# foggy-frost-forest/UniMoE-Audio

Hardware: AMD Instinct MI355X
Metric: audio-tokens/sec/node (TTS decode, bs=8 per GPU) (higher is better)
Workload: dtype bf16; 1 GPU; BASELINE configs[1]: TTS decode batch 8 (16 CFG rows) per GPU, 300-token prompt, 36-layer DCMoE (8+1 routed, 2 shared), 12x1027 codec head, CFG 3.0 + top-k 45 + top-p 0.95 sampling, 16 kHz DAC 50 frames/s; global_batch=8, prompt_len=300, kv_len_end=396, parallelism=single, graph=True

## Files before the change

include/umoe.h:

```cpp
#ifndef UMOE_H
#define UMOE_H

#include <stddef.h>
#include <stdint.h>

#ifdef __cplusplus
extern "C" {
#endif

typedef void* umoe_stream_t;

const char* umoe_last_error(void);
int umoe_abi_version(void);
size_t umoe_struct_size(const char* name);

size_t umoe_packed_elems(int N, int K);
int umoe_pack_weight(const uint16_t* W, int N, int K, uint16_t* packed, umoe_stream_t stream);
int umoe_pack_gate_up(const uint16_t* Wg, const uint16_t* Wu, int I, int K, uint16_t* packed, umoe_stream_t stream);

typedef struct {
    const uint16_t* x;
    const uint16_t* gate_w;
    const uint16_t* norm_w;
    uint16_t* h_out;
// ... 366 lines not shown
int umoe_delay_step(int64_t* pred, int32_t* tokens, int32_t* state, const int32_t* delay, int B, int C, int Tmax,
                    int eos, int pad, int max_delay, umoe_stream_t stream);
int umoe_delay_step_rows(int64_t* pred, int32_t* tokens, int32_t* state, const int32_t* delay, int B, int C, int Tmax,
                         int eos, int pad, int max_delay, const umoe_row_params* row_params, umoe_stream_t stream);
int umoe_delay_step_clock(int64_t* pred, int32_t* tokens, int32_t* state, const int32_t* delay, int B, int C, int Tmax,
                          int eos, int pad, int max_delay, const umoe_row_params* row_params, const int32_t* row_clock,
                          umoe_stream_t stream);

int umoe_codec_ce_fwd(const float* logits, const int64_t* labels, int N, int C, int V, float* nll_ws, float* probs,
                      float* ch_loss, int32_t* ch_count, float* total, umoe_stream_t stream);
int umoe_codec_ce_bwd(const float* probs, const int64_t* labels, const int32_t* ch_count, int N, int C, int V, float grad,
                      float* dlogits, umoe_stream_t stream);

int umoe_rvq_from_codes(const int32_t* codes, const float* codebooks, const float* out_w, const float* out_b, int NQ,
                        int CB, int cd, int Dl, int T, float* z, umoe_stream_t stream);
int umoe_rvq_from_delayed(const int32_t* tokens, int B, int Tmax, int NQ, const int32_t* prefill_step, const int32_t* delay, int t_valid,
                          int pad, const int32_t* rows, int Bz, int f0, int n, const float* codebooks, const float* out_w, const float* out_b,
                          int CB, int cd, int Dl, float* z, int z_off, int Lz, umoe_stream_t stream);
int umoe_rvq_nearest(const float* z, const float* codebooks, const float* in_w, const float* in_b, const float* out_w,
                     const float* out_b, int NQ, int CB, int cd, int Dl, int T, int32_t* codes, float* resid_ws,
                     umoe_stream_t stream);

int umoe_dac_conv1d(const float* x, const float* w, const float* bias, const float* snake_alpha, const float* resid, int B, int Cin,
                    int L, int Cout, int K, int stride, int dilation, int pad, int act, float* y, int* Lout_out, umoe_stream_t stream);
int umoe_dac_conv_transpose1d(const float* x, const float* w, const float* bias, const float* snake_alpha, int B, int Cin, int L,
                              int Cout, int K, int stride, int pad, int out_pad, float* y, int* Lout_out, umoe_stream_t stream);
int umoe_dac_conv1d_win(const float* x, int x_off, int Lx, const float* w, const float* bias, const float* snake_alpha, const float* resid,
                        int r_off, int Lr, int B, int Cin, int L, int Cout, int K, int stride, int dilation, int pad, int act, int t_begin,
                        int n, float* y, int y_off, int Ly, umoe_stream_t stream);
int umoe_dac_conv_transpose1d_win(const float* x, int x_off, int Lx, const float* w, const float* bias, const float* snake_alpha, int B,
                                  int Cin, int L, int Cout, int K, int stride, int pad, int out_pad, int t_begin, int n, float* y, int y_off,
                                  int Ly, umoe_stream_t stream);
int umoe_dac_resample(const float* x, const float* kern, int B, int L, int o, int n, int width, int Lout, float* y, umoe_stream_t stream);

int umoe_vision_rope(uint16_t* qkv, const float* cos_t, const float* sin_t, int S, int H, int hd, umoe_stream_t stream);
int umoe_vision_attn(const uint16_t* qkv, const int32_t* seg_lo, const int32_t* seg_hi, int S, int H, int hd, float scale, uint16_t* out,
                     umoe_stream_t stream);
int umoe_swiglu_pair(const uint16_t* gu, int S, int I, int ldh, uint16_t* h, umoe_stream_t stream);
int umoe_gelu(uint16_t* x, long n, umoe_stream_t stream);

typedef struct {
    int hidden, layers, heads, kv_heads, head_dim;
    int n_dyn, n_real, n_fix, inter_dyn, inter_shared;
    int codec_channels, codec_vocab, eos, pad, bos;
    int mrope0, mrope1, mrope2;
    float rms_eps, top_p;
    int fixed_top_k;
    double jitter_eps;
    int rows;
    int Lmax;
    int Tmax;
    int attn_splits;
    int ep_rank, ep_size;
} umoe_engine_cfg;

typedef struct {
    const uint16_t* in_norm;
    const uint16_t* qkv_w;
    const float* qkv_b;
    const uint16_t* o_w;
    const uint16_t* post_norm;
    const uint16_t* gate_w;
    const uint16_t* const* exp_gu;
    const uint16_t* const* exp_dn;
    const uint16_t* const* sh_gu;
    const uint16_t* const* sh_dn;
    const uint16_t* rm_qkv;
    const uint16_t* rm_o;
    const uint16_t* const* rm_exp_gate;
    const uint16_t* const* rm_exp_up;
    const uint16_t* const* rm_exp_down;
    const uint16_t* const* rm_sh_gate;
    const uint16_t* const* rm_sh_up;
    const uint16_t* const* rm_sh_down;
} umoe_layer_weights;

typedef struct umoe_engine umoe_engine;
int umoe_engine_create(const umoe_engine_cfg* cfg, umoe_engine** out);
void umoe_engine_destroy(umoe_engine* e);
int umoe_engine_set_layer(umoe_engine* e, int layer, const umoe_layer_weights* w);
int umoe_engine_set_layer_fp8(umoe_engine* e, int layer, const uint8_t* const* gu8, const int8_t* const* gu_e, const uint8_t* const* dn8,
                              const int8_t* const* dn_e);
int umoe_engine_set_fp8_wide(umoe_engine* e, int on);
int umoe_fp8_convert_probe(const uint8_t* q, const int8_t* e, int N, int K, uint16_t* out, umoe_stream_t stream);
int umoe_engine_set_globals(umoe_engine* e, const uint16_t* final_norm, const uint16_t* codec_emb,
                            const uint16_t* codec_head_w, const uint16_t* cos_tab, const uint16_t* sin_tab, int max_pos,
                            const int32_t* delay_pattern_host);
size_t umoe_engine_workspace_bytes(const umoe_engine* e);
int umoe_engine_prefill(umoe_engine* e, const uint16_t* x, const uint8_t* valid_host, int T, umoe_stream_t stream);
int umoe_engine_prefill_pos(umoe_engine* e, const uint16_t* x, const uint8_t* valid_host, int T, const int32_t* pos3_host,
                            const int32_t* next_pos_host, umoe_stream_t stream);
int umoe_engine_prefill_external(umoe_engine* e, const uint8_t* valid_host, int T, const int32_t* pos3_host, const int32_t* next_pos_host,
                                 umoe_stream_t stream);
typedef struct {
    int32_t* tokens;
    int32_t* state;
    float cfg_scale, temperature, top_p, eos_mul;
    int top_k, do_sample, min_tokens;
    uint64_t seed;
    int32_t* row_clock;
    const umoe_row_params* row_params;
} umoe_decode_io;
int umoe_engine_decode_step(umoe_engine* e, const umoe_decode_io* io, umoe_stream_t stream);
int umoe_engine_capture(umoe_engine* e, const umoe_decode_io* io, umoe_stream_t stream);
int umoe_engine_replay(umoe_engine* e, umoe_stream_t stream);
int umoe_engine_profile_step(umoe_engine* e, const umoe_decode_io* io, umoe_stream_t stream, float* ms, int* launches,
                             int n);
int umoe_engine_reserve(umoe_engine* e, int n_tok);
int umoe_engine_admit(umoe_engine* e, const umoe_decode_io* io, int b, const uint16_t* x, const uint8_t* valid_host, int T,
                      int prefill_step, int prefix_len, umoe_stream_t stream);
int umoe_engine_admit_external(umoe_engine* e, const umoe_decode_io* io, int b, const uint8_t* valid_host, int T, int prefill_step,
                               int prefix_len, umoe_stream_t stream);
enum { UMOE_EP_PEER = 0, UMOE_EP_LOOPBACK = 1, UMOE_EP_RCCL = 2 };
int umoe_engine_ep_region(umoe_engine* e, void** base_out, size_t* bytes_out);
int umoe_engine_ep_connect(umoe_engine* e, void* const* peers, void* rccl_comm, int mode);
int umoe_engine_ep_error(umoe_engine* e, umoe_stream_t stream, int* code_out);
int umoe_engine_set_probe(umoe_engine* e, const uint16_t* teach_x, uint16_t* dump_x1, uint16_t* dump_x, uint16_t* dump_logits);
int umoe_engine_info(umoe_engine* e, const char* key);
const void* umoe_engine_buffer(umoe_engine* e, const char* name, size_t* bytes);

#ifdef __cplusplus
}
#endif
#endif
```

unimoe_audio_amd/_lib.py:

```python
from __future__ import annotations

import ctypes as C
import os
import subprocess

_HERE = os.path.dirname(os.path.abspath(__file__))
_CSRC = os.path.join(_HERE, "csrc")
_SO = os.environ.get("UMOE_HIP_LIB") or os.path.join(_CSRC, "libumoe_hip.so")
_lib = None


class UmoeError(RuntimeError):
    pass


def build(force: bool = False) -> str:
    srcs = [os.path.join(_CSRC, f) for f in os.listdir(_CSRC) if f.endswith((".hip", ".h"))]
    srcs.append(os.path.join(os.path.dirname(_HERE), "include", "umoe.h"))
    stale = (not os.path.exists(_SO)) or any(os.path.getmtime(s) > os.path.getmtime(_SO) for s in srcs)
    if force or stale:
        subprocess.check_call(["make", "-C", _CSRC, "-j4", "-s"])
    return _SO


# ... 44 lines not shown
                ("counts", vp), ("offsets", vp), ("slot_token", vp), ("max_rows", i32), ("slot_rows", i32), ("row_base", i32),
                ("x", vp), ("ldx", i32), ("h", vp), ("ldh", i32), ("gu", vp), ("ldgu", i32), ("dy", vp), ("lddy", i32),
                ("dx_slots", vp), ("lddx", i32), ("dw_gate", C.POINTER(vp)), ("dw_up", C.POINTER(vp)), ("dw_down", C.POINTER(vp)),
                ("ws", vp), ("ws_bytes", C.c_size_t), ("w_down_T", vp), ("w_gateup_T", vp)]


class AttnBwdArgs(C.Structure):
    _fields_ = [("q", vp), ("k_cache", vp), ("v_cache", vp), ("kv_start_host", vp), ("d_out", vp), ("rows", i32), ("T", i32), ("H", i32),
                ("KVH", i32), ("hd", i32), ("Lmax", i32), ("scale", f32), ("dq", vp), ("dk_cache", vp), ("dv_cache", vp), ("ws", vp),
                ("ws_bytes", C.c_size_t), ("out", vp), ("lse", vp)]


class CombineArgs(C.Structure):
    _fields_ = [("y_slots", vp), ("slot_of", vp), ("moe_w", vp), ("y_shared", vp), ("global_w", vp), ("resid", vp),
                ("out", vp), ("S", i32), ("D", i32), ("n_real", i32), ("n_dyn", i32), ("n_fix", i32), ("y_parts", vp), ("n_parts", i32), ("part_stride", C.c_long),
                ("shared_row0", i32), ("norm_w", vp),
                ("norm_out", vp), ("rms_eps", f32), ("expert_mask", vp), ("mask_ld", i32), ("dense_rows", i32), ("ep_xfer", vp)]


class RopeArgs(C.Structure):
    _fields_ = [("qkv", vp), ("cos_tab", vp), ("sin_tab", vp), ("pos3", vp), ("kv_pos", vp), ("n_tok", i32), ("T", i32),
                ("H", i32), ("KVH", i32), ("hd", i32), ("sec0", i32), ("sec1", i32), ("sec2", i32), ("Lmax", i32),
                ("q_out", vp), ("k_cache", vp), ("v_cache", vp)]


class AttnArgs(C.Structure):
    _fields_ = [("q", vp), ("k_cache", vp), ("v_cache", vp), ("kv_start", vp), ("q_pos0", vp), ("rows", i32),
                ("nq", i32), ("H", i32), ("KVH", i32), ("hd", i32), ("Lmax", i32), ("splits", i32), ("scale", f32),
                ("part_o", vp), ("part_ml", vp), ("out", vp), ("qkv_raw", vp), ("cos_tab", vp), ("sin_tab", vp), ("pos3", vp),
                ("sec0", i32), ("sec1", i32), ("sec2", i32), ("lse_out", vp)]


class RowParams(C.Structure):
    _fields_ = [("cfg_scale", f32), ("temperature", f32), ("top_p", f32), ("eos_mul", f32), ("top_k", C.c_int32), ("do_sample", C.c_int32),
                ("min_tokens", C.c_int32), ("max_tokens", C.c_int32), ("seed", u64)]


class SampleArgs(C.Structure):
    _fields_ = [("logits", vp), ("B", i32), ("C", i32), ("V", i32), ("cfg_scale", f32), ("temperature", f32),
                ("top_p", f32), ("eos_mul", f32), ("top_k", i32), ("eos", i32), ("enable_eos", i32),
                ("min_tokens", i32), ("step", vp), ("do_sample", i32), ("seed", u64), ("pred", vp), ("probs_out", vp),
                ("row_clock", vp), ("row_params", vp)]


class EngineCfg(C.Structure):
    _fields_ = [("hidden", i32), ("layers", i32), ("heads", i32), ("kv_heads", i32), ("head_dim", i32),
                ("n_dyn", i32), ("n_real", i32), ("n_fix", i32), ("inter_dyn", i32), ("inter_shared", i32),
                ("codec_channels", i32), ("codec_vocab", i32), ("eos", i32), ("pad", i32), ("bos", i32),
                ("mrope0", i32), ("mrope1", i32), ("mrope2", i32), ("rms_eps", f32), ("top_p", f32),
                ("fixed_top_k", i32), ("jitter_eps", f64), ("rows", i32), ("Lmax", i32), ("Tmax", i32),
                ("attn_splits", i32), ("ep_rank", i32), ("ep_size", i32)]


class LayerWeights(C.Structure):
    _fields_ = [("in_norm", vp), ("qkv_w", vp), ("qkv_b", vp), ("o_w", vp), ("post_norm", vp), ("gate_w", vp),
                ("exp_gu", C.POINTER(vp)), ("exp_dn", C.POINTER(vp)), ("sh_gu", C.POINTER(vp)), ("sh_dn", C.POINTER(vp)),
                ("rm_qkv", vp), ("rm_o", vp), ("rm_exp_gate", C.POINTER(vp)), ("rm_exp_up", C.POINTER(vp)),
                ("rm_exp_down", C.POINTER(vp)), ("rm_sh_gate", C.POINTER(vp)), ("rm_sh_up", C.POINTER(vp)),
                ("rm_sh_down", C.POINTER(vp))]


class DecodeIO(C.Structure):
    _fields_ = [("tokens", vp), ("state", vp), ("cfg_scale", f32), ("temperature", f32), ("top_p", f32),
                ("eos_mul", f32), ("top_k", i32), ("do_sample", i32), ("min_tokens", i32), ("seed", u64), ("row_clock", vp), ("row_params", vp)]


EXPORTS = [
    "umoe_last_error", "umoe_abi_version", "umoe_packed_elems", "umoe_pack_weight", "umoe_pack_gate_up",
    "umoe_router_fwd", "umoe_router_dispatch_fwd", "umoe_dispatch_build", "umoe_transpose_slots_compact", "umoe_aux_loss_fwd", "umoe_aux_loss_fwd_ws", "umoe_aux_loss_workspace_floats", "umoe_permute_fwd", "umoe_grouped_gemm", "umoe_grouped_swiglu_fwd", "umoe_shared_swiglu_fwd", "umoe_attn_prefill_fwd",
    "umoe_unpermute_combine_fwd", "umoe_rmsnorm_residual_fwd", "umoe_qkv_mrope_kvappend", "umoe_attn_decode",
    "umoe_codec_embed_sum", "umoe_codec_embed_sum_bwd", "umoe_mul_noise", "umoe_codec_head_cfg_sample", "umoe_delay_step", "umoe_rvq_from_codes",
    "umoe_rvq_nearest", "umoe_codec_ce_fwd", "umoe_codec_ce_bwd", "umoe_engine_create", "umoe_engine_destroy", "umoe_engine_set_layer",
    "umoe_engine_set_globals", "umoe_engine_workspace_bytes", "umoe_engine_prefill", "umoe_engine_decode_step",
    "umoe_engine_capture", "umoe_engine_replay", "umoe_engine_buffer", "umoe_engine_profile_step", "umoe_prefetch", "umoe_tiled_gemm", "umoe_tiled_gemm_tn", "umoe_tiled_gemm_tn_workspace_bytes", "umoe_tiled_gemm_tn_split", "umoe_dispatch_build_aligned", "umoe_transpose_slots", "umoe_swiglu_bwd",
    "umoe_unpermute_combine_bwd", "umoe_permute_bwd", "umoe_router_bwd", "umoe_rmsnorm_residual_bwd", "umoe_aux_loss_bwd", "umoe_attn_softmax_fwd", "umoe_attn_softmax_bwd", "umoe_qkv_mrope_bwd",
    "umoe_swiglu_bwd_workspace_bytes", "umoe_grouped_swiglu_bwd", "umoe_shared_swiglu_bwd",
    "umoe_attn_prefill_bwd_workspace_bytes", "umoe_attn_prefill_bwd",
    "umoe_ep_unique_id", "umoe_ep_comm_create", "umoe_ep_comm_destroy", "umoe_ep_all_to_all",
    "umoe_ep_ipc_export", "umoe_ep_ipc_open", "umoe_ep_ipc_close", "umoe_engine_ep_region", "umoe_engine_ep_connect",
    "umoe_engine_ep_error", "umoe_token_drop", "umoe_router_bwd_drop", "umoe_router_bwd_ex", "umoe_dac_conv1d", "umoe_dac_conv_transpose1d", "umoe_dac_resample", "umoe_vision_rope", "umoe_vision_attn", "umoe_swiglu_pair", "umoe_gelu", "umoe_engine_prefill_pos", "umoe_engine_set_probe", "umoe_engine_info", "umoe_engine_prefill_external", "umoe_engine_set_layer_fp8", "umoe_fp8_convert_probe",
    "umoe_dac_conv1d_win", "umoe_dac_conv_transpose1d_win", "umoe_rvq_from_delayed", "umoe_delay_step_rows",
    "umoe_delay_step_clock", "umoe_engine_reserve", "umoe_engine_admit", "umoe_engine_admit_external", "umoe_gemm_wide", "umoe_pack_rows",
    "umoe_gemm_wide_fp8", "umoe_engine_set_fp8_wide", "umoe_tiled_gemm_wp8",
]

EP_PEER, EP_LOOPBACK, EP_RCCL = 0, 1, 2
MAX_EP = 8


def _mirrors():
    return {"umoe_router_args": RouterArgs, "umoe_group_t": Group, "umoe_gemm_args": GemmArgs, "umoe_tgroup_t": TGroup,
            "umoe_tgemm_args": TGemmArgs, "umoe_tn_group_t": TnGroup, "umoe_tgemm_tn_args": TGemmTnArgs, "umoe_swiglu_bwd_args": SwigluBwdArgs, "umoe_attn_bwd_args": AttnBwdArgs,
            "umoe_combine_args": CombineArgs, "umoe_rope_args": RopeArgs, "umoe_attn_args": AttnArgs, "umoe_sample_args": SampleArgs,
            "umoe_engine_cfg": EngineCfg, "umoe_layer_weights": LayerWeights, "umoe_decode_io": DecodeIO}


STRUCT_MIRRORS = _mirrors()
TABLE_MIRRORS = {"umoe_row_params": RowParams}


def lib():
    global _lib
    if _lib is None:
        if not os.path.exists(_SO):
            raise UmoeError(f"{_SO} is missing: run `python -c 'import __graft_entry__ as g; g.build()'` "
                            "(hipcc --offload-arch=gfx950). There is no CPU fallback for the product path.")
        L = C.CDLL(_SO)
        L.umoe_last_error.restype = C.c_char_p
        L.umoe_packed_elems.restype = C.c_size_t
        L.umoe_packed_elems.argtypes = [i32, i32]
        L.umoe_engine_workspace_bytes.restype = C.c_size_t
        L.umoe_engine_workspace_bytes.argtypes = [vp]
        L.umoe_engine_buffer.restype = vp
        L.umoe_engine_buffer.argtypes = [vp, C.c_char_p, C.POINTER(C.c_size_t)]
        L.umoe_engine_destroy.restype = None
        L.umoe_engine_destroy.argtypes = [vp]
        L.umoe_pack_weight.argtypes = [vp, i32, i32, vp, vp]
        L.umoe_pack_gate_up.argtypes = [vp, vp, i32, i32, vp, vp]
        L.umoe_router_fwd.argtypes = [C.POINTER(RouterArgs), vp]
        L.umoe_dispatch_build.argtypes = [vp, i32, i32, i32, vp, vp, vp, vp, vp]
        L.umoe_aux_loss_fwd.argtypes = [vp, i32, vp, vp, i32, i32, i32, vp, vp]
        L.umoe_aux_loss_fwd_ws.argtypes = [vp, i32, vp, vp, i32, i32, i32, vp, vp, vp]
        L.umoe_aux_loss_workspace_floats.argtypes = []
        L.umoe_aux_loss_workspace_floats.restype = C.c_size_t
        L.umoe_prefetch.argtypes = [vp, C.c_size_t, i32, vp]
        L.umoe_transpose_slots.argtypes = [vp, i32, i32, vp, vp, vp, i32, i32, vp, i32, vp]
        L.umoe_swiglu_bwd.argtypes = [vp, i32, vp, i32, i32, vp, i32, vp, i32, vp]
        L.umoe_unpermute_combine_bwd.argtypes = [vp, vp, vp, vp, vp, vp, vp]
        L.umoe_permute_bwd.argtypes = [vp, vp, i32, vp, i32, i32, i32, vp, vp, vp]
        L.umoe_router_bwd.argtypes = [vp, i32, vp, vp, vp, vp, vp, vp, i32, i32, i32, i32, f64, vp, vp]
        L.umoe_router_bwd_drop.argtypes = [vp, i32, vp, vp, vp, vp, vp, vp, i32, i32, i32, i32, f64, vp, vp]
        L.umoe_router_bwd_ex.argtypes = [vp, i32, vp, vp, vp, vp, vp, vp, i32, i32, i32, i32, f64, i32, vp, vp, vp]
        L.umoe_dac_conv1d.argtypes = [vp, vp, vp, vp, vp, i32, i32, i32, i32, i32, i32, i32, i32, i32, vp, C.POINTER(i32), vp]
        L.umoe_dac_conv_transpose1d.argtypes = [vp, vp, vp, vp, i32, i32, i32, i32, i32, i32, i32, i32, vp, C.POINTER(i32), vp]
        L.umoe_dac_resample.argtypes = [vp, vp, i32, i32, i32, i32, i32, i32, vp, vp]
        L.umoe_dac_conv1d_win.argtypes = [vp, i32, i32, vp, vp, vp, vp, i32, i32] + [i32] * 9 + [i32, i32, vp, i32, i32, vp]
        L.umoe_dac_conv_transpose1d_win.argtypes = [vp, i32, i32, vp, vp, vp] + [i32] * 8 + [i32, i32, vp, i32, i32, vp]
        L.umoe_rvq_from_delayed.argtypes = [vp, i32, i32, i32, vp, vp, i32, i32, vp, i32, i32, i32, vp, vp, vp, i32, i32, i32, vp, i32, i32, vp]
        L.umoe_vision_rope.argtypes = [vp, vp, vp, i32, i32, i32, vp]
        L.umoe_vision_attn.argtypes = [vp, vp, vp, i32, i32, i32, f32, vp, vp]
        L.umoe_swiglu_pair.argtypes = [vp, i32, i32, i32, vp, vp]
        L.umoe_gelu.argtypes = [vp, C.c_long, vp]
        L.umoe_engine_prefill_pos.argtypes = [vp, vp, vp, i32, vp, vp, vp]
        L.umoe_token_drop.argtypes = [vp, i32, vp, vp, i32, i32, i32, i32, i32, i32, vp, vp, vp, vp, vp]
        L.umoe_rmsnorm_residual_bwd.argtypes = [vp, vp, vp, vp, f32, i32, i32, vp, vp, vp, C.c_size_t, vp]
        L.umoe_dispatch_build_aligned.argtypes = [vp, i32, i32, i32, i32, vp, vp, vp, vp, vp]
        L.umoe_aux_loss_bwd.argtypes = [vp, i32, vp, vp, i32, i32, i32, vp, vp, vp, vp]
        L.umoe_attn_softmax_fwd.argtypes = [vp, i32, i32, i32, i32, i32, f32, vp, i32, vp]
        L.umoe_attn_softmax_bwd.argtypes = [vp, vp, i32, i32, i32, i32, f32, vp, vp]
        L.umoe_qkv_mrope_bwd.argtypes = [C.POINTER(RopeArgs), vp, vp, vp, vp, vp]
        L.umoe_tiled_gemm_tn.argtypes = [C.POINTER(TGemmTnArgs), vp]
        L.umoe_tiled_gemm_tn_workspace_bytes.argtypes = [C.POINTER(TGemmTnArgs)]
        L.umoe_tiled_gemm_tn_workspace_bytes.restype = C.c_size_t
        L.umoe_tiled_gemm_tn_split.argtypes = [C.POINTER(TGemmTnArgs)]
        L.umoe_swiglu_bwd_workspace_bytes.argtypes = [C.POINTER(SwigluBwdArgs)]
        L.umoe_swiglu_bwd_workspace_bytes.restype = C.c_size_t
        L.umoe_grouped_swiglu_bwd.argtypes = [C.POINTER(SwigluBwdArgs), vp]
        L.umoe_shared_swiglu_bwd.argtypes = [C.POINTER(SwigluBwdArgs), vp]
        L.umoe_attn_prefill_bwd_workspace_bytes.argtypes = [C.POINTER(AttnBwdArgs)]
        L.umoe_attn_prefill_bwd_workspace_bytes.restype = C.c_size_t
        L.umoe_attn_prefill_bwd.argtypes = [C.POINTER(AttnBwdArgs), vp]
        L.umoe_ep_unique_id.argtypes = [vp]
        L.umoe_ep_comm_create.argtypes = [vp, i32, i32, C.POINTER(vp)]
        L.umoe_ep_comm_destroy.argtypes = [vp]
        L.umoe_ep_all_to_all.argtypes = [vp, vp, vp, C.c_size_t, i32, vp]
        L.umoe_ep_ipc_export.argtypes = [vp, vp]
        L.umoe_ep_ipc_open.argtypes = [vp, C.POINTER(vp)]
        L.umoe_ep_ipc_close.argtypes = [vp]
        L.umoe_engine_ep_region.argtypes = [vp, C.POINTER(vp), C.POINTER(C.c_size_t)]
        L.umoe_engine_ep_connect.argtypes = [vp, C.POINTER(vp), vp, i32]
        L.umoe_engine_ep_error.argtypes = [vp, vp, C.POINTER(i32)]
        L.umoe_engine_set_probe.argtypes = [vp, vp, vp, vp, vp]
        L.umoe_engine_info.argtypes = [vp, C.c_char_p]
        L.umoe_engine_prefill_external.argtypes = [vp, vp, i32, vp, vp, vp]
        L.umoe_router_dispatch_fwd.argtypes = [C.POINTER(RouterArgs), vp, vp, vp, vp, vp]
        L.umoe_permute_fwd.argtypes = [vp, i32, vp, vp, i32, vp, vp]
        L.umoe_grouped_gemm.argtypes = [C.POINTER(GemmArgs), vp]
        L.umoe_unpermute_combine_fwd.argtypes = [C.POINTER(CombineArgs), vp]
        L.umoe_rmsnorm_residual_fwd.argtypes = [vp, vp, vp, f32, i32, i32, vp, vp, vp]
        L.umoe_qkv_mrope_kvappend.argtypes = [C.POINTER(RopeArgs), vp]
        L.umoe_attn_decode.argtypes = [C.POINTER(AttnArgs), vp]
        L.umoe_attn_prefill_fwd.argtypes = [C.POINTER(AttnArgs), vp]
        L.umoe_codec_embed_sum.argtypes = [vp, vp, i32, i32, i32, i32, vp, vp]
        L.umoe_codec_embed_sum_bwd.argtypes = [vp, vp, i32, i32, i32, i32, vp, vp]
        L.umoe_mul_noise.argtypes = [vp, vp, C.c_long, vp, vp]
        L.umoe_codec_head_cfg_sample.argtypes = [C.POINTER(SampleArgs), vp]
        L.umoe_delay_step.argtypes = [vp, vp, vp, vp, i32, i32, i32, i32, i32, i32, vp]
        if not hasattr(L, "umoe_delay_step_rows"):
            raise UmoeError(f"{_SO} predates this package (no umoe_delay_step_rows): rebuild it (`make -C unimoe_audio_amd/csrc`)")
        L.umoe_delay_step_rows.argtypes = [vp, vp, vp, vp, i32, i32, i32, i32, i32, i32, vp, vp]
        if not hasattr(L, "umoe_engine_admit"):
            raise UmoeError(f"{_SO} predates this package (no umoe_engine_admit): rebuild it (`make -C unimoe_audio_amd/csrc`)")
        L.umoe_delay_step_clock.argtypes = [vp, vp, vp, vp, i32, i32, i32, i32, i32, i32, vp, vp, vp]
        L.umoe_engine_reserve.argtypes = [vp, i32]
        L.umoe_engine_admit.argtypes = [vp, C.POINTER(DecodeIO), i32, vp, vp, i32, i32, i32, vp]
        L.umoe_engine_admit_external.argtypes = [vp, C.POINTER(DecodeIO), i32, vp, i32, i32, i32, vp]
        if not hasattr(L, "umoe_gemm_wide"):
            raise UmoeError(f"{_SO} predates this package (no umoe_gemm_wide): rebuild it (`make -C unimoe_audio_amd/csrc`)")
        L.umoe_gemm_wide.argtypes = [C.POINTER(vp), C.POINTER(i32), C.POINTER(i32), i32, i32, C.POINTER(vp), C.POINTER(vp), i32, i32,
                                     C.POINTER(vp), C.POINTER(vp), i32, i32, i32, vp]
        L.umoe_pack_rows.argtypes = [vp, i32, i32, i32, vp, f32, vp, vp]
        if not hasattr(L, "umoe_gemm_wide_fp8"):
            raise UmoeError(f"{_SO} predates this package (no umoe_gemm_wide_fp8): rebuild it (`make -C unimoe_audio_amd/csrc`)")
        L.umoe_gemm_wide_fp8.argtypes = [C.POINTER(vp), C.POINTER(vp), C.POINTER(i32), C.POINTER(i32), i32, i32, C.POINTER(vp), C.POINTER(vp), i32, i32,
                                         i32, i32, i32, vp]
        L.umoe_engine_set_fp8_wide.argtypes = [vp, i32]
        if not hasattr(L, "umoe_tiled_gemm_wp8"):
            raise UmoeError(f"{_SO} predates this package (no umoe_tiled_gemm_wp8): rebuild it (`make -C unimoe_audio_amd/csrc`)")
        L.umoe_tiled_gemm_wp8.argtypes = [C.POINTER(TGemmArgs), C.POINTER(vp), C.POINTER(vp), vp]
        L.umoe_rvq_from_codes.argtypes = [vp, vp, vp, vp, i32, i32, i32, i32, i32, vp, vp]
        L.umoe_rvq_nearest.argtypes = [vp, vp, vp, vp, vp, vp, i32, i32, i32, i32, i32, vp, vp, vp]
        L.umoe_codec_ce_fwd.argtypes = [vp, vp, i32, i32, i32, vp, vp, vp, vp, vp, vp]
        L.umoe_codec_ce_bwd.argtypes = [vp, vp, vp, i32, i32, i32, f32, vp, vp]
        L.umoe_engine_create.argtypes = [C.POINTER(EngineCfg), C.POINTER(vp)]
        L.umoe_engine_set_layer.argtypes = [vp, i32, C.POINTER(LayerWeights)]
        L.umoe_engine_set_globals.argtypes = [vp, vp, vp, vp, vp, vp, i32, vp]
        L.umoe_engine_prefill.argtypes = [vp, vp, vp, i32, vp]
        L.umoe_engine_decode_step.argtypes = [vp, C.POINTER(DecodeIO), vp]
        L.umoe_engine_capture.argtypes = [vp, C.POINTER(DecodeIO), vp]
        L.umoe_engine_replay.argtypes = [vp, vp]
        L.umoe_engine_profile_step.argtypes = [vp, C.POINTER(DecodeIO), vp, C.POINTER(f32), C.POINTER(i32), i32]
        if not hasattr(L, "umoe_struct_size"):
            raise UmoeError(f"{_SO} predates this package (no umoe_struct_size): rebuild it (`make -C unimoe_audio_amd/csrc`)")
        L.umoe_struct_size.restype = C.c_size_t
        L.umoe_struct_size.argtypes = [C.c_char_p]
        for cname, cls in list(STRUCT_MIRRORS.items()) + list(TABLE_MIRRORS.items()):
            built = int(L.umoe_struct_size(cname.encode()))
            if built != C.sizeof(cls):
                raise UmoeError(f"{_SO}: sizeof({cname}) is {built} in the library and {C.sizeof(cls)} in unimoe_audio_amd/_lib.py: "
                                "the library and the package are of different versions -- rebuild (`make -C unimoe_audio_amd/csrc`)")
        _lib = L
    return _lib


def check(rc: int, what: str = ""):
    if rc != 0:
        msg = lib().umoe_last_error()
        raise UmoeError(f"{what} failed (rc={rc}): {msg.decode() if msg else ''}")
```

unimoe_audio_amd/csrc/umoe_common.h:

```cpp
#pragma once
#include <hip/hip_runtime.h>
#include <stdarg.h>
#include <stdint.h>
#include <stdio.h>

#include "umoe.h"

typedef __attribute__((ext_vector_type(8))) __bf16 bf16x8_t;
typedef __attribute__((ext_vector_type(4))) float f32x4_t;

#define UMOE_MAXE 16

void umoe_set_error(const char* fmt, ...);
#define UMOE_HIP(expr)                                                                      \
    do {                                                                                    \
        hipError_t _e = (expr);                                                             \
        if (_e != hipSuccess) {                                                             \
            umoe_set_error("%s failed: %s (%s:%d)", #expr, hipGetErrorString(_e), __FILE__, __LINE__); \
            return -2;                                                                      \
        }                                                                                   \
    } while (0)
#define UMOE_REQUIRE(cond, ...)          \
    do {                                 \
        if (!(cond)) {                   \
// ... 101 lines not shown
    p = fma(p, r, 1.0 / 3628800.0);
    p = fma(p, r, 1.0 / 362880.0);
    p = fma(p, r, 1.0 / 40320.0);
    p = fma(p, r, 1.0 / 5040.0);
    p = fma(p, r, 1.0 / 720.0);
    p = fma(p, r, 1.0 / 120.0);
    p = fma(p, r, 1.0 / 24.0);
    p = fma(p, r, 1.0 / 6.0);
    p = fma(p, r, 0.5);
    p = fma(p, r, 1.0);
    p = fma(p, r, 1.0);
    const long long ki = (long long)k;
    const double scale = __longlong_as_double((ki + 1023) << 52);
    return (float)(p * scale);
}

__device__ __forceinline__ float wave_sum(float v) {
#pragma unroll
    for (int o = 32; o >= 1; o >>= 1) v += __shfl_xor(v, o, 64);
    return v;
}
__device__ __forceinline__ float wave_max(float v) {
#pragma unroll
    for (int o = 32; o >= 1; o >>= 1) v = fmaxf(v, __shfl_xor(v, o, 64));
    return v;
}

#if defined(__HIPCC__)
__device__ __forceinline__ float block_sum_256(float v, float* sh) {
    v = wave_sum(v);
    if ((threadIdx.x & 63) == 0) sh[threadIdx.x >> 6] = v;
    __syncthreads();
    const float r = sh[0] + sh[1] + sh[2] + sh[3];
    __syncthreads();
    return r;
}
#endif
static inline int ceil_div(int a, int b) { return (a + b - 1) / b; }

struct BwdSide {
    hipStream_t side = nullptr;
    hipEvent_t fork = nullptr, mid = nullptr, join = nullptr;
    bool ok = false;
};
BwdSide& bwd_side();

#define UMOE_EP_PARTS 16
#define UMOE_EP_FLAG_BYTES (2 * UMOE_MAX_EP * UMOE_EP_PARTS * 64)
struct umoe_ep_xfer {
    char* peer_base[UMOE_MAX_EP];
    const char* src;
    long src_stride;
    char* dst;
    size_t chunk;
    size_t data_off;
    int kind;
    int rank, size, loopback;
    int rows, row_bytes, n_sub;
    const uint32_t* step;
    int layer, layers;
    uint32_t* err;
    const uint32_t* round;
    int n_cwg;
};
int umoe_ep_push(const umoe_ep_xfer& x, hipStream_t s);
int umoe_ep_pull(const umoe_ep_xfer& x, hipStream_t s);
int umoe_ep_pull_pack(const umoe_ep_xfer& x, const uint16_t* own_rows, hipStream_t s);
int umoe_router_norm_push(const umoe_router_args* a, const umoe_ep_xfer& x, hipStream_t s);
int umoe_ep_rccl_allgather(void* comm, const void* send, void* recv, size_t bytes, hipStream_t s);

#define UMOE_FLAG_REPL 8
struct umoe_rider_pub {
    uint32_t* flags;
    const uint32_t* step;
    int layer, layers;
    uint32_t* err;
};

int umoe_moe_flat(const umoe_gemm_args* gu, const umoe_gemm_args* dn, uint32_t* flags, int flag_words, int n_wg, hipStream_t s);
bool umoe_moe_flat_feasible(int n_wg, int S, int D, int I_dyn, int I_sh, int n_real, int n_fix);
int umoe_moe_flat_fp8(const umoe_gemm_args* gu, const umoe_gemm_args* dn, const int8_t* const* e_gu, const int8_t* const* e_dn, uint32_t* flags,
                      int flag_words, int n_wg, hipStream_t s);
bool umoe_moe_flat_fp8_feasible(int n_wg, int S, int D, int I_dyn, int I_sh, int n_real, int n_fix);

struct umoe_rider2;
int umoe_gemm_riders(const umoe_gemm_args* a, int kind, const umoe_rider2* r2, const umoe_rider_pub* pub, hipStream_t s);

#define UMOE_MT_MAXG 4
#define UMOE_MT_MAXT UMOE_MAX_EP
struct umoe_mt_args {
    const uint16_t* w[UMOE_MT_MAXG];
    int num_groups, n_blocks, k;
    int tiles, n_rows;
    const uint16_t* b;
    int b_group_tiles;
    uint16_t* h_out;
    uint16_t* y_out[UMOE_MT_MAXG][UMOE_MT_MAXT];
    int ldo;
    int epilogue;
    const umoe_router_args* fused_router;
};
int umoe_gemm_mt(const umoe_mt_args* a, hipStream_t s);

#define UMOE_EPF_MAXT 24
struct umoe_epf_desc {
    const umoe_router_args* router;
    const umoe_rider_pub* pub;
    int R, rank, loopback, E_loc, S, D, I_dyn, I_sh, n_fix, n_wg;
    char* const* peer_base;
    size_t disp_off, ret_off;
    const uint16_t* const* w_lgu;
    const uint16_t* const* w_ldn;
    const uint16_t* const* w_sgu;
    const uint16_t* const* w_sdn;
    uint16_t* xgp;
    uint16_t* hpk;
    uint16_t* h_sh; int ldh, h_row0;
    uint16_t* y_sh; int ldy, y_row0;
    uint32_t* flags; int flag_words;
    const uint32_t* round;
    uint32_t* tasks_dev;
    int n_cwg;
    int proda_base[4], proda_n[4], prodb_base[UMOE_MT_MAXG], prodb_n[UMOE_MT_MAXG];
};
int umoe_moe_ep_prepare(umoe_epf_desc* d, hipStream_t s);
int umoe_moe_ep(const umoe_epf_desc* d, hipStream_t s);

#if defined(__HIPCC__)
typedef __attribute__((address_space(1))) uint32_t umoe_gu32;
#define UMOE_SYS_AUX 17
__device__ __forceinline__ umoe_gu32* umoe_ep_flag(char* base, int kind, int tile, int part) {
    return reinterpret_cast<umoe_gu32*>(reinterpret_cast<uintptr_t>(base + ((size_t)(kind * UMOE_MAX_EP + tile) * UMOE_EP_PARTS + part) * 64));
}
__device__ __forceinline__ uint32_t umoe_ep_epoch(const umoe_ep_xfer& x) { return *x.step * (uint32_t)x.layers + (uint32_t)x.layer + 1u; }
__device__ __forceinline__ void umoe_ep_wait(umoe_gu32* flag, uint32_t epoch, uint32_t* err_word) {
    umoe_gu32* err = reinterpret_cast<umoe_gu32*>(reinterpret_cast<uintptr_t>(err_word));
    const unsigned long long t0 = wall_clock64();
    for (unsigned spins = 0;; ++spins) {
        const uint32_t v = __hip_atomic_load(flag, __ATOMIC_RELAXED, __HIP_MEMORY_SCOPE_SYSTEM);
        if ((int32_t)(v - epoch) >= 0) break;
        __builtin_amdgcn_s_sleep(2);
        if ((spins & 255u) == 255u) {
            if (__hip_atomic_load(err, __ATOMIC_RELAXED, __HIP_MEMORY_SCOPE_AGENT) != 0u) break;
            if (wall_clock64() - t0 > 1000000000ull) {
                __hip_atomic_store(err, 1u, __ATOMIC_RELAXED, __HIP_MEMORY_SCOPE_AGENT);
                break;
            }
        }
    }
}
#endif
```

unimoe_audio_amd/csrc/umoe_engine.hip:

```cpp
#include <string.h>

#include <string>
#include <vector>

#include "umoe_common.h"
#include "umoe_riders_dev.h"

namespace {

struct LayerDev {
    umoe_layer_weights w;
    std::vector<const uint16_t*> exp_gu, exp_dn, sh_gu, sh_dn;
    std::vector<const uint16_t*> rm_eg, rm_eu, rm_ed, rm_sg, rm_su, rm_sd;
    bool has_rm = false;
    bool has_rm_attn = false;
    bool has_rm_exp = false;
    bool exp_bf16 = true;
    bool set = false;
    std::vector<const uint16_t*> f8_gu, f8_dn;
    std::vector<const int8_t*> f8e_gu, f8e_dn;
    bool has_f8 = false;
};

struct Carver {
    char* base = nullptr;
    size_t off = 0;
    template <typename T>
    T* take(size_t n) {
        off = (off + 255) & ~(size_t)255;
        T* p = base ? reinterpret_cast<T*>(base + off) : nullptr;
        off += n * sizeof(T);
        return p;
    }
};

}

struct umoe_engine {
    umoe_engine_cfg c;
    std::vector<LayerDev> layers;
    const uint16_t *final_norm = nullptr, *codec_emb = nullptr, *codec_head_w = nullptr, *cos_tab = nullptr,
                   *sin_tab = nullptr;
    int max_pos = 0;
    int max_delay = 0;
    char* ws = nullptr;
    size_t ws_bytes = 0;
    int cap_tok = 0;
    uint16_t *k_cache = nullptr, *v_cache = nullptr;
    int32_t* d_delay = nullptr;
    umoe_group_t* d_groups = nullptr;
    std::vector<umoe_group_t> h_groups;
    std::vector<umoe_group_t> h_gu_pub;
    int groups_for_tok = -1;
    uint16_t *x = nullptr, *hin = nullptr, *x1 = nullptr, *h2 = nullptr, *qkv = nullptr, *q_r = nullptr, *attn_out = nullptr,
             *hbuf = nullptr, *ybuf = nullptr;
    float *part_o = nullptr, *part_ml = nullptr, *logits = nullptr, *ypart = nullptr;
    int32_t *pos3 = nullptr, *kv_pos = nullptr, *q_pos0 = nullptr, *kv_start = nullptr, *tok_in = nullptr,
            *valid_count = nullptr, *eng_state = nullptr;
    void* r_logits = nullptr;
    int64_t *r_topk = nullptr, *pred = nullptr;
    int32_t *r_sel = nullptr, *r_mask = nullptr, *counts = nullptr, *offsets = nullptr, *slot_token = nullptr,
            *slot_of = nullptr;
    float *r_routing = nullptr, *r_global = nullptr, *r_moe = nullptr;
    int32_t* all_mask = nullptr;
    int64_t* all_topk = nullptr;
    int T_prompt = 0;
    int adm_row0 = -1;
    int32_t* adm_q0 = nullptr;
    int reserved_tok = 0;
    const uint16_t* probe_teach = nullptr;
    uint16_t *probe_x1 = nullptr, *probe_x = nullptr, *probe_logits = nullptr;
    bool probe_on() const { return probe_teach || probe_x1 || probe_x || probe_logits; }
    hipGraph_t graph = nullptr;
    hipGraphExec_t exec = nullptr;
    bool fuse_router = true;
    bool fuse_cq = true;
    int cb_ep_layer = -1;
    bool cb_pending = false;
    umoe_combine_args cb_stash{};
    int dense_min_rows = 2;
    int expert_launch = 0;
    bool fp8 = false;
    int prefill_fp8 = 0;
    int expert_fp8 = 0;
    bool fp8_wide = false;
    int n_cu = 0;
    bool tiled_prefill = true;
    bool prof = false;
    std::vector<hipEvent_t> ev;
    std::vector<int> ev_kind;
    size_t ev_used = 0;
    int E_loc = 0;
    char* ep_region = nullptr;
    size_t ep_region_bytes = 0;
    int ep_mem_kind = 0;
    char* ep_peers[UMOE_MAX_EP] = {};
    void* ep_comm = nullptr;
    int ep_mode = -1;
    uint32_t* ep_words = nullptr;
    uint16_t* xg = nullptr;
    uint16_t *xgp = nullptr, *hpk = nullptr;
    uint16_t *wide_in = nullptr, *wide_h = nullptr;
    int row_tiles = 1;
    bool in_decode_step = false;
    bool ep_flat = true;
    bool epf_ready = false;
    umoe_epf_desc epf{};
    uint32_t* epf_tasks = nullptr;
    bool ep_decode(int n_tok) const { return c.ep_size > 1 && n_tok == c.rows; }
    int groups_per_layer() const { return 2 + 2 * (c.n_real + c.n_fix); }
};

static size_t carve(umoe_engine* e, int n_tok, char* base) {
    const umoe_engine_cfg& c = e->c;
    const int D = c.hidden, QKV = (c.heads + 2 * c.kv_heads) * c.head_dim, HD = c.heads * c.head_dim;
    const int E = c.n_dyn + c.n_fix, G = c.n_real + c.n_fix;
    const int Imax = c.inter_dyn > c.inter_shared ? c.inter_dyn : c.inter_shared;
    const size_t slots = (size_t)n_tok * G;
    const int splits = c.attn_splits > 1 ? c.attn_splits : 1;
    Carver k;
    k.base = base;
    e->x = k.take<uint16_t>((size_t)n_tok * D);
    e->hin = k.take<uint16_t>((size_t)n_tok * D);
    e->x1 = k.take<uint16_t>((size_t)n_tok * D);
    e->h2 = k.take<uint16_t>((size_t)n_tok * D);
    e->qkv = k.take<uint16_t>((size_t)n_tok * QKV);
    e->q_r = k.take<uint16_t>((size_t)n_tok * HD);
    e->attn_out = k.take<uint16_t>((size_t)n_tok * HD);
    e->hbuf = k.take<uint16_t>(slots * Imax);
    e->ybuf = k.take<uint16_t>(slots * D + (c.ep_size > 1 ? (size_t)c.n_real * c.rows * D : 0));
    e->xg = k.take<uint16_t>(c.ep_size > 1 ? (size_t)c.ep_size * c.rows * D : 0);
    e->xgp = k.take<uint16_t>(c.ep_size > 1 ? (size_t)c.ep_size * 16 * D : 0);
    e->hpk = k.take<uint16_t>(c.ep_size > 1 ? (size_t)c.n_real * 16 * c.inter_dyn : 0);
    const int wt = (c.ep_size == 1 && c.rows > 16 && c.rows <= 64) ? ceil_div(c.rows, 16) : 0;
    e->wide_in = k.take<uint16_t>((size_t)wt * 16 * (D > HD ? D : HD));
    e->wide_h = k.take<uint16_t>((size_t)wt * 16 * Imax * G);
    e->part_o = k.take<float>((size_t)n_tok * c.heads * splits * c.head_dim);
    e->part_ml = k.take<float>((size_t)n_tok * c.heads * splits * 2);
    e->logits = k.take<float>((size_t)c.rows * c.codec_channels * c.codec_vocab);
    e->pos3 = k.take<int32_t>((size_t)3 * n_tok);
    e->kv_pos = k.take<int32_t>(n_tok);
    e->q_pos0 = k.take<int32_t>(c.rows);
    e->kv_start = k.take<int32_t>(c.rows);
    e->valid_count = k.take<int32_t>(c.rows);
    e->eng_state = k.take<int32_t>(8);
    e->tok_in = k.take<int32_t>((size_t)c.rows * c.codec_channels);
    e->r_logits = k.take<float>((size_t)n_tok * E);
    e->r_topk = k.take<int64_t>(n_tok);
    e->pred = k.take<int64_t>((size_t)c.rows * c.codec_channels);
    e->r_sel = k.take<int32_t>((size_t)n_tok * c.n_dyn);
    e->r_mask = k.take<int32_t>((size_t)n_tok * E);
    e->counts = k.take<int32_t>(UMOE_MAXE);
    e->offsets = k.take<int32_t>(UMOE_MAXE + 1);
    e->slot_token = k.take<int32_t>((size_t)n_tok * c.n_real + 1);
    e->slot_of = k.take<int32_t>((size_t)n_tok * c.n_real);
    e->r_routing = k.take<float>((size_t)n_tok * c.n_dyn);
    e->r_global = k.take<float>((size_t)n_tok * E);
    e->r_moe = k.take<float>((size_t)n_tok * c.n_real);
    e->all_mask = k.take<int32_t>((size_t)c.layers * c.rows * E);
    e->all_topk = k.take<int64_t>((size_t)c.layers * c.rows);
    return (k.off + 255) & ~(size_t)255;
}

static int ensure_workspace(umoe_engine* e, int n_tok) {
    if (n_tok <= e->cap_tok) return 0;
    if (e->ws) UMOE_HIP(hipFree(e->ws));
// ... 175 lines not shown
    if (const char* v = getenv("UMOE_FUSE_ROUTER")) e->fuse_router = atoi(v) != 0;
    if (const char* v = getenv("UMOE_DENSE_MIN_ROWS")) e->dense_min_rows = atoi(v);
    if (const char* v = getenv("UMOE_FUSE_CQ")) e->fuse_cq = atoi(v) != 0;
    *out = e;
    return 0;
}

extern "C" void umoe_engine_destroy(umoe_engine* e) {
    if (!e) return;
    if (e->exec) (void)hipGraphExecDestroy(e->exec);
    if (e->graph) (void)hipGraphDestroy(e->graph);
    for (hipEvent_t x : e->ev) (void)hipEventDestroy(x);
    if (e->ws) (void)hipFree(e->ws);
    if (e->adm_q0) (void)hipFree(e->adm_q0);
    if (e->ep_region) (void)hipFree(e->ep_region);
    if (e->ep_words) (void)hipFree(e->ep_words);
    if (e->epf_tasks) (void)hipFree(e->epf_tasks);
    if (e->k_cache) (void)hipFree(e->k_cache);
    if (e->v_cache) (void)hipFree(e->v_cache);
    if (e->d_delay) (void)hipFree(e->d_delay);
    if (e->d_groups) (void)hipFree(e->d_groups);
    delete e;
}

extern "C" int umoe_engine_set_layer(umoe_engine* e, int layer, const umoe_layer_weights* w) {
    UMOE_REQUIRE(e && w && layer >= 0 && layer < e->c.layers, "umoe_engine_set_layer: bad layer %d", layer);
    LayerDev& L = e->layers[layer];
    L.w = *w;
    const bool any_exp = w->exp_gu || w->exp_dn || w->sh_gu || w->sh_dn || w->rm_exp_gate || w->rm_exp_up || w->rm_exp_down || w->rm_sh_gate ||
                         w->rm_sh_up || w->rm_sh_down;
    L.exp_bf16 = any_exp;
    if (any_exp) {
        UMOE_REQUIRE(w->exp_gu && w->exp_dn && (e->c.n_fix == 0 || (w->sh_gu && w->sh_dn)),
                     "umoe_engine_set_layer: layer %d: exp_gu / exp_dn / sh_gu / sh_dn go together (all NULL with every rm_exp_* / rm_sh_*: an fp8-only layer)", layer);
        L.exp_gu.assign(w->exp_gu, w->exp_gu + e->E_loc);
        L.exp_dn.assign(w->exp_dn, w->exp_dn + e->E_loc);
        L.sh_gu.assign(w->sh_gu, w->sh_gu + e->c.n_fix);
        L.sh_dn.assign(w->sh_dn, w->sh_dn + e->c.n_fix);
    } else {
        UMOE_REQUIRE(e->c.ep_size == 1, "umoe_engine_set_layer: layer %d: an fp8-only layer (no bf16 expert weights) is not supported expert parallel", layer);
        L.exp_gu.assign(e->E_loc, nullptr); L.exp_dn.assign(e->E_loc, nullptr);
        L.sh_gu.assign(e->c.n_fix, nullptr); L.sh_dn.assign(e->c.n_fix, nullptr);
    }
    L.has_rm_attn = w->rm_qkv && w->rm_o;
    L.has_rm_exp = w->rm_exp_gate && w->rm_exp_up && w->rm_exp_down && (e->c.n_fix == 0 || (w->rm_sh_gate && w->rm_sh_up && w->rm_sh_down));
    L.has_rm = L.has_rm_attn && L.has_rm_exp;
    L.rm_eg.clear(); L.rm_eu.clear(); L.rm_ed.clear(); L.rm_sg.clear(); L.rm_su.clear(); L.rm_sd.clear();
    if (L.has_rm) {
        L.rm_eg.assign(w->rm_exp_gate, w->rm_exp_gate + e->c.n_real);
        L.rm_eu.assign(w->rm_exp_up, w->rm_exp_up + e->c.n_real);
        L.rm_ed.assign(w->rm_exp_down, w->rm_exp_down + e->c.n_real);
        if (e->c.n_fix) {
            L.rm_sg.assign(w->rm_sh_gate, w->rm_sh_gate + e->c.n_fix);
            L.rm_su.assign(w->rm_sh_up, w->rm_sh_up + e->c.n_fix);
            L.rm_sd.assign(w->rm_sh_down, w->rm_sh_down + e->c.n_fix);
        }
    }
    L.set = true;
    e->groups_for_tok = -1;
    return 0;
}

extern "C" int umoe_engine_set_layer_fp8(umoe_engine* e, int layer, const uint8_t* const* gu8, const int8_t* const* gu_e, const uint8_t* const* dn8,
                                         const int8_t* const* dn_e) {
    UMOE_REQUIRE(e && gu8 && gu_e && dn8 && dn_e && layer >= 0 && layer < e->c.layers, "umoe_engine_set_layer_fp8: bad argument (layer %d)", layer);
    UMOE_REQUIRE(e->c.ep_size == 1, "umoe_engine_set_layer_fp8: fp8 expert weights run on the flat expert launch only, not expert parallel (ep_size %d)",
                 e->c.ep_size);
    LayerDev& L = e->layers[layer];
    UMOE_REQUIRE(L.set, "umoe_engine_set_layer_fp8: umoe_engine_set_layer(%d) first", layer);
    const int G = e->c.n_real + e->c.n_fix;
    for (int i = 0; i < G; ++i)
        UMOE_REQUIRE(gu8[i] && gu_e[i] && dn8[i] && dn_e[i], "umoe_engine_set_layer_fp8: layer %d group %d: null pointer", layer, i);
    L.f8_gu.assign(G, nullptr); L.f8_dn.assign(G, nullptr);
    for (int i = 0; i < G; ++i) {
        L.f8_gu[i] = reinterpret_cast<const uint16_t*>(gu8[i]);
        L.f8_dn[i] = reinterpret_cast<const uint16_t*>(dn8[i]);
    }
    L.f8e_gu.assign(gu_e, gu_e + G); L.f8e_dn.assign(dn_e, dn_e + G);
    L.has_f8 = true;
    e->fp8 = true;
    return 0;
}

extern "C" int umoe_engine_set_fp8_wide(umoe_engine* e, int on) {
    UMOE_REQUIRE(e, "umoe_engine_set_fp8_wide: null engine");
    e->fp8_wide = on != 0;
    return 0;
}

extern "C" int umoe_engine_set_globals(umoe_engine* e, const uint16_t* final_norm, const uint16_t* codec_emb,
                                       const uint16_t* codec_head_w, const uint16_t* cos_tab, const uint16_t* sin_tab,
                                       int max_pos, const int32_t* delay_pattern_host) {
    UMOE_REQUIRE(e && final_norm && codec_emb && codec_head_w && cos_tab && sin_tab && delay_pattern_host,
                 "umoe_engine_set_globals: null argument");
    e->final_norm = final_norm; e->codec_emb = codec_emb; e->codec_head_w = codec_head_w;
    e->cos_tab = cos_tab; e->sin_tab = sin_tab; e->max_pos = max_pos;
    UMOE_HIP(hipMemcpy(e->d_delay, delay_pattern_host, sizeof(int32_t) * e->c.codec_channels, hipMemcpyHostToDevice));
    e->max_delay = 0;
    for (int i = 0; i < e->c.codec_channels; ++i) e->max_delay = delay_pattern_host[i] > e->max_delay ? delay_pattern_host[i] : e->max_delay;
    e->groups_for_tok = -1;
    return 0;
}

extern "C" size_t umoe_engine_workspace_bytes(const umoe_engine* e) { return e ? e->ws_bytes : 0; }

extern "C" int umoe_engine_ep_region(umoe_engine* e, void** base_out, size_t* bytes_out) {
    UMOE_REQUIRE(e && base_out && bytes_out, "umoe_engine_ep_region: null argument");
    UMOE_REQUIRE(e->c.ep_size > 1 && e->ep_region, "umoe_engine_ep_region: engine was created with ep_size 1");
    *base_out = e->ep_region;
    *bytes_out = e->ep_region_bytes;
    return 0;
}

extern "C" int umoe_engine_ep_connect(umoe_engine* e, void* const* peers, void* rccl_comm, int mode) {
    UMOE_REQUIRE(e && e->c.ep_size > 1, "umoe_engine_ep_connect: engine was created with ep_size 1");
    UMOE_REQUIRE(mode == UMOE_EP_PEER || mode == UMOE_EP_LOOPBACK || mode == UMOE_EP_RCCL, "umoe_engine_ep_connect: bad mode %d", mode);
    if (mode == UMOE_EP_RCCL) {
        UMOE_REQUIRE(rccl_comm, "umoe_engine_ep_connect: the RCCL mode needs a communicator");
        e->ep_comm = rccl_comm;
        for (int p = 0; p < e->c.ep_size; ++p) e->ep_peers[p] = e->ep_region;
    } else if (mode == UMOE_EP_LOOPBACK) {
        for (int p = 0; p < e->c.ep_size; ++p) e->ep_peers[p] = e->ep_region;
    } else {
        UMOE_REQUIRE(peers, "umoe_engine_ep_connect: the peer mode needs every rank's region");
        for (int p = 0; p < e->c.ep_size; ++p) {
            UMOE_REQUIRE(peers[p], "umoe_engine_ep_connect: region of rank %d is null", p);
            e->ep_peers[p] = (char*)peers[p];
        }
        UMOE_REQUIRE(e->ep_peers[e->c.ep_rank] == e->ep_region, "umoe_engine_ep_connect: peers[ep_rank] must be this engine's own region");
    }
    e->ep_mode = mode;
    e->groups_for_tok = -1;
    e->epf_ready = false;
    const umoe_engine_cfg& c = e->c;
    if (mode != UMOE_EP_RCCL && e->ep_flat && e->fuse_router && e->n_cu > 0 && c.hidden == 2048 && c.n_dyn == 9 && c.n_fix == 2 && c.rows <= 16 &&
        e->E_loc >= 1 && e->E_loc <= UMOE_MT_MAXG) {
        umoe_epf_desc& d = e->epf;
        memset(&d, 0, sizeof(d));
        d.n_wg = e->n_cu < 256 ? e->n_cu : 256;
        d.R = c.ep_size; d.E_loc = e->E_loc; d.S = c.rows; d.D = c.hidden; d.I_dyn = c.inter_dyn; d.I_sh = c.inter_shared; d.n_fix = c.n_fix;
        if (!e->epf_tasks) UMOE_HIP(hipMalloc(&e->epf_tasks, (size_t)256 * UMOE_EPF_MAXT * sizeof(uint32_t)));
        d.tasks_dev = e->epf_tasks;
        const int rc = umoe_moe_ep_prepare(&d, nullptr);
        if (rc < 0) return rc;
        e->epf_ready = rc == 0;
    }
    return 0;
}

extern "C" int umoe_engine_ep_error(umoe_engine* e, umoe_stream_t stream, int* code_out) {
    UMOE_REQUIRE(e && code_out, "umoe_engine_ep_error: null argument");
    uint32_t w[2] = {0, 0};
    UMOE_HIP(hipStreamSynchronize((hipStream_t)stream));
    UMOE_HIP(hipMemcpy(w, e->ep_words, sizeof(w), hipMemcpyDeviceToHost));
    *code_out = (int)w[1];
    return 0;
}

enum { K_QKV = 0, K_ROPE, K_ATTN, K_OPROJ, K_ROUTER, K_DISPATCH, K_GATEUP, K_DOWN, K_COMBINE, K_EMBED, K_HEAD, K_SAMPLE,
       K_DELAY, K_NUM };

static void prof_mark(umoe_engine* e, int kind, hipStream_t s) {
    if (!e->prof) return;
    if (e->ev_used == e->ev.size()) {
        hipEvent_t x;
        if (hipEventCreate(&x) != hipSuccess) return;
// ... 176 lines not shown
    int rc;
    umoe_router_args ra{};
    ra.x = e->x1; ra.gate_w = L.w.gate_w; ra.norm_w = L.w.post_norm; ra.h_out = e->h2; ra.S = n_tok; ra.D = D;
    ra.n_dyn = c.n_dyn; ra.n_real = c.n_real; ra.n_fix = c.n_fix; ra.logits_bf16 = 1; ra.top_p = c.top_p;
    ra.fixed_top_k = c.fixed_top_k; ra.jitter_eps = c.jitter_eps; ra.rms_eps = c.rms_eps;
    ra.logits_out = e->r_logits; ra.sel = e->r_sel; ra.routing_w = e->r_routing; ra.global_w = e->r_global; ra.moe_w = e->r_moe;
    ra.expert_mask = e->all_mask + (size_t)l * c.rows * E;
    ra.top_k = e->all_topk + (size_t)l * c.rows;
    const size_t tile = (size_t)n_tok * D * 2, chunk_y = (size_t)El * tile;
    umoe_ep_xfer x{};
    for (int p = 0; p < ep; ++p) x.peer_base[p] = e->ep_peers[p];
    x.rank = rank; x.size = ep; x.loopback = e->ep_mode == UMOE_EP_LOOPBACK; x.step = e->ep_words; x.err = e->ep_words + 1;
    x.layer = l; x.layers = c.layers; x.rows = n_tok; x.row_bytes = D * 2;
    x.kind = 0; x.n_sub = 1; x.chunk = tile; x.data_off = UMOE_EP_FLAG_BYTES;
    umoe_router_args rn = ra;
    rn.norm_only = 1;
    if ((rc = umoe_router_norm_push(&rn, x, s))) return rc;
    ra.h_out = nullptr;
    PROF(K_ROUTER);
    umoe_gemm_args sg{};
    sg.groups = g + 2 + c.n_real; sg.groups_host = gh + 2 + c.n_real; sg.num_groups = c.n_fix; sg.max_rows = n_tok;
    sg.max_n_blocks = 2 * c.inter_shared / 16; sg.max_k = D; sg.a = e->h2; sg.lda = D; sg.out = e->hbuf; sg.ldo = Imax; sg.n_valid = Imax;
    sg.prologue = UMOE_PRO_PLAIN; sg.epilogue = UMOE_EPI_SWIGLU; sg.nt = 2; sg.waves = 8;
    if ((rc = umoe_grouped_gemm(&sg, s))) return rc;
    PROF(K_GATEUP);
    x.dst = (char*)e->xgp; x.chunk = tile;
    {
        umoe_ep_xfer xp = x;
        if ((rc = umoe_ep_pull_pack(xp, e->h2, s))) return rc;
    }
    PROF(K_DISPATCH);
    umoe_mt_args gu{};
    for (int q = 0; q < El; ++q) gu.w[q] = L.exp_gu[q];
    gu.num_groups = El; gu.n_blocks = 2 * c.inter_dyn / 16; gu.k = D; gu.tiles = ep; gu.n_rows = n_tok;
    gu.b = e->xgp; gu.b_group_tiles = 0; gu.h_out = e->hpk; gu.epilogue = UMOE_EPI_SWIGLU;
    gu.fused_router = e->fuse_router ? &ra : nullptr;
    if ((rc = umoe_gemm_mt(&gu, s))) return rc;
    if (!e->fuse_router) {
        if ((rc = umoe_router_fwd(&ra, s))) return rc;
    }
    PROF(K_GATEUP);
    uint16_t* yloc = e->ybuf + (size_t)G * n_tok * D;
    uint16_t* slab_ret = reinterpret_cast<uint16_t*>(e->ep_region + UMOE_EP_FLAG_BYTES + (size_t)ep * tile);
    umoe_mt_args dn{};
    for (int q = 0; q < El; ++q) dn.w[q] = L.exp_dn[q];
    dn.num_groups = El; dn.n_blocks = D / 16; dn.k = c.inter_dyn; dn.tiles = ep; dn.n_rows = n_tok;
    dn.b = e->hpk; dn.b_group_tiles = ep; dn.ldo = D; dn.epilogue = UMOE_EPI_BF16;
    for (int q = 0; q < El; ++q)
        for (int t = 0; t < ep; ++t)
            dn.y_out[q][t] = (t == rank) ? slab_ret + (size_t)(rank * El + q) * n_tok * D : yloc + (size_t)(t * El + q) * n_tok * D;
    if ((rc = umoe_gemm_mt(&dn, s))) return rc;
    PROF(K_DOWN);
    x.kind = 1; x.n_sub = El; x.chunk = chunk_y; x.data_off = UMOE_EP_FLAG_BYTES + (size_t)ep * tile;
    x.src = (const char*)yloc; x.src_stride = (long)chunk_y;
    if ((rc = umoe_ep_push(x, s))) return rc;
    PROF(K_DISPATCH);
    umoe_gemm_args sd{};
    sd.groups = g + 2 + G + c.n_real; sd.groups_host = gh + 2 + G + c.n_real; sd.num_groups = c.n_fix; sd.max_rows = n_tok;
    sd.max_n_blocks = D / 16; sd.max_k = c.inter_shared; sd.a = e->hbuf; sd.lda = Imax; sd.out = e->ybuf; sd.ldo = D; sd.n_valid = D;
    sd.prologue = UMOE_PRO_PLAIN; sd.epilogue = UMOE_EPI_BF16; sd.nt = 2; sd.waves = 8;
    if ((rc = umoe_grouped_gemm(&sd, s))) return rc;
    PROF(K_DOWN);
    umoe_combine_args cb{};
    cb.y_slots = slab_ret; cb.shared_row0 = -1; cb.slot_of = nullptr; cb.moe_w = e->r_moe;
    cb.expert_mask = ra.expert_mask; cb.mask_ld = E; cb.dense_rows = n_tok;
    cb.y_shared = e->ybuf + (size_t)n_tok * c.n_real * D; cb.global_w = e->r_global;
    cb.resid = e->x1; cb.out = e->x; cb.S = n_tok; cb.D = D; cb.n_real = c.n_real; cb.n_dyn = c.n_dyn; cb.n_fix = c.n_fix;
    cb.norm_w = (l + 1 < c.layers) ? e->layers[l + 1].w.in_norm : e->final_norm; cb.norm_out = e->hin; cb.rms_eps = c.rms_eps;
    cb.ep_xfer = &x;
    rc = umoe_unpermute_combine_fwd(&cb, s);
    PROF(K_COMBINE);
    return rc;
}

enum MoeForm {
    MOE_TILED,
    MOE_RAGGED,
    MOE_FLAT,
    MOE_RIDERS,
    MOE_ROUTER,
    MOE_WIDE,
};

static bool flat_moe_on() {
    const char* v = getenv("UMOE_FLAT_MOE");
    return !v || atoi(v) != 0;
}
static int flat_wgs(const umoe_engine* e) { return e->n_cu < 256 ? e->n_cu : 256; }

static MoeForm moe_form(const umoe_engine* e, const LayerDev& L, int n_tok) {
    const umoe_engine_cfg& c = e->c;
    if (wide_mode(e, n_tok)) return MOE_WIDE;
    if (!dense_mode(e, n_tok)) {
        if (!L.exp_bf16) return MOE_TILED;
        return (L.has_rm && n_tok >= 64 && e->tiled_prefill && c.n_real + c.n_fix <= 12) ? MOE_TILED : MOE_RAGGED;
    }
    if (!(e->fuse_router && c.n_dyn == 9 && c.n_fix == 2 && (c.hidden == 2048 || c.hidden == 4096))) return MOE_ROUTER;
    const int n_wg = flat_wgs(e);
    if (flat_moe_on() && n_wg > 0 && umoe_moe_flat_feasible(n_wg, n_tok, c.hidden, c.inter_dyn, c.inter_shared, c.n_real, c.n_fix)) return MOE_FLAT;
    return MOE_RIDERS;
}

static int experts_two_launches(umoe_engine* e, const umoe_gemm_args* gu, const umoe_gemm_args* dn, hipStream_t s) {
    int rc;
    if ((rc = umoe_grouped_gemm(gu, s))) return rc;
    PROF(K_GATEUP);
    if ((rc = umoe_grouped_gemm(dn, s))) return rc;
    PROF(K_DOWN);
    return 0;
}

static int experts_tiled(umoe_engine* e, const LayerDev& L, const umoe_group_t* gu_groups, int n_tok, hipStream_t s) {
    const umoe_engine_cfg& c = e->c;
    const int D = c.hidden, G = c.n_real + c.n_fix, Imax = c.inter_dyn > c.inter_shared ? c.inter_dyn : c.inter_shared;
    int rc;
    const bool f8 = !L.exp_bf16;
    const uint8_t* w8[12];
    const int8_t* ex[12];
    umoe_tgroup_t tg[12];
    memset(tg, 0, sizeof(tg));
    for (int x = 0; x < G; ++x) {
        const umoe_group_t& src = gu_groups[x];
        const bool sh = x >= c.n_real;
        if (f8) {
            w8[x] = reinterpret_cast<const uint8_t*>(L.f8_gu[x]); ex[x] = L.f8e_gu[x];
        } else {
            tg[x].w = sh ? L.rm_sg[x - c.n_real] : L.rm_eg[x];
            tg[x].w2 = sh ? L.rm_su[x - c.n_real] : L.rm_eu[x];
        }
        tg[x].rows = src.rows; tg[x].row_off = src.row_off; tg[x].count = src.count; tg[x].static_count = src.static_count;
        tg[x].a_row_base = src.a_row_base; tg[x].out_row_base = src.out_row_base;
        tg[x].n = sh ? c.inter_shared : c.inter_dyn; tg[x].k = D; tg[x].ldw = D;
    }
    umoe_tgemm_args ta{};
    ta.groups = tg; ta.num_groups = G; ta.max_rows = n_tok; ta.a = e->h2; ta.lda = D; ta.out = e->hbuf; ta.ldo = Imax;
    ta.epilogue = UMOE_EPI_SWIGLU;
    if ((rc = f8 ? umoe_tiled_gemm_wp8(&ta, w8, ex, s) : umoe_tiled_gemm(&ta, s))) return rc;
    PROF(K_GATEUP);
    memset(tg, 0, sizeof(tg));
    for (int x = 0; x < G; ++x) {
        const umoe_group_t& src = gu_groups[G + x];
        const bool sh = x >= c.n_real;
        if (f8) {
            w8[x] = reinterpret_cast<const uint8_t*>(L.f8_dn[x]); ex[x] = L.f8e_dn[x];
        } else {
            tg[x].w = sh ? L.rm_sd[x - c.n_real] : L.rm_ed[x];
        }
        tg[x].row_off = src.row_off; tg[x].count = src.count; tg[x].static_count = src.static_count;
        tg[x].a_row_base = src.a_row_base; tg[x].out_row_base = src.out_row_base;
        tg[x].n = D; tg[x].k = sh ? c.inter_shared : c.inter_dyn; tg[x].ldw = tg[x].k;
    }
    umoe_tgemm_args td{};
    td.groups = tg; td.num_groups = G; td.max_rows = n_tok; td.a = e->hbuf; td.lda = Imax; td.out = e->ybuf; td.ldo = D;
    td.epilogue = UMOE_EPI_BF16;
    if ((rc = f8 ? umoe_tiled_gemm_wp8(&td, w8, ex, s) : umoe_tiled_gemm(&td, s))) return rc;
    PROF(K_DOWN);
    if (f8) e->prefill_fp8 = 1;
    return 0;
}

static int wide_dense(umoe_engine* e, const uint16_t* a, int K, const uint16_t* w, int n_blocks, const float* bias, const uint16_t* resid, void* out,
                      int ldo, int n_valid, int epilogue, int u, int n_tok, hipStream_t s) {
    int rc;
    if ((rc = umoe_pack_rows(a, K, n_tok, K, nullptr, 0.f, e->wide_in, s))) return rc;
    PROF(K_DISPATCH);
    const uint16_t* b = e->wide_in;
// ... 90 lines not shown
                e->cb_ep_layer = -1;
            }
            rc = umoe_gemm_riders(&a, epc ? 4 : 2, &r2, &cpub, s);
            if (rc == 1) {
                if (epc) e->cb_stash.ep_xfer = &x;
                if ((rc = umoe_unpermute_combine_fwd(&e->cb_stash, s)) == 0) rc = 1;
            }
        }
        if (rc == 1) rc = umoe_grouped_gemm(&a, s);
    }
    if (rc) return rc;
    PROF(K_QKV);
    umoe_rope_args r{};
    r.qkv = e->qkv; r.cos_tab = e->cos_tab; r.sin_tab = e->sin_tab; r.pos3 = e->pos3; r.kv_pos = e->kv_pos;
    r.n_tok = n_tok; r.T = T; r.H = c.heads; r.KVH = c.kv_heads; r.hd = c.head_dim;
    r.sec0 = c.mrope0; r.sec1 = c.mrope1; r.sec2 = c.mrope2; r.Lmax = c.Lmax;
    r.q_out = e->q_r; r.k_cache = e->k_cache + kv_l; r.v_cache = e->v_cache + kv_l;
    const bool fuse_rope = (T == 1) && (c.mrope0 % 8 == 0) && ((c.mrope0 + c.mrope1) % 8 == 0);
    if (!fuse_rope) {
        if ((rc = umoe_qkv_mrope_kvappend(&r, s))) return rc;
        PROF(K_ROPE);
    }
    umoe_attn_args t{};
    t.q = e->q_r; t.k_cache = r.k_cache; t.v_cache = r.v_cache; t.kv_start = e->kv_start; t.q_pos0 = e->q_pos0;
    t.rows = c.rows; t.nq = T;
    if (adm) { t.kv_start = e->kv_start + e->adm_row0; t.q_pos0 = e->adm_q0; t.rows = 2; } t.H = c.heads; t.KVH = c.kv_heads; t.hd = c.head_dim; t.Lmax = c.Lmax; t.splits = splits;
    t.scale = 1.0f / sqrtf((float)c.head_dim); t.part_o = e->part_o; t.part_ml = e->part_ml; t.out = e->attn_out;
    if (fuse_rope) {
        t.qkv_raw = e->qkv; t.cos_tab = e->cos_tab; t.sin_tab = e->sin_tab; t.pos3 = e->pos3;
        t.sec0 = c.mrope0; t.sec1 = c.mrope1; t.sec2 = c.mrope2;
    }
    if ((rc = (T > 1 ? umoe_attn_prefill_fwd(&t, s) : umoe_attn_decode(&t, s)))) return rc;
    PROF(K_ATTN);
    umoe_gemm_args o{};
    o.groups = g + 1; o.groups_host = gh + 1; o.num_groups = 1; o.max_rows = n_tok; o.max_n_blocks = D / 16; o.max_k = HD;
    o.a = e->attn_out; o.lda = HD; o.resid = e->x; o.out = e->x1; o.ldo = D; o.n_valid = D;
    o.prologue = UMOE_PRO_PLAIN; o.epilogue = UMOE_EPI_BF16_RESID;
    if (wide) {
        rc = wide_dense(e, e->attn_out, HD, L.w.o_w, D / 16, nullptr, e->x, e->x1, D, D, UMOE_EPI_BF16_RESID, 16, n_tok, s);
    } else if (tiled) {
        umoe_tgroup_t tg{};
        tg.w = L.w.rm_o; tg.static_count = n_tok; tg.n = D; tg.k = HD; tg.ldw = HD;
        umoe_tgemm_args ta{};
        ta.groups = &tg; ta.num_groups = 1; ta.max_rows = n_tok; ta.a = e->attn_out; ta.lda = HD; ta.resid = e->x; ta.out = e->x1;
        ta.ldo = D; ta.epilogue = UMOE_EPI_BF16_RESID;
        rc = umoe_tiled_gemm(&ta, s);
    } else {
        rc = umoe_grouped_gemm(&o, s);
    }
    if (rc) return rc;
    PROF(K_OPROJ);
    if (e->probe_x1 && n_tok == c.rows && !adm)
        UMOE_HIP(hipMemcpyAsync(e->probe_x1 + (size_t)l * c.rows * D, e->x1, (size_t)c.rows * D * 2, hipMemcpyDeviceToDevice, s));
    if (e->ep_decode(n_tok)) return run_moe_ep(e, l, n_tok, s);
    const MoeForm form = moe_form(e, L, n_tok);
    const bool dense = form == MOE_FLAT || form == MOE_RIDERS || form == MOE_ROUTER || form == MOE_WIDE;
    if (form != MOE_WIDE && n_tok == c.rows && n_tok > 16 && !adm) {
        e->expert_launch = 0;
        e->row_tiles = 1;
    }
    UMOE_REQUIRE(!(e->fp8 && dense && form != MOE_FLAT && form != MOE_WIDE), "umoe_engine: fp8 expert weights need the flat expert launch (layer %d)", l);
    UMOE_REQUIRE(L.exp_bf16 || (L.has_f8 && (form == MOE_TILED || form == MOE_FLAT || form == MOE_WIDE)),
                 "umoe_engine: layer %d holds no bf16 expert weights (fp8-only) and this pass would stream them", l);
    umoe_router_args ra{};
    ra.x = e->x1; ra.gate_w = L.w.gate_w; ra.norm_w = L.w.post_norm; ra.h_out = e->h2; ra.S = n_tok; ra.D = D;
    ra.n_dyn = c.n_dyn; ra.n_real = c.n_real; ra.n_fix = c.n_fix; ra.logits_bf16 = 1; ra.top_p = c.top_p;
    ra.fixed_top_k = c.fixed_top_k; ra.jitter_eps = c.jitter_eps; ra.rms_eps = c.rms_eps;
    ra.logits_out = e->r_logits; ra.top_k = e->r_topk; ra.sel = e->r_sel; ra.expert_mask = e->r_mask;
    ra.routing_w = e->r_routing; ra.global_w = e->r_global; ra.moe_w = e->r_moe;
    if (n_tok == c.rows && !adm) {
        ra.expert_mask = e->all_mask + (size_t)l * c.rows * E;
        ra.top_k = e->all_topk + (size_t)l * c.rows;
    }
    umoe_gemm_args gu{};
    gu.groups = g + 2; gu.groups_host = gh + 2; gu.num_groups = G; gu.max_rows = n_tok;
    gu.max_n_blocks = 2 * Imax / 16; gu.max_k = D;
    gu.a = e->h2; gu.lda = D; gu.out = e->hbuf; gu.ldo = Imax; gu.n_valid = Imax;
    gu.prologue = UMOE_PRO_PLAIN; gu.epilogue = UMOE_EPI_SWIGLU; gu.nt = dense ? 14 : 0;
    umoe_gemm_args dn{};
    dn.groups = g + 2 + G; dn.groups_host = gh + 2 + G; dn.num_groups = G; dn.max_rows = n_tok; dn.max_n_blocks = D / 16;
    dn.max_k = Imax;
    dn.a = e->hbuf; dn.lda = Imax; dn.out = e->ybuf; dn.ldo = D; dn.n_valid = D;
    dn.prologue = UMOE_PRO_PLAIN; dn.epilogue = UMOE_EPI_BF16; dn.nt = dense ? 6 : 0;
    switch (form) {
        case MOE_TILED:
            if ((rc = umoe_router_dispatch_fwd(&ra, e->counts, e->offsets, e->slot_token, e->slot_of, s))) return rc;
            PROF(K_ROUTER);
            if ((rc = experts_tiled(e, L, gh + 2, n_tok, s))) return rc;
            break;
        case MOE_RAGGED:
            if ((rc = umoe_router_dispatch_fwd(&ra, e->counts, e->offsets, e->slot_token, e->slot_of, s))) return rc;
            PROF(K_ROUTER);
            if ((rc = experts_two_launches(e, &gu, &dn, s))) return rc;
            break;
        case MOE_FLAT: {
            umoe_rider_pub rpub{};
            rpub.flags = e->ep_words + 1024; rpub.step = e->ep_words; rpub.layer = l; rpub.layers = c.layers; rpub.err = e->ep_words + 1;
            gu.fused_router = &ra;
            gu.rider_pub = &rpub;
            gu.groups_host = e->h_gu_pub.data() + (size_t)l * G;
            const int n_wg = flat_wgs(e);
            if (e->fp8) {
                UMOE_REQUIRE(L.has_f8 && G <= UMOE_MAXE, "umoe_engine: fp8 expert weights: layer %d has none (umoe_engine_set_layer_fp8)", l);
                umoe_group_t g8u[UMOE_MAXE], g8d[UMOE_MAXE];
                const int8_t* e8u[UMOE_MAXE];
                const int8_t* e8d[UMOE_MAXE];
                for (int i = 0; i < G; ++i) {
                    const int x = i < c.n_fix ? c.n_real + i : i - c.n_fix;
                    g8u[i] = gu.groups_host[i]; g8u[i].w = L.f8_gu[x]; e8u[i] = L.f8e_gu[x];
                    g8d[i] = dn.groups_host[i]; g8d[i].w = L.f8_dn[i]; e8d[i] = L.f8e_dn[i];
                }
                umoe_gemm_args gu8 = gu, dn8 = dn;
                gu8.groups_host = g8u; dn8.groups_host = g8d;
                rc = umoe_moe_flat_fp8(&gu8, &dn8, e8u, e8d, e->ep_words + 64, 512 - 64, n_wg, s);
            } else {
                rc = umoe_moe_flat(&gu, &dn, e->ep_words + 64, 512 - 64, n_wg, s);
            }
            UMOE_REQUIRE(rc != 1, "umoe_engine: the %sflat expert launch has no schedule for this shape on %d workgroups (layer %d)", e->fp8 ? "fp8 " : "", n_wg, l);
            if (rc) return rc;
            e->expert_launch = 2;
            e->expert_fp8 = e->fp8 ? 1 : 0;
            PROF(K_GATEUP);
            break;
        }
        case MOE_RIDERS: {
            umoe_router_args rn = ra;
            rn.norm_only = 1;
            if ((rc = umoe_router_fwd(&rn, s))) return rc;
            PROF(K_ROUTER);
            ra.h_out = nullptr;
            gu.fused_router = &ra;
            if ((rc = experts_two_launches(e, &gu, &dn, s))) return rc;
            e->expert_launch = 0;
            e->expert_fp8 = 0;
            break;
        }
        case MOE_ROUTER:
            if ((rc = umoe_router_fwd(&ra, s))) return rc;
            PROF(K_ROUTER);
            if ((rc = experts_two_launches(e, &gu, &dn, s))) return rc;
            e->expert_launch = 0;
            e->expert_fp8 = 0;
            break;
        case MOE_WIDE:
            ra.h_out = nullptr;
            if ((rc = umoe_router_fwd(&ra, s))) return rc;
            PROF(K_ROUTER);
            if ((rc = experts_wide(e, L, n_tok, s))) return rc;
            e->expert_launch = 4;
            e->expert_fp8 = e->fp8 ? 1 : 0;
            e->row_tiles = ceil_div(n_tok, 16);
            break;
    }
    umoe_combine_args cb{};
    cb.y_slots = e->ybuf; cb.shared_row0 = -1; cb.slot_of = dense ? nullptr : e->slot_of; cb.moe_w = e->r_moe;
    cb.expert_mask = ra.expert_mask; cb.mask_ld = E; cb.dense_rows = n_tok;
    cb.y_shared = c.n_fix ? e->ybuf + (size_t)n_tok * c.n_real * D : nullptr; cb.global_w = e->r_global;
    cb.resid = e->x1; cb.out = e->x; cb.S = n_tok; cb.D = D; cb.n_real = c.n_real; cb.n_dyn = c.n_dyn; cb.n_fix = c.n_fix;
    cb.norm_w = (l + 1 < c.layers) ? e->layers[l + 1].w.in_norm : e->final_norm; cb.norm_out = e->hin; cb.rms_eps = c.rms_eps;
    const bool cq_fits = e->n_cu <= 0 || n_tok + QKV / 16 <= 2 * e->n_cu;
    if (dense && T == 1 && e->fuse_cq && cq_fits && l + 1 < c.layers && D == 2048 && n_tok <= 16 && c.n_fix >= 1 && !e->probe_on()) {
        e->cb_stash = cb;
        e->cb_pending = true;
        return 0;
    }
    rc = umoe_unpermute_combine_fwd(&cb, s);
    PROF(K_COMBINE);
    return rc;
}

__global__ void epoch_bump_kernel(uint32_t* ep_step) {
    if (threadIdx.x == 0) ep_step[0] += 1u;
}

extern "C" int umoe_engine_prefill(umoe_engine* e, const uint16_t* x, const uint8_t* valid_host, int T,
                                   umoe_stream_t stream) {
    return umoe_engine_prefill_pos(e, x, valid_host, T, nullptr, nullptr, stream);
}

static int prefill_state(umoe_engine* e, const uint8_t* valid_host, int T, const int32_t* pos3_host, const int32_t* next_pos_host, hipStream_t s) {
    const umoe_engine_cfg& c = e->c;
    const int n_tok = c.rows * T;
    std::vector<int32_t> pos((size_t)3 * n_tok), kvp(n_tok), start(c.rows), q0(c.rows, 0), vc(c.rows);
    for (int r = 0; r < c.rows; ++r) {
        int cnt = 0, first = T;
        for (int t = 0; t < T; ++t) {
            const int v = valid_host[(size_t)r * T + t] != 0;
            cnt += v;
            if (v && first == T) first = t;
            const int p = v ? cnt - 1 : 1;
            for (int k = 0; k < 3; ++k) {
                const int pk = pos3_host ? pos3_host[((size_t)k * c.rows + r) * T + t] : p;
                UMOE_REQUIRE(pk >= 0 && pk < e->max_pos, "umoe_engine_prefill: position %d outside the rope table (%d)", pk, e->max_pos);
                pos[(size_t)k * n_tok + r * T + t] = pk;
            }
            kvp[r * T + t] = t;
        }
        for (int t = first; t < T; ++t)
            UMOE_REQUIRE(valid_host[(size_t)r * T + t], "umoe_engine_prefill: row %d is not left-padded", r);
        start[r] = first;
        vc[r] = next_pos_host ? next_pos_host[r] : cnt;
        UMOE_REQUIRE(vc[r] >= 0 && vc[r] + c.Lmax - T < e->max_pos, "umoe_engine_prefill: rope table too short");
    }
    UMOE_HIP(hipMemcpyAsync(e->pos3, pos.data(), pos.size() * 4, hipMemcpyHostToDevice, s));
// ... 309 lines not shown
    if (int rc = fp8_only_check(e, 0)) return rc;
    if (!e->fp8) return 0;
    const umoe_engine_cfg& c = e->c;
    UMOE_REQUIRE(c.ep_size == 1, "umoe_engine: fp8 expert weights are not supported expert parallel (ep_size %d)", c.ep_size);
    if (e->fp8_wide && fp8_wide_on() && wide_shapes(e, c.rows)) {
        for (int l = 0; l < c.layers; ++l)
            UMOE_REQUIRE(e->layers[l].has_f8, "umoe_engine: fp8 expert weights: layer %d has none (umoe_engine_set_layer_fp8)", l);
        return 0;
    }
    UMOE_REQUIRE(flat_moe_on(), "umoe_engine: fp8 expert weights need the flat expert launch (UMOE_FLAT_MOE=0 UMOE_FUSE_CQ=0 is the bf16 launch-per-kernel form)");
    UMOE_REQUIRE(e->fuse_router, "umoe_engine: fp8 expert weights need the flat expert launch with its router riders (UMOE_FUSE_ROUTER=0 selects a bf16 path)");
    UMOE_REQUIRE(dense_mode(e, c.rows) && c.n_dyn == 9 && c.n_fix == 2 && (c.hidden == 2048 || c.hidden == 4096),
                 "umoe_engine: fp8 expert weights need the dense decode layout of the flat expert launch (rows %d)", c.rows);
    const int n_wg = flat_wgs(e);
    UMOE_REQUIRE(n_wg > 0 && umoe_moe_flat_feasible(n_wg, c.rows, c.hidden, c.inter_dyn, c.inter_shared, c.n_real, c.n_fix) &&
                     umoe_moe_flat_fp8_feasible(n_wg, c.rows, c.hidden, c.inter_dyn, c.inter_shared, c.n_real, c.n_fix),
                 "umoe_engine: fp8 expert weights: the flat expert launch has no schedule on %d compute units", e->n_cu);
    for (int l = 0; l < c.layers; ++l)
        UMOE_REQUIRE(e->layers[l].has_f8, "umoe_engine: fp8 expert weights: layer %d has none (umoe_engine_set_layer_fp8)", l);
    return 0;
}

extern "C" int umoe_engine_decode_step(umoe_engine* e, const umoe_decode_io* io, umoe_stream_t stream) {
    UMOE_REQUIRE(e && io && io->tokens && io->state, "umoe_engine_decode_step: null argument");
    UMOE_REQUIRE(e->T_prompt > 0 || (io->row_clock && e->reserved_tok > 0), "umoe_engine_decode_step: prefill first");
    UMOE_REQUIRE(!io->row_clock || e->c.ep_size == 1, "umoe_engine_decode_step: per-row clocks are not supported expert parallel");
    if (int rc = fp8_step_check(e)) return rc;
    return enqueue_step(e, io, (hipStream_t)stream);
}

extern "C" int umoe_engine_profile_step(umoe_engine* e, const umoe_decode_io* io, umoe_stream_t stream, float* ms,
                                        int* launches, int n) {
    UMOE_REQUIRE(e && io && ms && launches && n >= K_NUM, "umoe_engine_profile_step: need %d output slots", K_NUM);
    hipStream_t s = (hipStream_t)stream;
    if (int rc = fp8_step_check(e)) return rc;
    e->prof = true;
    e->ev_used = 0;
    const int rc = enqueue_step(e, io, s);
    e->prof = false;
    if (rc) return rc;
    UMOE_HIP(hipStreamSynchronize(s));
    for (size_t i = 1; i < e->ev_used; ++i) {
        const int k = e->ev_kind[i];
        if (k < 0) continue;
        float t = 0.f;
        UMOE_HIP(hipEventElapsedTime(&t, e->ev[i - 1], e->ev[i]));
        ms[k] += t;
        launches[k] += 1;
    }
    return 0;
}

extern "C" int umoe_engine_capture(umoe_engine* e, const umoe_decode_io* io, umoe_stream_t stream) {
    UMOE_REQUIRE(e && io && io->tokens && io->state, "umoe_engine_capture: null argument");
    UMOE_REQUIRE(e->T_prompt > 0 || (io->row_clock && e->reserved_tok > 0), "umoe_engine_capture: prefill first");
    UMOE_REQUIRE(!io->row_clock || e->c.ep_size == 1, "umoe_engine_capture: per-row clocks are not supported expert parallel");
    UMOE_REQUIRE(!e->probe_on(), "umoe_engine_capture: the per-layer probe works on eager steps only (umoe_engine_set_probe)");
    if (int rc = fp8_step_check(e)) return rc;
    hipStream_t s = (hipStream_t)stream;
    if (e->exec) { (void)hipGraphExecDestroy(e->exec); e->exec = nullptr; }
    if (e->graph) { (void)hipGraphDestroy(e->graph); e->graph = nullptr; }
    UMOE_HIP(hipStreamBeginCapture(s, hipStreamCaptureModeThreadLocal));
    const int rc = enqueue_step(e, io, s);
    hipGraph_t g = nullptr;
    const hipError_t ec = hipStreamEndCapture(s, &g);
    if (rc) return rc;
    UMOE_REQUIRE(ec == hipSuccess && g, "umoe_engine_capture: hipStreamEndCapture failed: %s", hipGetErrorString(ec));
    e->graph = g;
    UMOE_HIP(hipGraphInstantiate(&e->exec, e->graph, nullptr, nullptr, 0));
    return 0;
}

extern "C" int umoe_engine_replay(umoe_engine* e, umoe_stream_t stream) {
    UMOE_REQUIRE(e && e->exec, "umoe_engine_replay: no captured step");
    UMOE_HIP(hipGraphLaunch(e->exec, (hipStream_t)stream));
    return 0;
}

extern "C" int umoe_engine_info(umoe_engine* e, const char* key) {
    if (!e || !key) return -1;
    if (!strcmp(key, "expert_launch")) return e->expert_launch;
    if (!strcmp(key, "row_tiles")) return e->expert_launch == 4 ? e->row_tiles : 1;
    if (!strcmp(key, "expert_fp8")) return e->expert_fp8;
    if (!strcmp(key, "prefill_fp8")) return e->prefill_fp8;
    if (!strcmp(key, "expert_bf16_resident")) return fp8_only(e) ? 0 : 1;
    if (!strcmp(key, "n_cu")) return e->n_cu;
    return -1;
}

extern "C" int umoe_engine_set_probe(umoe_engine* e, const uint16_t* teach_x, uint16_t* dump_x1, uint16_t* dump_x, uint16_t* dump_logits) {
    UMOE_REQUIRE(e, "umoe_engine_set_probe: null engine");
    UMOE_REQUIRE(e->c.ep_size == 1 || !(teach_x || dump_x1 || dump_x || dump_logits), "umoe_engine_set_probe: not with expert parallel engines");
    e->probe_teach = teach_x; e->probe_x1 = dump_x1; e->probe_x = dump_x; e->probe_logits = dump_logits;
    return 0;
}

extern "C" const void* umoe_engine_buffer(umoe_engine* e, const char* name, size_t* bytes) {
    if (!e || !name) return nullptr;
    const umoe_engine_cfg& c = e->c;
    const int E = c.n_dyn + c.n_fix;
    struct Item { const char* n; const void* p; size_t b; };
    const Item items[] = {
        {"x", e->x, (size_t)c.rows * c.hidden * 2},
        {"logits", e->logits, (size_t)c.rows * c.codec_channels * c.codec_vocab * 4},
        {"pred", e->pred, (size_t)c.rows / 2 * c.codec_channels * 8},
        {"all_mask", e->all_mask, (size_t)c.layers * c.rows * E * 4},
        {"all_topk", e->all_topk, (size_t)c.layers * c.rows * 8},
        {"router_logits", e->r_logits, (size_t)c.rows * E * 2},
        {"k_cache", e->k_cache, (size_t)c.layers * c.rows * c.kv_heads * c.Lmax * c.head_dim * 2},
        {"v_cache", e->v_cache, (size_t)c.layers * c.rows * c.kv_heads * c.Lmax * c.head_dim * 2},
        {"counts", e->counts, (size_t)c.n_real * 4},
        {"xg", e->xg, (size_t)(c.ep_size > 1 ? c.ep_size : 0) * c.rows * c.hidden * 2},
        {"ep_words", e->ep_words, 8},
        {"q_pos0", e->q_pos0, (size_t)c.rows * 4},
        {"kv_start", e->kv_start, (size_t)c.rows * 4},
        {"valid_count", e->valid_count, (size_t)c.rows * 4},
    };
    for (const Item& it : items)
        if (!strcmp(it.n, name)) {
            if (bytes) *bytes = it.b;
            return it.p;
        }
    return nullptr;
}
```

unimoe_audio_amd/csrc/umoe_flat_dev.h:

```cpp
#pragma once
#include "umoe_common.h"
#include "umoe_router_dev.h"

#include <type_traits>

#define FLAT_MAXG UMOE_GROUPS_INLINE
#define FLAT_MAXWG 256
#define FLAT_NP_MIN 4
#define FLAT_NP_MAX 7
#define FLAT_ND_MAX2 6
#define FLAT_ND_MAX1 10
#define FLAT_SLICES 2

struct flat_args {
    const uint16_t* a;
    const uint16_t* norm_w;
    float rms_eps;
    int lda, S, G;
    int pair0[FLAT_MAXG + 1];
    const uint16_t* w_gu[FLAT_MAXG];
    uint16_t* h;
    uint16_t* y;
    uint32_t* flags;
    unsigned long long* dbg;
    int ldh, ldy, kb_gu;
    const uint16_t* w_dn[FLAT_MAXG];
    int h_row[FLAT_MAXG];
    int dn_kb[FLAT_MAXG];
    int dn_a_row[FLAT_MAXG];
    int dn_y_row[FLAT_MAXG];
    int dn_nb[FLAT_MAXG];
    int prod_base[FLAT_MAXG];
    int prod_n[FLAT_MAXG];
    uint32_t gu[FLAT_MAXWG];
    uint32_t dn[FLAT_MAXWG];
};

__device__ __forceinline__ int flat_lds_chunk_off(int QS, int h, int i, int m) {
    return h * QS + (i >> 4) * 256 + (((i & 15) + m) & 15) * 16;
}

__device__ __forceinline__ void flat_wait(uint32_t* flag, uint32_t epoch, uint32_t* err_word, uint32_t code) {
    umoe_gu32* f = reinterpret_cast<umoe_gu32*>(reinterpret_cast<uintptr_t>(flag));
    umoe_gu32* err = reinterpret_cast<umoe_gu32*>(reinterpret_cast<uintptr_t>(err_word));
    const unsigned long long t0 = wall_clock64();
    for (unsigned spins = 0;; ++spins) {
        if ((int32_t)(__hip_atomic_load(f, __ATOMIC_RELAXED, __HIP_MEMORY_SCOPE_AGENT) - epoch) >= 0) break;
        __builtin_amdgcn_s_sleep(1);
        if ((spins & 1023u) == 1023u) {
            if (__hip_atomic_load(err, __ATOMIC_RELAXED, __HIP_MEMORY_SCOPE_AGENT) != 0u) break;
            if (wall_clock64() - t0 > 200000000ull) {
                uint32_t zero = 0u;
                __hip_atomic_compare_exchange_strong(err, &zero, code, __ATOMIC_RELAXED, __ATOMIC_RELAXED, __HIP_MEMORY_SCOPE_AGENT);
                break;
            }
        }
    }
}

#ifdef UMOE_TIMELINE
struct flat_stamps { unsigned long long t[16]; };
#define FSTAMP(k) do { if (A.dbg) st.t[k] = wall_clock64(); } while (0)
#else
struct flat_stamps {};
#define FSTAMP(k) do { } while (0)
#endif

typedef uint32_t flat_u32x4 __attribute__((ext_vector_type(4)));
typedef uint32_t flat_u32x2 __attribute__((ext_vector_type(2)));

struct flat_f8 {
    const int8_t* e_gu[FLAT_MAXG];
    const int8_t* e_dn[FLAT_MAXG];
};
typedef __bf16 flat_bf16x2 __attribute__((ext_vector_type(2)));
__device__ __forceinline__ float flat_f8_scale(int e) { return __uint_as_float((uint32_t)(e + 127) << 23); }
__device__ __forceinline__ bf16x8_t flat_f8_frag(uint32_t lo, uint32_t hi, float sc) {
    const flat_bf16x2 a = __builtin_amdgcn_cvt_scalef32_pk_bf16_fp8(lo, sc, false), b = __builtin_amdgcn_cvt_scalef32_pk_bf16_fp8(lo, sc, true);
    const flat_bf16x2 c = __builtin_amdgcn_cvt_scalef32_pk_bf16_fp8(hi, sc, false), d = __builtin_amdgcn_cvt_scalef32_pk_bf16_fp8(hi, sc, true);
    return bf16x8_t{a[0], a[1], b[0], b[1], c[0], c[1], d[0], d[1]};
}

__device__ __forceinline__ uint32_t flat_epoch(const umoe_rider_pub& pub) {
    asm volatile("" ::: "memory");
    return __builtin_nontemporal_load(pub.step) * (uint32_t)pub.layers + (uint32_t)pub.layer + 1u;
}

template <int NP, bool PUBLISH = true, bool F8 = false>
__device__ __forceinline__ void flat_gateup(const flat_args& A, const umoe_rider_pub& pub, const int fp0, const unsigned b, char* smem, flat_stamps& st,
                                            const int tid_in, const flat_f8* F = nullptr) {
    constexpr int NT = 2 * NP, WV = 8, KB = 64;
    const int tid = tid_in, lane = tid & 63;
    const int wave = __builtin_amdgcn_readfirstlane(tid >> 6);
    constexpr int QS = (KB * 16 + 255) & ~255, RS = QS * 4;
    const int i0 = __builtin_amdgcn_readfirstlane((KB * wave) / WV), i1 = __builtin_amdgcn_readfirstlane((KB * (wave + 1)) / WV);
    constexpr int CS = F8 ? 2 : 1;
    const int c0 = i0 / CS, c1 = i1 / CS;
    int g0 = 0;
#pragma unroll
    for (int i = 1; i < FLAT_MAXG; ++i) g0 += (fp0 >= A.pair0[i] && i < A.G) ? 1 : 0;
    const int p0 = A.pair0[g0], cut = A.pair0[g0 + 1];
    const uint16_t *wg0 = A.w_gu[g0], *wg1 = A.w_gu[g0 + 1 < FLAT_MAXG ? g0 + 1 : g0];
    const int g1 = min(g0 + 1, A.G - 1);
    f32x4_t acc[NT];
    const flat_u32x4* wp[NT];
    [[maybe_unused]] const int8_t* ep[F8 ? NT : 1];
    [[maybe_unused]] int ev[F8 ? NT : 1];
#pragma unroll
    for (int t = 0; t < NT; ++t) {
        acc[t] = f32x4_t{0.f, 0.f, 0.f, 0.f};
        const int pp = fp0 + (t >> 1);
        const bool second = pp >= cut;
        const int lp = pp - (second ? cut : p0);
        if constexpr (F8) {
            const int blk = 2 * lp + (t & 1);
            wp[t] = reinterpret_cast<const flat_u32x4*>(second ? wg1 : wg0) + ((size_t)blk * (KB / 2)) * 64 + lane;
            ep[t] = (second ? F->e_gu[g0 + 1 < FLAT_MAXG ? g0 + 1 : g0] : F->e_gu[g0]) + blk * 16 + (lane & 15);
        } else {
            wp[t] = reinterpret_cast<const flat_u32x4*>(second ? wg1 : wg0) + ((size_t)(2 * lp + (t & 1)) * KB) * 64 + lane;
        }
    }
    auto load_scales = [&]() {
        if constexpr (F8) {
#pragma unroll
            for (int t = 0; t < NT; ++t) ev[t] = *ep[t];
        }
    };
    flat_u32x4 w0[NT], w1[NT];
    auto load_chunk = [&](flat_u32x4 (&dst)[NT], int ii) {
        const int ic = min(ii, c1 - 1);
#pragma unroll
        for (int t = 0; t < NT; ++t) dst[t] = __builtin_nontemporal_load(wp[t] + (size_t)ic * 64);
    };
    const int count = A.S;
    {
        constexpr int TPR = WV * 4;
        const int m = tid / TPR, sub = tid % TPR;
        const bool valid = m < count;
        const uint16_t* src = A.a + (size_t)(valid ? m : 0) * A.lda;
        char* dst = smem + m * RS;
        char* nw_lds = smem + 16 * RS;
        auto norm_stage = [&](uint4 (&buf)[8], const uint4 nw1) {
            st16(nw_lds + (tid & (4 * KB - 1)) * 16, nw1);
            float q4[4];
#pragma unroll
            for (int hq = 0; hq < 4; ++hq) {
                float c2[2];
#pragma unroll
                for (int k2 = 0; k2 < 2; ++k2) {
                    float f[8];
                    unpack8(buf[hq * 2 + k2], f);
                    float cs = 0.f;
#pragma unroll
                    for (int j = 0; j < 8; ++j) cs += f[j] * f[j];
                    c2[k2] = cs;
                }
                float v = c2[0] + c2[1];
#pragma unroll
                for (int o = 16; o >= 1; o >>= 1) v += __shfl_xor(v, o, 64);
                q4[hq] = v;
            }
            const float ss = ((q4[0] + q4[1]) + q4[2]) + q4[3];
            const float rs = rsqrtf(ss / (float)(KB * 32) + A.rms_eps);
            __syncthreads();
            FSTAMP(2);
#pragma unroll
            for (int n = 0; n < 8; ++n) asm volatile("" : "+v"(buf[n].x), "+v"(buf[n].y), "+v"(buf[n].z), "+v"(buf[n].w));
#pragma unroll
            for (int n = 0; n < 8; ++n) {
                const int h = n >> 1, i = sub + TPR * (n & 1);
                float f[8], w[8];
                unpack8(buf[n], f);
                unpack8(*reinterpret_cast<const uint4*>(nw_lds + (h * KB + i) * 16), w);
#pragma unroll
                for (int j = 0; j < 8; ++j) f[j] = w[j] * rbf(f[j] * rs);
                if (valid) st16(dst + flat_lds_chunk_off(QS, h, i, m), pack8(f));
            }
        };
        uint4 buf[8];
#pragma unroll
        for (int n = 0; n < 8; ++n) buf[n] = ld16(src + ((n >> 1) * KB + sub + TPR * (n & 1)) * 8);
        const uint4 nw1 = ld16(A.norm_w + (tid & (4 * KB - 1)) * 8);
        __builtin_amdgcn_sched_barrier(0);
        load_chunk(w0, c0);
        load_scales();
        __builtin_amdgcn_sched_barrier(0);
        FSTAMP(1);
        norm_stage(buf, nw1);
    }
    __syncthreads();
    FSTAMP(3);
    const int h = lane >> 4, mm = lane & 15;
    const char* bbase = smem + mm * RS;
    auto compute_chunk = [&](const flat_u32x4 (&src)[NT], int ii) {
        if (ii < c1) {
            if constexpr (F8) {
#pragma unroll
                for (int k = 0; k < 2; ++k) {
                    const uint4 bv = *reinterpret_cast<const uint4*>(bbase + flat_lds_chunk_off(QS, h, 2 * ii + k, mm));
                    const bf16x8_t bfrag = __builtin_bit_cast(bf16x8_t, bv);
#pragma unroll
                    for (int t = 0; t < NT; ++t)
                        acc[t] = __builtin_amdgcn_mfma_f32_16x16x32_bf16(flat_f8_frag(src[t][2 * k], src[t][2 * k + 1], flat_f8_scale(ev[t])), bfrag, acc[t], 0, 0, 0);
                }
            } else {
                const uint4 bv = *reinterpret_cast<const uint4*>(bbase + flat_lds_chunk_off(QS, h, ii, mm));
                const bf16x8_t bfrag = __builtin_bit_cast(bf16x8_t, bv);
#pragma unroll
                for (int t = 0; t < NT; ++t) acc[t] = __builtin_amdgcn_mfma_f32_16x16x32_bf16(__builtin_bit_cast(bf16x8_t, src[t]), bfrag, acc[t], 0, 0, 0);
            }
        }
    };
    for (int i = c0; i < c1; i += 2) {
        if (i + 1 < c1) load_chunk(w1, i + 1);
        compute_chunk(w0, i);
        if (i + 2 < c1) load_chunk(w0, i + 2);
        if (i + 1 < c1) compute_chunk(w1, i + 1);
    }
    FSTAMP(4);
    __syncthreads();
    FSTAMP(5);
    f32x4_t* red = reinterpret_cast<f32x4_t*>(smem);
#pragma unroll
    for (int t = 0; t < NT; ++t) red[(wave * NT + t) * 64 + lane] = acc[t];
    __syncthreads();
    auto reduced = [&](int t) -> f32x4_t {
        f32x4_t s = red[t * 64 + lane];
#pragma unroll
        for (int w = 1; w < WV; ++w) {
            const f32x4_t v = red[(w * NT + t) * 64 + lane];
            s[0] += v[0]; s[1] += v[1]; s[2] += v[2]; s[3] += v[3];
        }
        return s;
    };
    const auto orsrc = __builtin_amdgcn_make_buffer_rsrc(A.h, 0, 0x7fffffff, 0x00020000);
    for (int q = wave; q < NP; q += WV) {
        const int pp = fp0 + q;
        const int grp = pp >= cut ? g1 : g0;
        const int col = (pp - A.pair0[grp]) * 16 + 4 * h;
        const long orow = (long)A.h_row[grp] + mm;
        const f32x4_t ga = reduced(2 * q), ua = reduced(2 * q + 1);
        uint16_t yv[4];
#pragma unroll
        for (int j = 0; j < 4; ++j) {
            const float gt = rbf(ga[j]);
            const float up = rbf(ua[j]);
            const float si = rbf(gt / (1.0f + expf(-gt)));
            yv[j] = f2bf(si * up);
        }
        const flat_u32x2 v2 = {(uint32_t)yv[0] | ((uint32_t)yv[1] << 16), (uint32_t)yv[2] | ((uint32_t)yv[3] << 16)};
        if (mm < count) __builtin_amdgcn_raw_buffer_store_b64(v2, orsrc, (int)((orow * A.ldh + col) * 2), 0, 16);
    }
    if constexpr (PUBLISH) {
        asm volatile("s_waitcnt vmcnt(0)" ::: "memory");
        __syncthreads();
        if (tid == 0)
            __hip_atomic_store(reinterpret_cast<umoe_gu32*>(reinterpret_cast<uintptr_t>(A.flags + b)), flat_epoch(pub), __ATOMIC_RELAXED, __HIP_MEMORY_SCOPE_AGENT);
    }
    FSTAMP(6);
}

template <int ND, int U, bool F8 = false>
__device__ __forceinline__ void flat_down(const flat_args& A, const umoe_rider_pub& pub, const int grp, const int nb0, char* smem, flat_stamps& st,
                                          const int sb, const int tid_in, const flat_f8* F = nullptr) {
    constexpr int NT = ND, WV = 8;
    const int tid = tid_in, lane = tid & 63;
    const int wave = __builtin_amdgcn_readfirstlane(tid >> 6);
    const int KB = A.dn_kb[grp];
    const int QS = (KB * 16 + 255) & ~255, RS = QS * 4;
    int i0, i1;
    if (KB % 2 == 0) {
        const int units = KB / 2;
        i0 = 2 * ((units * wave) / WV);
        i1 = 2 * ((units * (wave + 1)) / WV);
    } else {
        i0 = (KB * wave) / WV;
        i1 = (KB * (wave + 1)) / WV;
    }
    i0 = __builtin_amdgcn_readfirstlane(i0);
    i1 = __builtin_amdgcn_readfirstlane(i1);
    f32x4_t acc[NT];
    using FW = std::conditional_t<U == 2, flat_u32x4, flat_u32x2>;
    constexpr int UL = F8 ? 1 : U;
    using WT = std::conditional_t<F8, FW, flat_u32x4>;
    const WT* wp[NT];
    [[maybe_unused]] int ev[F8 ? NT : 1];
#pragma unroll
    for (int t = 0; t < NT; ++t) {
        acc[t] = f32x4_t{0.f, 0.f, 0.f, 0.f};
        if constexpr (F8) {
            const int KB2 = (KB + 1) >> 1;
            wp[t] = reinterpret_cast<const WT*>(reinterpret_cast<const flat_u32x4*>(A.w_dn[grp]) + ((size_t)(nb0 + t) * KB2) * 64 + lane);
        } else {
            wp[t] = reinterpret_cast<const flat_u32x4*>(A.w_dn[grp]) + ((size_t)(nb0 + t) * KB) * 64 + lane;
        }
    }
    WT w0[NT][UL], w1[NT][UL];
    auto load_chunk = [&](WT (&dst)[NT][UL], int ibase) {
        if constexpr (F8) {
            const int ii = min(ibase, i1 - U);
#pragma unroll
            for (int t = 0; t < NT; ++t)
                dst[t][0] = __builtin_nontemporal_load(U == 2 ? wp[t] + (size_t)(ii >> 1) * 64 : wp[t] + (size_t)(ii >> 1) * 128 + (ii & 1));
        } else {
#pragma unroll
            for (int u = 0; u < U; ++u) {
                const int ii = min(ibase + u, i1 - 1);
#pragma unroll
                for (int t = 0; t < NT; ++t) dst[t][u] = __builtin_nontemporal_load(wp[t] + (size_t)ii * 64);
            }
        }
    };
    if (i0 < i1) load_chunk(w0, i0);
    if constexpr (F8) {
        const int8_t* e = F->e_dn[grp] + nb0 * 16 + (lane & 15);
#pragma unroll
        for (int t = 0; t < NT; ++t) ev[t] = e[t * 16];
    }
    const int count = A.S;
    if (tid < A.prod_n[grp]) flat_wait(A.flags + A.prod_base[grp] + tid, flat_epoch(pub), pub.err, 3u);
    __syncthreads();
    FSTAMP(sb);
    {
        constexpr int TPR = WV * 4;
        const int m = tid / TPR, sub = tid % TPR;
        const bool valid = m < count;
        const long arow = (long)A.dn_a_row[grp] + (valid ? m : 0);
        char* dst = smem + m * RS;
        const auto rsrc = __builtin_amdgcn_make_buffer_rsrc(A.h, 0, 0x7fffffff, 0x00020000);
        for (int ib0 = 0; ib0 < KB; ib0 += 4 * TPR) {
            uint4 buf[16];
#pragma unroll
            for (int n = 0; n < 16; ++n) {
                const int h = n >> 2, i = min(ib0 + sub + TPR * (n & 3), KB - 1);
                const flat_u32x4 t4 = __builtin_amdgcn_raw_buffer_load_b128(rsrc, (int)((arow * A.ldh + (h * KB + i) * 8) * 2), 0, 16);
                buf[n] = make_uint4(t4[0], t4[1], t4[2], t4[3]);
            }
            if (ib0 == 0) {
                __builtin_amdgcn_sched_barrier(0);
                if (i0 + U < i1) load_chunk(w1, i0 + U);
                __builtin_amdgcn_sched_barrier(0);
            }
#pragma unroll
            for (int n = 0; n < 16; ++n) {
                const int h = n >> 2, i = ib0 + sub + TPR * (n & 3);
                if (valid && i < KB) st16(dst + flat_lds_chunk_off(QS, h, i, m), buf[n]);
            }
        }
    }
    __syncthreads();
    FSTAMP(sb + 1);
    const int h = lane >> 4, mm = lane & 15;
    const char* bbase = smem + mm * RS;
    auto compute_chunk = [&](const WT (&src)[NT][UL], int ibase) {
#pragma unroll
        for (int u = 0; u < U; ++u) {
            const int ii = ibase + u;
            if (ii < i1) {
                const uint4 bv = *reinterpret_cast<const uint4*>(bbase + flat_lds_chunk_off(QS, h, ii, mm));
                const bf16x8_t bfrag = __builtin_bit_cast(bf16x8_t, bv);
#pragma unroll
                for (int t = 0; t < NT; ++t) {
                    if constexpr (F8)
                        acc[t] = __builtin_amdgcn_mfma_f32_16x16x32_bf16(flat_f8_frag(src[t][0][2 * u], src[t][0][2 * u + 1], flat_f8_scale(ev[t])), bfrag, acc[t], 0, 0, 0);
                    else
                        acc[t] = __builtin_amdgcn_mfma_f32_16x16x32_bf16(__builtin_bit_cast(bf16x8_t, src[t][u]), bfrag, acc[t], 0, 0, 0);
                }
            }
        }
    };
    for (int i = i0; i < i1; i += 2 * U) {
        if (i + U < i1 && i != i0) load_chunk(w1, i + U);
        compute_chunk(w0, i);
        if (i + 2 * U < i1) load_chunk(w0, i + 2 * U);
        if (i + U < i1) compute_chunk(w1, i + U);
    }
    FSTAMP(sb + 2);
    __syncthreads();
    FSTAMP(sb + 3);
    f32x4_t* red = reinterpret_cast<f32x4_t*>(smem);
#pragma unroll
    for (int t = 0; t < NT; ++t) red[(wave * NT + t) * 64 + lane] = acc[t];
    __syncthreads();
    if (mm >= count) return;
    for (int t = wave; t < NT; t += WV) {
        f32x4_t s = red[t * 64 + lane];
#pragma unroll
        for (int w = 1; w < WV; ++w) {
            const f32x4_t v = red[(w * NT + t) * 64 + lane];
            s[0] += v[0]; s[1] += v[1]; s[2] += v[2]; s[3] += v[3];
        }
        const int n = (nb0 + t) * 16 + 4 * h;
        uint16_t yv[4];
#pragma unroll
        for (int j = 0; j < 4; ++j) yv[j] = f2bf(rbf(s[j] + 0.f));
        uint16_t* o = A.y + ((long)A.dn_y_row[grp] + mm) * A.ldy + n;
        *reinterpret_cast<uint2*>(o) = make_uint2((uint32_t)yv[0] | ((uint32_t)yv[1] << 16), (uint32_t)yv[2] | ((uint32_t)yv[3] << 16));
    }
}
```

unimoe_audio_amd/csrc/umoe_moe_flat.hip:

```cpp
#include <stdlib.h>
#include <string.h>

#include <algorithm>
#include <vector>

#include "umoe_common.h"
#include "umoe_router_dev.h"

#include "umoe_flat_dev.h"

#define FLAT_RIDER_LDS 512

template <bool F8>
__device__ __forceinline__ void moe_flat_body(const flat_args& A, const umoe_router_args& ra, const umoe_rider_pub& pub, const int lds_gemm, const flat_f8* F) {
    extern __shared__ __attribute__((aligned(16))) char smem[];
    const unsigned b = blockIdx.x;
    const unsigned eg = A.gu[b], ed = A.dn[b];
    flat_stamps st;
#ifdef UMOE_TIMELINE
    if (A.dbg) {
#pragma unroll
        for (int k = 0; k < 16; ++k) st.t[k] = 0;
        st.t[0] = wall_clock64();
    }
#endif
    const int token = (int)(eg >> 16) - 1;
    if (token >= 0) {
        float* rl = reinterpret_cast<float*>(smem + lds_gemm);
        if (threadIdx.x < 256) {
#ifdef UMOE_TIMELINE
            TL_ENTER(5);
#endif
            if (ra.logits_bf16) router4_body<9, 2, 1, false>(ra, token, threadIdx.x, rl TL_PASS);
            else router4_body<9, 2, 0, false>(ra, token, threadIdx.x, rl TL_PASS);
        } else {
            __syncthreads();
            __syncthreads();
        }
    }
    const int fp0 = (int)(eg & 2047u), np = (int)((eg >> 11) & 7u);
    switch (np) {
        case 4: flat_gateup<4, true, F8>(A, pub, fp0, b, smem, st, (int)threadIdx.x, F); break;
        case 5: flat_gateup<5, true, F8>(A, pub, fp0, b, smem, st, (int)threadIdx.x, F); break;
        case 6: flat_gateup<6, true, F8>(A, pub, fp0, b, smem, st, (int)threadIdx.x, F); break;
        case 7: flat_gateup<7, true, F8>(A, pub, fp0, b, smem, st, (int)threadIdx.x, F); break;
        default: break;
    }
    for (int sl = 0; sl < FLAT_SLICES; ++sl) {
        const unsigned e16 = (ed >> (16 * sl)) & 0xffffu;
        const int nd = (int)(e16 >> 12), grp = (int)(e16 & 15u), nb0 = (int)((e16 >> 4) & 255u);
        if (nd == 0) break;
        __syncthreads();
        if (A.dn_kb[grp] & 1) {
            switch (nd) {
                case 1: flat_down<1, 1, F8>(A, pub, grp, nb0, smem, st, 7 + 4 * sl, (int)threadIdx.x, F); break;
                case 2: flat_down<2, 1, F8>(A, pub, grp, nb0, smem, st, 7 + 4 * sl, (int)threadIdx.x, F); break;
                case 3: flat_down<3, 1, F8>(A, pub, grp, nb0, smem, st, 7 + 4 * sl, (int)threadIdx.x, F); break;
                case 4: flat_down<4, 1, F8>(A, pub, grp, nb0, smem, st, 7 + 4 * sl, (int)threadIdx.x, F); break;
                case 5: flat_down<5, 1, F8>(A, pub, grp, nb0, smem, st, 7 + 4 * sl, (int)threadIdx.x, F); break;
                case 6: flat_down<6, 1, F8>(A, pub, grp, nb0, smem, st, 7 + 4 * sl, (int)threadIdx.x, F); break;
                case 7: flat_down<7, 1, F8>(A, pub, grp, nb0, smem, st, 7 + 4 * sl, (int)threadIdx.x, F); break;
                case 8: flat_down<8, 1, F8>(A, pub, grp, nb0, smem, st, 7 + 4 * sl, (int)threadIdx.x, F); break;
                case 9: flat_down<9, 1, F8>(A, pub, grp, nb0, smem, st, 7 + 4 * sl, (int)threadIdx.x, F); break;
                default: flat_down<10, 1, F8>(A, pub, grp, nb0, smem, st, 7 + 4 * sl, (int)threadIdx.x, F); break;
            }
        } else {
            switch (nd) {
                case 1: flat_down<1, 2, F8>(A, pub, grp, nb0, smem, st, 7 + 4 * sl, (int)threadIdx.x, F); break;
                case 2: flat_down<2, 2, F8>(A, pub, grp, nb0, smem, st, 7 + 4 * sl, (int)threadIdx.x, F); break;
                case 3: flat_down<3, 2, F8>(A, pub, grp, nb0, smem, st, 7 + 4 * sl, (int)threadIdx.x, F); break;
                case 4: flat_down<4, 2, F8>(A, pub, grp, nb0, smem, st, 7 + 4 * sl, (int)threadIdx.x, F); break;
                case 5: flat_down<5, 2, F8>(A, pub, grp, nb0, smem, st, 7 + 4 * sl, (int)threadIdx.x, F); break;
                default: flat_down<6, 2, F8>(A, pub, grp, nb0, smem, st, 7 + 4 * sl, (int)threadIdx.x, F); break;
            }
        }
    }
#ifdef UMOE_TIMELINE
    if (A.dbg && threadIdx.x == 0) {
        st.t[15] = wall_clock64();
#pragma unroll
        for (int k = 0; k < 16; ++k) A.dbg[(size_t)b * 16 + k] = st.t[k];
    }
#endif
}

__global__ __launch_bounds__(512, 1) void moe_flat_kernel(const flat_args A, const umoe_router_args ra, const umoe_rider_pub pub, const int lds_gemm) {
    moe_flat_body<false>(A, ra, pub, lds_gemm, nullptr);
}

__global__ __launch_bounds__(512, 1) void moe_flat_fp8_kernel(const flat_args A, const umoe_router_args ra, const umoe_rider_pub pub, const int lds_gemm,
                                                              const flat_f8 F) {
    moe_flat_body<true>(A, ra, pub, lds_gemm, &F);
}

struct FlatPlan {
    bool ok = false;
    int n_wg = 0;
    uint32_t gu[FLAT_MAXWG], dn[FLAT_MAXWG];
    int prod_base[FLAT_MAXG], prod_n[FLAT_MAXG];
    double makespan = 0, mean = 0;
};

struct FlatShape {
    int G, S, n_wg, kb_gu;
    int pairs[FLAT_MAXG], dn_nb[FLAT_MAXG], dn_kb[FLAT_MAXG], dn_src[FLAT_MAXG];
    int rider_less, heavy_at;
    double rider, stage, flagc, pair_scale;
    int fp8;
    bool operator==(const FlatShape& o) const { return memcmp(this, &o, sizeof(*this)) == 0; }
};

struct FlatSlices { int n[FLAT_MAXWG]; int grp[FLAT_MAXWG][FLAT_SLICES], nb0[FLAT_MAXWG][FLAT_SLICES], nd[FLAT_MAXWG][FLAT_SLICES]; };
static bool flat_assign(const FlatShape& sh, const double* avail, const double* seam, const int* ex, double T, FlatSlices& o) {
    const int n = sh.n_wg;
    double fre[FLAT_MAXWG];
    for (int j = 0; j < n; ++j) { fre[j] = avail[j]; o.n[j] = 0; }
    for (int q = 0; q < sh.G; ++q) {
        const int i = ex[q];
        const double se = seam[sh.dn_src[i]], cb = sh.fp8 ? 0.5 * sh.dn_kb[i] : (double)sh.dn_kb[i];
        const int ndmax = (sh.dn_kb[i] & 1) ? FLAT_ND_MAX1 : FLAT_ND_MAX2;
        int left = sh.dn_nb[i], next = 0;
        while (left > 0) {
            int bj = -1;
            double bs = 1e30;
            for (int j = 0; j < n; ++j) {
                if (o.n[j] >= FLAT_SLICES) continue;
                const double st = std::max(fre[j], se);
                if (st < bs && st + sh.stage + cb <= T) { bs = st; bj = j; }
            }
            if (bj < 0) return false;
            int nd = (int)((T - bs - sh.stage) / cb);
            nd = std::min(std::min(nd, ndmax), left);
            const int k = o.n[bj]++;
            o.grp[bj][k] = i; o.nb0[bj][k] = next; o.nd[bj][k] = nd;
            fre[bj] = bs + sh.stage + nd * cb;
            next += nd; left -= nd;
        }
    }
    return true;
}

static void flat_plan(const FlatShape& sh, FlatPlan& out) {
    out.ok = false;
    out.n_wg = sh.n_wg;
    const int n = sh.n_wg, G = sh.G, S = sh.S;
    if (n < 1 || n > FLAT_MAXWG || G > FLAT_MAXG || S > n) return;
    int P = 0, pair0[FLAT_MAXG + 1];
    for (int i = 0; i < G; ++i) { pair0[i] = P; P += sh.pairs[i]; }
    pair0[G] = P;
    if (P >= 2048) return;
    const double cp = sh.fp8 ? (double)sh.kb_gu : 2.0 * sh.kb_gu;
    double total = P * cp + S * sh.rider + n * sh.stage;
    int kb_big = 0;
    for (int i = 0; i < G; ++i) { total += (sh.fp8 ? 0.5 : 1.0) * sh.dn_nb[i] * sh.dn_kb[i]; kb_big = std::max(kb_big, sh.dn_kb[i]); }
    FlatPlan best;
    double best_T = 1e30;
    std::vector<int> np(n), fp0(n);
    std::vector<double> avail(n);
    FlatSlices sl;
    for (int rider_less = 1; rider_less >= 0; --rider_less) {
        if (sh.rider_less >= 0 && rider_less != sh.rider_less) continue;
        if (best.ok) break;
        const int adj = rider_less ? S : 0;
        const int base = (P + adj) / n;
        const int extra = P + adj - base * n;
        const int np_max = extra ? base + 1 : base, np_min = rider_less ? base - 1 : base;
        if (np_max > FLAT_NP_MAX || np_min < FLAT_NP_MIN || extra > n - S) continue;
        std::vector<int> cand;
        cand.push_back(S);
        cand.push_back(n - extra);
        for (int g = 1; g < G; ++g) {
            const int rp = S * (base - rider_less);
            if (pair0[g] >= rp) {
                const int h0 = S + (pair0[g] - rp + base - 1) / base;
                cand.push_back(h0);
                cand.push_back(h0 - extra);
                cand.push_back(h0 - extra - 1);
                cand.push_back(h0 + 1);
            }
        }
        for (int h0 : cand) {
            if (h0 < S || h0 + extra > n) continue;
            if (sh.heavy_at >= 0 && h0 != std::min(std::max(sh.heavy_at, S), n - extra)) continue;
            for (int j = 0; j < n; ++j) np[j] = (j < S) ? base - rider_less : ((j >= h0 && j < h0 + extra) ? base + 1 : base);
            int acc = 0;
            for (int j = 0; j < n; ++j) { fp0[j] = acc; acc += np[j]; }
            if (acc != P) break;
            for (int j = 0; j < n; ++j) avail[j] = (j < S ? sh.rider : 0.0) + base * cp + (np[j] - base) * cp * sh.pair_scale;
            double seam[FLAT_MAXG];
            int pb[FLAT_MAXG], pn[FLAT_MAXG], ex[FLAT_MAXG];
            bool fits = true;
            for (int g = 0; g < G; ++g) {
                int lo = -1, hi = -1;
                double sm = 0;
                for (int j = 0; j < n; ++j)
                    if (fp0[j] < pair0[g + 1] && fp0[j] + np[j] > pair0[g]) {
                        if (lo < 0) lo = j;
                        hi = j;
                        sm = std::max(sm, avail[j]);
                    }
                if (lo < 0 || hi - lo + 1 > 64) fits = false;
                pb[g] = lo; pn[g] = hi - lo + 1;
                seam[g] = sm + sh.flagc;
            }
            if (!fits) continue;
            for (int i = 0; i < G; ++i) ex[i] = i;
            std::stable_sort(ex, ex + G, [&](int x, int y) {
                const bool bx = sh.dn_kb[x] == kb_big, by = sh.dn_kb[y] == kb_big;
                if (bx != by) return bx;
                return seam[sh.dn_src[x]] < seam[sh.dn_src[y]];
            });
            double lo = total / n - 1.0, hi = std::min(best_T, 3.0 * total / n + 4096.0);
            if (!flat_assign(sh, avail.data(), seam, ex, hi, sl)) continue;
            for (int it = 0; it < 24 && hi - lo > 0.5; ++it) {
                const double mid = 0.5 * (lo + hi);
                if (flat_assign(sh, avail.data(), seam, ex, mid, sl)) hi = mid;
                else lo = mid;
            }
            if (hi >= best_T) continue;
            flat_assign(sh, avail.data(), seam, ex, hi, sl);
            best_T = hi;
            best.ok = true;
            best.n_wg = n;
            for (int j = 0; j < n; ++j) {
                best.gu[j] = (uint32_t)fp0[j] | ((uint32_t)np[j] << 11) | (j < S ? (uint32_t)(j + 1) << 16 : 0u);
                uint32_t d = 0;
                for (int k = 0; k < sl.n[j]; ++k) d |= ((uint32_t)sl.grp[j][k] | ((uint32_t)sl.nb0[j][k] << 4) | ((uint32_t)sl.nd[j][k] << 12)) << (16 * k);
                best.dn[j] = d;
            }
            for (int i = 0; i < G; ++i) { best.prod_base[i] = pb[sh.dn_src[i]]; best.prod_n[i] = pn[sh.dn_src[i]]; }
            best.makespan = hi;
            best.mean = total / n;
        }
    }
    if (best.ok) out = best;
}

extern "C" int umoe_moe_flat_plan_probe(int n_wg, int S, int D, int I_dyn, int I_sh, int n_real, int n_fix, double* out, int out_len);
static unsigned long long* g_flat_dbg = nullptr;
extern "C" int umoe_moe_flat_stamps(unsigned long long* host_out) {
    if (!host_out) {
        if (!g_flat_dbg && hipMalloc(&g_flat_dbg, sizeof(unsigned long long) * 16 * FLAT_MAXWG) != hipSuccess) return -2;
        return hipMemset(g_flat_dbg, 0, sizeof(unsigned long long) * 16 * FLAT_MAXWG) == hipSuccess ? 0 : -2;
    }
    if (!g_flat_dbg) return -1;
    return hipMemcpy(host_out, g_flat_dbg, sizeof(unsigned long long) * 16 * FLAT_MAXWG, hipMemcpyDeviceToHost) == hipSuccess ? 0 : -2;
}
static double flat_env(const char* name, double dflt) {
    const char* v = getenv(name);
    return v ? atof(v) : dflt;
}
static void flat_knobs(FlatShape& sh) {
    sh.rider = flat_env("UMOE_FLAT_RIDER_KIB", 110.0);
    sh.stage = flat_env("UMOE_FLAT_STAGE_KIB", 40.0);
    sh.flagc = flat_env("UMOE_FLAT_FLAG_KIB", 0.0);
    sh.pair_scale = flat_env("UMOE_FLAT_PAIR_SCALE", 0.3);
    sh.rider_less = (int)flat_env("UMOE_FLAT_RIDER_LESS", -1.0);
    sh.heavy_at = (int)flat_env("UMOE_FLAT_HEAVY_AT", -1.0);
}

static int moe_flat_launch(const umoe_gemm_args* gu, const umoe_gemm_args* dn, uint32_t* flags, int flag_words, int n_wg, hipStream_t s,
                           const flat_f8* f8) {
    UMOE_REQUIRE(gu && dn && flags, "umoe_moe_flat: null argument");
    const int G = gu->num_groups;
    if (!(gu->fused_router && gu->rider_pub && gu->groups_host && dn->groups_host && G == dn->num_groups && G <= FLAT_MAXG && gu->prologue == UMOE_PRO_PLAIN &&
          gu->epilogue == UMOE_EPI_SWIGLU && dn->prologue == UMOE_PRO_PLAIN && dn->epilogue == UMOE_EPI_BF16 && gu->ksplit <= 1 && dn->ksplit <= 1 &&
          gu->max_rows <= 16 && dn->max_rows <= 16 && dn->a == gu->out && dn->lda == gu->ldo && !dn->fused_router && gu->max_k % 32 == 0 &&
          dn->max_k % 32 == 0 && (gu->lda & 7) == 0 && (gu->ldo & 7) == 0 && (dn->ldo & 3) == 0 && n_wg >= 1 && n_wg <= FLAT_MAXWG && n_wg <= flag_words))
        return 1;
    const umoe_router_args* r = gu->fused_router;
    if (!(r->S >= 1 && r->S <= 16 && r->n_dyn == 9 && r->n_fix == 2 && r->D == 2048 && r->x && r->gate_w && r->expert_mask && !r->logits_in &&
          !r->norm_only && r->norm_w && !r->gumbel && !r->x_noise && !r->attn_mask))
        return 1;
    FlatShape sh;
    memset(&sh, 0, sizeof(sh));
    sh.G = G; sh.S = r->S; sh.n_wg = n_wg; sh.kb_gu = gu->groups_host[0].k / 32;
    for (int i = 0; i < G; ++i) {
        const umoe_group_t& a = gu->groups_host[i];
        const umoe_group_t& b = dn->groups_host[i];
        if (a.rows || a.count || a.row_off || a.a_row_base || a.a_col_off || a.static_count != r->S || a.bias || (a.n_blocks & 1) || a.k != gu->groups_host[0].k ||
            a.k != r->D || b.rows || b.count || b.row_off || b.a_col_off || b.static_count != r->S || b.bias || b.k % 32 || b.n_blocks * 16 != dn->n_valid ||
            b.n_blocks > 255 || a.n_blocks / 2 < 2 * FLAT_NP_MAX)
            return 1;
        sh.pairs[i] = a.n_blocks / 2;
        sh.dn_nb[i] = b.n_blocks;
        sh.dn_kb[i] = b.k / 32;
        int j = -1;
        for (int t = 0; t < G; ++t)
            if (gu->groups_host[t].out_row_base == b.a_row_base) j = t;
        if (j < 0 || gu->groups_host[j].n_blocks * 8 != b.k) return 1;
        sh.dn_src[i] = j;
    }
    flat_knobs(sh);
    sh.fp8 = f8 ? 1 : 0;
    static FlatShape cached_shapes[2];
    static FlatPlan cached_plans[2];
    static bool haves[2] = {false, false};
    FlatShape& cached_shape = cached_shapes[sh.fp8];
    FlatPlan& cached_plan = cached_plans[sh.fp8];
    bool& have = haves[sh.fp8];
    if (!have || !(cached_shape == sh)) {
        flat_plan(sh, cached_plan);
        cached_shape = sh;
        have = true;
        if (getenv("UMOE_FLAT_DEBUG")) {
            fprintf(stderr, "umoe_moe_flat: plan ok=%d n_wg=%d makespan %.0f KiB mean %.0f KiB\n", (int)cached_plan.ok, n_wg, cached_plan.makespan, cached_plan.mean);
            if (cached_plan.ok && atoi(getenv("UMOE_FLAT_DEBUG")) > 1)
                for (int j = 0; j < n_wg; ++j)
                    fprintf(stderr, "  wg %3d: pairs %4d +%d | down group %2d blocks %3d +%d | group %2d blocks %3d +%d\n", j, cached_plan.gu[j] & 2047,
                            (cached_plan.gu[j] >> 11) & 7, cached_plan.dn[j] & 15, (cached_plan.dn[j] >> 4) & 255, (cached_plan.dn[j] >> 12) & 15,
                            (cached_plan.dn[j] >> 16) & 15, (cached_plan.dn[j] >> 20) & 255, cached_plan.dn[j] >> 28);
        }
    }
    const FlatPlan& pl = cached_plan;
    if (!pl.ok) return 1;
    flat_args A;
    memset(&A, 0, sizeof(A));
    A.a = r->x; A.norm_w = r->norm_w; A.rms_eps = r->rms_eps; A.h = reinterpret_cast<uint16_t*>(gu->out); A.y = reinterpret_cast<uint16_t*>(dn->out); A.flags = flags;
    A.dbg = g_flat_dbg;
    A.lda = r->D; A.ldh = gu->ldo; A.ldy = dn->ldo; A.S = r->S; A.G = G; A.kb_gu = sh.kb_gu;
    int P = 0, kb_dn_max = 0;
    for (int i = 0; i < G; ++i) {
        A.w_gu[i] = gu->groups_host[i].w; A.w_dn[i] = dn->groups_host[i].w;
        A.pair0[i] = P; P += sh.pairs[i];
        A.h_row[i] = gu->groups_host[i].out_row_base;
        A.dn_kb[i] = sh.dn_kb[i]; A.dn_a_row[i] = dn->groups_host[i].a_row_base; A.dn_y_row[i] = dn->groups_host[i].out_row_base; A.dn_nb[i] = sh.dn_nb[i];
        A.prod_base[i] = pl.prod_base[i]; A.prod_n[i] = pl.prod_n[i];
        kb_dn_max = std::max(kb_dn_max, sh.dn_kb[i]);
    }
    for (int i = G; i <= FLAT_MAXG; ++i) A.pair0[i] = P;
    memcpy(A.gu, pl.gu, sizeof(uint32_t) * n_wg);
    memcpy(A.dn, pl.dn, sizeof(uint32_t) * n_wg);
    const umoe_rider_pub pub = *reinterpret_cast<const umoe_rider_pub*>(gu->rider_pub);
    UMOE_REQUIRE(pub.flags && pub.step && pub.err, "umoe_moe_flat: rider_pub needs flags / step / err");
    auto stage_bytes = [](int kb) { return (size_t)16 * 4 * (size_t)((kb * 16 + 255) & ~255); };
    size_t lds = std::max(stage_bytes(sh.kb_gu), stage_bytes(kb_dn_max));
    lds = std::max(lds, (size_t)8 * 2 * FLAT_NP_MAX * 1024);
    lds = std::max(lds, (size_t)8 * FLAT_ND_MAX1 * 1024);
    if (lds + FLAT_RIDER_LDS > 160 * 1024) return 1;
    static size_t configured[2] = {0, 0};
    const void* kfn = f8 ? reinterpret_cast<const void*>(&moe_flat_fp8_kernel) : reinterpret_cast<const void*>(&moe_flat_kernel);
    if (lds + FLAT_RIDER_LDS > configured[sh.fp8]) {
        UMOE_HIP(hipFuncSetAttribute(kfn, hipFuncAttributeMaxDynamicSharedMemorySize, (int)(lds + FLAT_RIDER_LDS)));
        configured[sh.fp8] = lds + FLAT_RIDER_LDS;
    }
    umoe_router_args rr = *r;
    rr.h_out = nullptr;
    if (f8) moe_flat_fp8_kernel<<<dim3((unsigned)n_wg), 512, lds + FLAT_RIDER_LDS, s>>>(A, rr, pub, (int)lds, *f8);
    else moe_flat_kernel<<<dim3((unsigned)n_wg), 512, lds + FLAT_RIDER_LDS, s>>>(A, rr, pub, (int)lds);
    UMOE_LAUNCH_CHECK();
    return 0;
}

int umoe_moe_flat(const umoe_gemm_args* gu, const umoe_gemm_args* dn, uint32_t* flags, int flag_words, int n_wg, hipStream_t s) {
    return moe_flat_launch(gu, dn, flags, flag_words, n_wg, s, nullptr);
}

int umoe_moe_flat_fp8(const umoe_gemm_args* gu, const umoe_gemm_args* dn, const int8_t* const* e_gu, const int8_t* const* e_dn, uint32_t* flags,
                      int flag_words, int n_wg, hipStream_t s) {
    UMOE_REQUIRE(e_gu && e_dn && gu && dn && gu->num_groups <= FLAT_MAXG, "umoe_moe_flat_fp8: bad argument");
    flat_f8 F;
    memset(&F, 0, sizeof(F));
    for (int i = 0; i < gu->num_groups; ++i) {
        UMOE_REQUIRE(e_gu[i] && e_dn[i], "umoe_moe_flat_fp8: group %d has no exponents", i);
        F.e_gu[i] = e_gu[i]; F.e_dn[i] = e_dn[i];
    }
    return moe_flat_launch(gu, dn, flags, flag_words, n_wg, s, &F);
}

bool umoe_moe_flat_feasible(int n_wg, int S, int D, int I_dyn, int I_sh, int n_real, int n_fix) {
    static int key[7] = {-1, -1, -1, -1, -1, -1, -1};
    static bool ans = false;
    const int k[7] = {n_wg, S, D, I_dyn, I_sh, n_real, n_fix};
    if (memcmp(k, key, sizeof(k)) == 0) return ans;
    std::vector<double> out(3 + 9 * (size_t)std::max(n_wg, 1));
    const int rc = (n_wg >= 1 && n_wg <= FLAT_MAXWG && I_dyn % 32 == 0 && I_sh % 32 == 0 && I_dyn / 16 >= 2 * FLAT_NP_MAX && I_sh / 16 >= 2 * FLAT_NP_MAX && D / 16 <= 255)
                       ? umoe_moe_flat_plan_probe(n_wg, S, D, I_dyn, I_sh, n_real, n_fix, out.data(), (int)out.size()) : -1;
    memcpy(key, k, sizeof(k));
    ans = rc == 0 && out[0] != 0.0;
    return ans;
}

static int flat_plan_probe(int n_wg, int S, int D, int I_dyn, int I_sh, int n_real, int n_fix, double* out, int out_len, int fp8) {
    FlatShape sh;
    memset(&sh, 0, sizeof(sh));
    sh.G = n_real + n_fix; sh.S = S; sh.n_wg = n_wg; sh.kb_gu = D / 32;
    if (sh.G > FLAT_MAXG || out_len < 3 + 9 * n_wg || n_wg < 1 || n_wg > FLAT_MAXWG) return -1;
    for (int i = 0; i < sh.G; ++i) {
        const bool shd = i < n_fix;
        sh.pairs[i] = (shd ? I_sh : I_dyn) / 16; sh.dn_nb[i] = D / 16; sh.dn_kb[i] = (shd ? I_sh : I_dyn) / 32; sh.dn_src[i] = i;
    }
    flat_knobs(sh);
    sh.fp8 = fp8;
    FlatPlan pl;
    flat_plan(sh, pl);
    out[0] = pl.ok ? 1.0 : 0.0; out[1] = pl.makespan; out[2] = pl.mean;
    if (pl.ok)
        for (int j = 0; j < n_wg; ++j) {
            double* o = out + 3 + 9 * j;
            o[0] = pl.gu[j] & 2047; o[1] = (pl.gu[j] >> 11) & 7; o[2] = pl.gu[j] >> 16;
            for (int k = 0; k < 2; ++k) {
                const uint32_t e16 = (pl.dn[j] >> (16 * k)) & 0xffffu;
                o[3 + 3 * k] = e16 & 15; o[4 + 3 * k] = (e16 >> 4) & 255; o[5 + 3 * k] = e16 >> 12;
            }
        }
    return 0;
}

extern "C" int umoe_moe_flat_plan_probe(int n_wg, int S, int D, int I_dyn, int I_sh, int n_real, int n_fix, double* out, int out_len) {
    return flat_plan_probe(n_wg, S, D, I_dyn, I_sh, n_real, n_fix, out, out_len, 0);
}

extern "C" int umoe_moe_flat_plan_fp8_probe(int n_wg, int S, int D, int I_dyn, int I_sh, int n_real, int n_fix, double* out, int out_len) {
    return flat_plan_probe(n_wg, S, D, I_dyn, I_sh, n_real, n_fix, out, out_len, 1);
}

bool umoe_moe_flat_fp8_feasible(int n_wg, int S, int D, int I_dyn, int I_sh, int n_real, int n_fix) {
    static int key[7] = {-1, -1, -1, -1, -1, -1, -1};
    static bool ans = false;
    const int k[7] = {n_wg, S, D, I_dyn, I_sh, n_real, n_fix};
    if (memcmp(k, key, sizeof(k)) == 0) return ans;
    bool ok = false;
    if (n_wg >= 1 && n_wg <= FLAT_MAXWG && I_dyn % 32 == 0 && I_sh % 32 == 0 && I_dyn / 16 >= 2 * FLAT_NP_MAX && I_sh / 16 >= 2 * FLAT_NP_MAX && D / 16 <= 255) {
        std::vector<double> out(3 + 9 * (size_t)n_wg);
        ok = flat_plan_probe(n_wg, S, D, I_dyn, I_sh, n_real, n_fix, out.data(), (int)out.size(), 1) == 0 && out[0] != 0.0;
    }
    memcpy(key, k, sizeof(k));
    ans = ok;
    return ans;
}

__global__ void fp8_convert_probe_kernel(const uint8_t* q, const int8_t* e, int N, int K, uint16_t* out) {
    const int per_row = K / 8;
    const int i = blockIdx.x * blockDim.x + threadIdx.x;
    if (i >= N * per_row) return;
    const int r = i / per_row;
    const flat_u32x2 v = *reinterpret_cast<const flat_u32x2*>(q + (size_t)i * 8);
    const bf16x8_t f = flat_f8_frag(v[0], v[1], flat_f8_scale(e[r]));
    *reinterpret_cast<uint4*>(out + (size_t)i * 8) = __builtin_bit_cast(uint4, f);
}

extern "C" int umoe_fp8_convert_probe(const uint8_t* q, const int8_t* e, int N, int K, uint16_t* out, umoe_stream_t stream) {
    UMOE_REQUIRE(q && e && out && N > 0 && K > 0 && K % 8 == 0, "umoe_fp8_convert_probe: bad argument (N %d K %d)", N, K);
    const int n = N * (K / 8);
    fp8_convert_probe_kernel<<<dim3((unsigned)((n + 255) / 256)), 256, 0, (hipStream_t)stream>>>(q, e, N, K, out);
    UMOE_LAUNCH_CHECK();
    return 0;
}
```

unimoe_audio_amd/model.py:

```python
from __future__ import annotations

import ctypes as C
from dataclasses import dataclass
from typing import Dict, List, NamedTuple, Optional, Tuple

import torch
import torch.nn as nn

from . import _lib as L
from . import ops, quant
from . import row_params as RP
from .codec_utils import DecoderOutput
from .config import UniMoEAudioConfig
from .dcmoe import UniMoEAudioSparseMoeBlock


@dataclass
class BaseModelOutputWithPast:
    last_hidden_state: torch.Tensor = None
    past_key_values: Optional[tuple] = None
    hidden_states: Optional[tuple] = None
    attentions: Optional[tuple] = None
    all_router_logits: Optional[tuple] = None
    all_router_top_k: Optional[tuple] = None
    all_router_weight: Optional[tuple] = None
    all_router_expert_mask: Optional[tuple] = None
    all_aux_loss: Optional[tuple] = None


@dataclass
class MoEQwen2_5VLCausalLMOutputWithPast:
    loss: Optional[torch.Tensor] = None
    logits: Optional[torch.Tensor] = None
    codec_logits: Optional[torch.Tensor] = None
    past_key_values: Optional[tuple] = None
    hidden_states: Optional[torch.Tensor] = None
    attentions: Optional[tuple] = None
    rope_deltas: Optional[torch.Tensor] = None
    all_router_logits: Optional[tuple] = None
    all_router_top_k: Optional[tuple] = None
    all_router_expert_mask: Optional[tuple] = None
    all_router_weight: Optional[tuple] = None
    aux_balance_loss: Optional[torch.Tensor] = None


class Qwen2RMSNorm(nn.Module):
    def __init__(self, hidden_size, eps=1e-6):
        super().__init__()
        self.weight = nn.Parameter(torch.ones(hidden_size))
        self.variance_epsilon = eps


class Qwen2_5_VLAttention(nn.Module):

    def __init__(self, config):
        super().__init__()
        D, H, KV, hd = config.hidden_size, config.num_attention_heads, config.num_key_value_heads, config.head_dim
        self.q_proj = nn.Linear(D, H * hd, bias=True)
        self.k_proj = nn.Linear(D, KV * hd, bias=True)
        self.v_proj = nn.Linear(D, KV * hd, bias=True)
        self.o_proj = nn.Linear(H * hd, D, bias=False)


class Qwen2_5_VLMoEDecoderLayer(nn.Module):

    def __init__(self, config, layer_idx: int):
        super().__init__()
        self.self_attn = Qwen2_5_VLAttention(config)
        self.mlp = UniMoEAudioSparseMoeBlock(config)
        self.input_layernorm = Qwen2RMSNorm(config.hidden_size, config.rms_norm_eps)
        self.post_attention_layernorm = Qwen2RMSNorm(config.hidden_size, config.rms_norm_eps)


class Qwen2_5_VLMoETextModel(nn.Module):

    def __init__(self, config):
        super().__init__()
        self.embed_tokens = nn.Embedding(config.vocab_size, config.hidden_size)
        self.layers = nn.ModuleList([Qwen2_5_VLMoEDecoderLayer(config, i) for i in range(config.num_hidden_layers)])
        self.norm = Qwen2RMSNorm(config.hidden_size, config.rms_norm_eps)


class UniAudioRVQQwen2_5VLMoEForConditionalGeneration(nn.Module):
    def __init__(self, config: UniMoEAudioConfig, with_lm_head: bool = False):
        super().__init__()
        self.config = config
        self.language_model = Qwen2_5_VLMoETextModel(config)
        self.num_channels = config.codec_channels
        self.codec_vocab_size = config.codec_vocab_size
        self.codec_embed_tokens = nn.ModuleList(
            [nn.Embedding(self.codec_vocab_size, config.hidden_size) for _ in range(self.num_channels)])
        self.codec_placeholder_value = config.codec_placeholder_value
        self.codec_head = nn.Linear(config.hidden_size, self.num_channels * self.codec_vocab_size, bias=False)
# ... 150 lines not shown
                stats["logits"].append(out[1]); stats["top_k"].append(out[2])
            stats["expert_mask"].append(out[3]); stats["weight"].append(out[4]); stats["aux"].append(out[5])
        return BaseModelOutputWithPast(last_hidden_state=h.view(B, T, D), all_router_logits=tuple(stats["logits"]) or None,
                                       all_router_top_k=tuple(stats["top_k"]) or None,
                                       all_router_expert_mask=tuple(stats["expert_mask"]), all_router_weight=tuple(stats["weight"]),
                                       all_aux_loss=tuple(stats["aux"]))

    @property
    def cur_aux_weight(self):
        cfg = self.config
        steps = max(1, cfg.l_aux_weight_decay_steps)
        ts = getattr(self, "training_steps", 0)
        if ts >= steps:
            return cfg.min_l_aux_weight
        return cfg.l_aux_weight - (cfg.l_aux_weight - cfg.min_l_aux_weight) / steps * ts

    @torch.no_grad()
    def forward(self, input_ids=None, codec_input_ids=None, attention_mask=None, position_ids=None, inputs_embeds=None,
                labels=None, codec_labels=None, aux_balance_weight=None, padding_token_mask=None,
                output_router_logits_and_topk=None, **unused):
        dev = self.device
        if inputs_embeds is None:
            inputs_embeds = self.calculate_input_embedding(input_ids.to(dev), None if codec_input_ids is None else codec_input_ids.to(dev))
        if attention_mask is not None:
            attention_mask = attention_mask.to(dev)
            if aux_balance_weight is not None:
                aux_balance_weight = attention_mask * aux_balance_weight.to(dev)
            if padding_token_mask is None:
                padding_token_mask = attention_mask.bool()
        out = self.text_forward(inputs_embeds, attention_mask, position_ids, padding_token_mask, aux_balance_weight,
                                bool(output_router_logits_and_topk))
        B, T, D = out.last_hidden_state.shape
        C, V = self.num_channels, self.codec_vocab_size
        hs = out.last_hidden_state.reshape(B * T, D).contiguous()
        codec_logits = (ops.tlinear(hs, self.codec_head.weight.data, out_f32=True) if B * T >= 64
                        else ops.linear(hs, self.packed()["head"], C * V, out_f32=True)).view(B, T, C, V)
        loss = aux_mean = None
        if labels is not None and codec_labels is not None:
            aux_mean = torch.stack([a.float() for a in out.all_aux_loss]).mean()
            sl = codec_logits[:, :-1].reshape(B * (T - 1), C, V).contiguous()
            lab = codec_labels.to(dev)[:, 1:].reshape(B * (T - 1), C).contiguous()
            codec_loss, _, _ = ops.codec_ce(sl, lab)
            loss = codec_loss + self.cur_aux_weight * aux_mean
            self.training_steps = getattr(self, "training_steps", 0) + 1
        return MoEQwen2_5VLCausalLMOutputWithPast(loss=loss, logits=None, codec_logits=codec_logits,
                                                  hidden_states=out.last_hidden_state, all_router_logits=out.all_router_logits,
                                                  all_router_top_k=out.all_router_top_k,
                                                  all_router_expert_mask=out.all_router_expert_mask,
                                                  all_router_weight=out.all_router_weight, aux_balance_loss=aux_mean)

    def _run_with_labels(self, eng, dec_output, max_tokens, min_tokens, cfg_scale, eos_mul, debug_guidance_step, use_graph):
        cfg = self.config
        B, C, V, eos = eng.batch, cfg.codec_channels, cfg.codec_vocab_size, cfg.codec_eos_value
        labels = dec_output.labels_prefill.to(self.device)
        step0 = int(eng.state[4 * B].item())
        self.golden_losses = []
        budget = max_tokens - step0
        for i in range(budget):
            dec_step = step0 + i
            lab = labels[:, dec_step + 1] if dec_step + 1 < labels.shape[1] else None
            guided_step = lab is not None and (dec_step < debug_guidance_step or debug_guidance_step == -1)
            if guided_step:
                cur = eng.tokens[:, dec_step + 1]
                eng.tokens[:, dec_step + 1] = torch.where(cur == -1, lab.to(torch.int32), cur)
            eng.step(use_graph)
            if lab is not None:
                lg = eng.copy_buffer("logits", torch.float32, (2 * B, C, V)).view(B, 2, C, V)
                guided = (lg[:, 1] + cfg_scale * (lg[:, 1] - lg[:, 0])) if cfg_scale != 0 else lg[:, 1].clone()
                if min_tokens is None or dec_step >= min_tokens:
                    guided[:, :, eos + 1:] = float("-inf")
                    guided[:, 1:, eos:] = float("-inf")
                else:
                    guided[:, :, eos:] = float("-inf")
                guided[:, 0, eos] *= eos_mul
                gl = golden_loss(guided, lab, eos)
                self.golden_losses.append(None if gl is None else float(gl))
                print(f"golden loss: {gl}")
            if eng.all_done():
                break

    def _pack_key(self):
        return tuple((p.data_ptr(), p._version) for n, p in self.named_parameters() if not n.startswith("visual."))

    def engine(self, batch: int, max_prompt: int, max_tokens: int, attn_splits: int = 8, ep=None,
               expert_weights: Optional[str] = None) -> "DecodeEngine":
        need_L = max_prompt + max_tokens + 8
        e = self._engine
        key = self._pack_key()
        fmt = expert_weights or quant.expert_format(self)
        fp8_wide = fmt in ("fp8", "fp8-only")
        if (e is None or e.batch != batch or e.Lmax < need_L or e.Tmax < max_tokens + 64 or e.pack_key != key or e.ep is not ep
                or e.expert_weights != fmt or e.fp8_wide != fp8_wide):
            if e is not None:
                e.close()
            self._engine = DecodeEngine(self, batch, Lmax=need_L, Tmax=max_tokens + 64, attn_splits=attn_splits, ep=ep, expert_weights=fmt,
                                        fp8_wide=fp8_wide)
        return self._engine

    def quantize_experts_(self, fmt: str = "fp8", keep_bf16: bool = True):
        return quant.quantize_experts_(self, fmt, keep_bf16=keep_bf16)

    @torch.no_grad()
    def generate(self, input_ids, attention_mask, dec_output: DecoderOutput, max_tokens, min_tokens=None,
                 codec_input_ids: Optional[torch.Tensor] = None, pixel_values=None, pixel_values_videos=None,
                 image_grid_thw=None, video_grid_thw=None, second_per_grid_ts=None, cfg_scale: float = 3.0,
                 temperature: float = 1.2, top_p: float = 0.95, cfg_filter_top_k: int = 45,
                 eos_prob_mul_factor: float = 0.8, do_sample: bool = True, debug_guidance_step: int = 0, use_cache=True,
                 seed: int = 0, use_graph: bool = True, poll_every: int = 16, vision_in_generate: bool = False,
                 expert_weights: Optional[str] = None):
        if not use_cache and codec_input_ids is not None:
            raise AssertionError("use_cache=False with a codec prompt: the reference asserts use_cache here (model.py:1092-1093)")
        dev = self.device
        input_ids, attention_mask = input_ids.to(dev), attention_mask.to(dev)
        B = input_ids.shape[0] // 2
        T = input_ids.shape[1]
        per_row = [n for n, v in (("max_tokens", max_tokens), ("min_tokens", min_tokens), ("cfg_scale", cfg_scale), ("temperature", temperature),
                                  ("top_p", top_p), ("cfg_filter_top_k", cfg_filter_top_k), ("eos_prob_mul_factor", eos_prob_mul_factor),
                                  ("do_sample", do_sample), ("seed", seed)) if RP.is_sequence(v)]
        if per_row and getattr(dec_output, "labels_prefill", None) is not None:
            raise L.UmoeError(f"generate: teacher labels (DecoderOutput.labels_prefill) take one setting for the batch, not a sequence ({', '.join(per_row)})")
        top_tokens = RP.largest(max_tokens)
        eng = self.engine(B, T, top_tokens, expert_weights=expert_weights)
        pos3 = deltas = None
        if vision_in_generate and (pixel_values is not None or pixel_values_videos is not None):
            x = self.multimodal_embedding(input_ids, None if codec_input_ids is None else codec_input_ids.to(dev), pixel_values, image_grid_thw,
                                          pixel_values_videos, video_grid_thw)
            pos3, deltas = self.get_rope_index(input_ids, image_grid_thw, video_grid_thw, second_per_grid_ts, attention_mask)
        else:
            x = self.calculate_input_embedding(input_ids, None if codec_input_ids is None else codec_input_ids.to(dev))
        eng.prefill(x.reshape(-1, x.shape[-1]).contiguous(), attention_mask, position_ids=pos3, rope_deltas=deltas)
        eng.start_decode(dec_output.generated_tokens, dec_output.prefill_steps, max_tokens if RP.is_sequence(max_tokens) else int(max_tokens),
                         min_tokens, cfg_scale=cfg_scale, temperature=temperature, top_p=top_p, top_k=cfg_filter_top_k,
                         eos_mul=eos_prob_mul_factor, do_sample=do_sample, seed=seed)
        if getattr(dec_output, "labels_prefill", None) is not None:
            self._run_with_labels(eng, dec_output, int(max_tokens), min_tokens, cfg_scale, eos_prob_mul_factor, int(debug_guidance_step),
                                  use_graph)
        else:
            eng.run(use_graph=use_graph, poll_every=poll_every)
        codes, lengths, tokens = eng.finish()
        dec_output.generated_tokens = tokens
        if codes is None:
            print("Warning: Nothing generated for any sequence in the batch.")
        return codes, lengths


    @torch.no_grad()
    def generate_stream(self, input_ids, attention_mask, dec_output: DecoderOutput, max_tokens, min_tokens=None,
                        codec_input_ids: Optional[torch.Tensor] = None, pixel_values=None, pixel_values_videos=None,
                        image_grid_thw=None, video_grid_thw=None, second_per_grid_ts=None, cfg_scale: float = 3.0,
                        temperature: float = 1.2, top_p: float = 0.95, cfg_filter_top_k: int = 45,
                        eos_prob_mul_factor: float = 0.8, do_sample: bool = True, debug_guidance_step: int = 0, use_cache=True,
                        seed: int = 0, use_graph: bool = True, poll_every: int = 16, vision_in_generate: bool = False,
                        expert_weights: Optional[str] = None, chunk_frames: int = 25):
        if getattr(dec_output, "labels_prefill", None) is not None:
            raise L.UmoeError("generate_stream: teacher labels (DecoderOutput.labels_prefill) run the diagnostic path of generate() only")
        if not use_cache and codec_input_ids is not None:
            raise AssertionError("use_cache=False with a codec prompt: the reference asserts use_cache here (model.py:1092-1093)")
        dev = self.device
        input_ids, attention_mask = input_ids.to(dev), attention_mask.to(dev)
        B = input_ids.shape[0] // 2
        T = input_ids.shape[1]
        eng = self.engine(B, T, RP.largest(max_tokens), expert_weights=expert_weights)
        if (eng.ep is not None and eng.ep.size > 1) or getattr(eng, "sharded", False):
            raise L.UmoeError("generate_stream: expert-parallel decode is not streamed; use generate()")
        pos3 = deltas = None
        if vision_in_generate and (pixel_values is not None or pixel_values_videos is not None):
            x = self.multimodal_embedding(input_ids, None if codec_input_ids is None else codec_input_ids.to(dev), pixel_values, image_grid_thw,
                                          pixel_values_videos, video_grid_thw)
            pos3, deltas = self.get_rope_index(input_ids, image_grid_thw, video_grid_thw, second_per_grid_ts, attention_mask)
        else:
            x = self.calculate_input_embedding(input_ids, None if codec_input_ids is None else codec_input_ids.to(dev))
        eng.prefill(x.reshape(-1, x.shape[-1]).contiguous(), attention_mask, position_ids=pos3, rope_deltas=deltas)
        eng.start_decode(dec_output.generated_tokens, dec_output.prefill_steps, max_tokens if RP.is_sequence(max_tokens) else int(max_tokens),
                         min_tokens, cfg_scale=cfg_scale, temperature=temperature, top_p=top_p, top_k=cfg_filter_top_k,
                         eos_mul=eos_prob_mul_factor, do_sample=do_sample, seed=seed)
        ends = {}
        for upd in eng.run_stream(int(chunk_frames), use_graph=use_graph):
            ends.update({r: f1 for r, _, f1, done in upd.rows if done})
            yield upd
        _, lengths, tokens = eng.finish()
        dec_output.generated_tokens = tokens
        if lengths is not None and [ends.get(b) for b in range(B)] != [int(v) for v in lengths.cpu()]:
            raise AssertionError(f"run_stream ended rows at {ends}, finish() has lengths {lengths.tolist()}")


def golden_loss(guided_BxCxV: torch.Tensor, labels_BxC: torch.Tensor, eos: int) -> Optional[torch.Tensor]:
    lab = labels_BxC.clone().long()
    lab[lab > eos] = -100
    rest = lab[:, 1:]
    rest[rest >= eos] = -100
    total = None
    for c in range(lab.shape[1]):
        if c != 0 and int((lab[:, c] != -100).sum()) == 0:
            continue
        l = torch.nn.functional.cross_entropy(guided_BxCxV[:, c].float(), lab[:, c], ignore_index=-100) * (3 if c == 0 else 1)
        total = l if total is None else total + l
    return total


class StreamUpdate(NamedTuple):
    dec_step: int
    rows: List[Tuple[int, int, int, bool]]


class DecodeEngine:

    def __init__(self, model: UniAudioRVQQwen2_5VLMoEForConditionalGeneration, batch: int, Lmax: int, Tmax: int,
                 attn_splits: int = 8, max_pos: Optional[int] = None, ep=None, ep_connect: bool = True, expert_weights: Optional[str] = None,
                 fp8_wide: bool = False):
        cfg = model.config
        fmt = expert_weights or quant.expert_format(model)
        if fmt not in ("bf16", "fp8", "fp8-only"):
            raise L.UmoeError(f"expert_weights must be 'bf16', 'fp8' or 'fp8-only' (got {fmt!r})")
        if fmt != "fp8-only" and quant.is_released(model):
            raise L.UmoeError(quant._released_msg(f"DecodeEngine(expert_weights={fmt!r})"))
        if fmt in ("fp8", "fp8-only"):
            if ep is not None and ep.size > 1:
                raise L.UmoeError("fp8 expert weights run on the flat expert launch only: not with expert parallel decode")
            quant.check_quantized(model)
        self.expert_weights = fmt
        self.fp8_wide = bool(fp8_wide)
        dev = model.device
        if dev.type != "cuda":
            raise L.UmoeError("DecodeEngine needs the model on a ROCm device; there is no CPU path in the product")
        self.model, self.cfg, self.dev = model, cfg, dev
        self.batch, self.rows, self.Lmax, self.Tmax = batch, 2 * batch, int(Lmax), int(Tmax)
        sec = list(cfg.mrope_section)
        c = L.EngineCfg(hidden=cfg.hidden_size, layers=cfg.num_hidden_layers, heads=cfg.num_attention_heads,
                        kv_heads=cfg.num_key_value_heads, head_dim=cfg.head_dim, n_dyn=cfg.num_dyn,
                        n_real=cfg.mlp_dynamic_expert_num, n_fix=cfg.mlp_fixed_expert_num,
                        inter_dyn=cfg.dynamic_intermediate_size, inter_shared=cfg.shared_intermediate_size,
                        codec_channels=cfg.codec_channels, codec_vocab=cfg.codec_vocab_size, eos=cfg.codec_eos_value,
                        pad=cfg.codec_pad_value, bos=cfg.codec_bos_value, mrope0=sec[0], mrope1=sec[1], mrope2=sec[2],
                        rms_eps=cfg.rms_norm_eps, top_p=float(cfg.mlp_dynamic_top_p), fixed_top_k=int(cfg.mlp_dynamic_top_k),
                        jitter_eps=float(cfg.router_jitter_noise), rows=self.rows, Lmax=self.Lmax, Tmax=self.Tmax,
                        attn_splits=attn_splits, ep_rank=0 if ep is None else ep.rank, ep_size=1 if ep is None else ep.size)
        self.ep = ep
        self.ep_rank, self.ep_size = (0, 1) if ep is None else (ep.rank, ep.size)
        self.pack_key = model._pack_key()
        h = C.c_void_p()
        L.check(L.lib().umoe_engine_create(C.byref(c), C.byref(h)), "umoe_engine_create")
        self.h = h
        self.keep: List[torch.Tensor] = []
        self._pack_weights(max_pos)
        if self.fp8_wide:
            L.check(L.lib().umoe_engine_set_fp8_wide(self.h, 1), "umoe_engine_set_fp8_wide")
        if ep is not None and ep.size > 1 and ep_connect:
            ep.connect(self.h)
        self.tokens = None
        self.state = None
        self.io = None
        self.row_params = None
        self.row_clock = None
        self.reserved_prompt = 0
        self.captured = False

    def _k(self, t):
        self.keep.append(t)
        return t

    def _pack_weights(self, max_pos_override=None):
        m, cfg, lib = self.model, self.cfg, L.lib()
        bf = torch.bfloat16
        for p in m.parameters():
            if p.dtype != bf:
                raise L.UmoeError("engine weights must be bfloat16")
        mpk = m.packed()
        self._k(mpk)
        for li, layer in enumerate(m.language_model.layers):
            lp = mpk["layers"][li]
            qkv_w, qkv_b, o_w, pk = lp["qkv_w"], lp["qkv_b"], lp["o_w"], lp["moe"]
            n_real, n_fix = cfg.mlp_dynamic_expert_num, cfg.mlp_fixed_expert_num
            arr = lambda ts: (C.c_void_p * max(1, len(ts)))(*[t.data_ptr() for t in ts])
            e_loc = n_real // self.ep_size
            ex = layer.mlp.dynamic_real_moe.deepspeed_moe.experts.deepspeed_experts
            sh = layer.mlp.fixed_real_moe
            sharded = self.ep_size > 1 and len(ex) == e_loc
            if not sharded and len(ex) != n_real:
                raise L.UmoeError(f"the model holds {len(ex)} routed experts per layer: expected {n_real} (replicated) or {e_loc} (sharded for ep_size {self.ep_size})")
            self.sharded = sharded
            lo = 0 if sharded else self.ep_rank * e_loc
            only = self.expert_weights == "fp8-only"
            eg = ed = sg = sd = None
            if not only:
                eg, ed = arr(pk["exp_gu"][lo:lo + e_loc]), arr(pk["exp_dn"][lo:lo + e_loc])
                sg, sd = arr(pk["sh_gu"]), arr(pk["sh_dn"])
            rm = [p for mods in (ex, sh) for m_ in mods for p in (m_.gate_proj.weight, m_.up_proj.weight, m_.down_proj.weight)]
            if not all(p.is_contiguous() for p in rm + [layer.self_attn.o_proj.weight]):
                raise L.UmoeError("engine weights must be contiguous")
            if sharded or only:
                reg = reu = red = None
            else:
                reg, reu, red = arr([m_.gate_proj.weight for m_ in ex]), arr([m_.up_proj.weight for m_ in ex]), arr([m_.down_proj.weight for m_ in ex])
            rsg = rsu = rsd = None
            if not only:
                rsg, rsu, rsd = arr([m_.gate_proj.weight for m_ in sh]), arr([m_.up_proj.weight for m_ in sh]), arr([m_.down_proj.weight for m_ in sh])
            w = L.LayerWeights(in_norm=layer.input_layernorm.weight.data_ptr(), qkv_w=qkv_w.data_ptr(), qkv_b=qkv_b.data_ptr(),
                               o_w=o_w.data_ptr(), post_norm=layer.post_attention_layernorm.weight.data_ptr(),
                               gate_w=layer.mlp.gate.weight.data_ptr(), exp_gu=eg, exp_dn=ed, sh_gu=sg, sh_dn=sd,
                               rm_qkv=lp["qkv_rm"].data_ptr(), rm_o=layer.self_attn.o_proj.weight.data_ptr(),
                               rm_exp_gate=reg, rm_exp_up=reu, rm_exp_down=red, rm_sh_gate=rsg, rm_sh_up=rsu, rm_sh_down=rsd)
            L.check(lib.umoe_engine_set_layer(self.h, li, C.byref(w)), "umoe_engine_set_layer")
            if self.expert_weights in ("fp8", "fp8-only"):
                self._set_layer_fp8(li, ex, sh)
        emb, head = mpk["emb"], mpk["head"]
        max_pos = self.Lmax + 4104 if max_pos_override is None else int(max_pos_override)
        self.max_pos = max_pos
        cos, sin = ops.rope_tables(max_pos, cfg.head_dim, cfg.rope_theta, self.dev)
        self._k(cos), self._k(sin)
        delay = (C.c_int32 * cfg.codec_channels)(*cfg.codec_delay_pattern)
        L.check(lib.umoe_engine_set_globals(self.h, m.language_model.norm.weight.data_ptr(), emb.data_ptr(), head.data_ptr(),
                                            cos.data_ptr(), sin.data_ptr(), max_pos, delay), "umoe_engine_set_globals")
        torch.cuda.synchronize()

    def _set_layer_fp8(self, li, ex, sh):
        gu8, gue, dn8, dne = [], [], [], []
        for m_ in list(ex) + list(sh):
            st = m_._fp8
            for k in ("gu", "dn"):
                if st[k][0].device != self.dev:
                    st[k] = (st[k][0].to(self.dev), st[k][1].to(self.dev))
            gu8.append(self._k(st["gu"][0])), gue.append(self._k(st["gu"][1]))
            dn8.append(self._k(st["dn"][0])), dne.append(self._k(st["dn"][1]))
        arr = lambda ts: (C.c_void_p * len(ts))(*[t.data_ptr() for t in ts])
        L.check(L.lib().umoe_engine_set_layer_fp8(self.h, li, arr(gu8), arr(gue), arr(dn8), arr(dne)), "umoe_engine_set_layer_fp8")

    def _stream(self):
        return C.c_void_p(torch.cuda.current_stream().cuda_stream)

    def prefill(self, x: torch.Tensor, attention_mask: torch.Tensor, position_ids: Optional[torch.Tensor] = None,
                rope_deltas: Optional[torch.Tensor] = None, external: bool = False):
        rows, T = attention_mask.shape
        assert rows == self.rows and x.shape == (rows * T, self.cfg.hidden_size) and x.dtype == torch.bfloat16
        valid = attention_mask.to(torch.uint8).cpu().contiguous()
        self.T_prompt = T
        if getattr(self, "sharded", False) or external:
            return self._prefill_sharded(x, attention_mask, valid, position_ids, rope_deltas)
        if position_ids is None:
            L.check(L.lib().umoe_engine_prefill(self.h, x.data_ptr(), valid.data_ptr(), T, self._stream()), "umoe_engine_prefill")
        else:
            assert tuple(position_ids.shape) == (3, rows, T) and rope_deltas is not None
            pos = position_ids.to(torch.int32).cpu().contiguous()
            nxt = (rope_deltas.reshape(rows).to(torch.int64).cpu() + T).to(torch.int32).contiguous()
            need = int(max(int(pos.max()), int(nxt.max()) + self.Lmax - T)) + 2
            if need > self.max_pos:
                raise L.UmoeError(f"rope table of the engine covers {self.max_pos} positions, the prompt needs {need}")
            L.check(L.lib().umoe_engine_prefill_pos(self.h, x.data_ptr(), valid.data_ptr(), T, pos.data_ptr(), nxt.data_ptr(), self._stream()),
                    "umoe_engine_prefill_pos")
        self.captured = False

    def _prefill_sharded(self, x, attention_mask, valid, position_ids, rope_deltas):
        rows, T = attention_mask.shape
        cfg = self.cfg
        KVH, hd, Lmax = cfg.num_key_value_heads, cfg.head_dim, self.Lmax
        per_layer = rows * KVH * Lmax * hd * 2
        pad_k = torch.zeros((rows, KVH, Lmax, hd), dtype=torch.bfloat16, device=self.dev)
        pad_v = torch.zeros_like(pad_k)

        def sink(li, kc, vc):
            pad_k[:, :, :T] = kc
            pad_v[:, :, :T] = vc
            self.write_buffer("k_cache", pad_k, li * per_layer)
            self.write_buffer("v_cache", pad_v, li * per_layer)

        with torch.no_grad():
            self.model.text_forward(x.view(rows, T, cfg.hidden_size), attention_mask.to(self.dev), position_ids=position_ids, kv_sink=sink)
        pos_p = nxt_p = None
        if position_ids is not None:
            assert tuple(position_ids.shape) == (3, rows, T) and rope_deltas is not None
            pos = position_ids.to(torch.int32).cpu().contiguous()
            nxt = (rope_deltas.reshape(rows).to(torch.int64).cpu() + T).to(torch.int32).contiguous()
            pos_p, nxt_p = pos.data_ptr(), nxt.data_ptr()
        L.check(L.lib().umoe_engine_prefill_external(self.h, valid.data_ptr(), T, pos_p, nxt_p, self._stream()), "umoe_engine_prefill_external")
        self.captured = False

    def start_decode(self, prefill_tokens: torch.Tensor, prefill_steps: List[int], max_tokens, min_tokens,
                     cfg_scale, temperature, top_p, top_k, eos_mul, do_sample, seed=0):
        B, Cc = self.batch, self.cfg.codec_channels
        assert prefill_tokens.shape[0] == B and prefill_tokens.shape[2] == Cc
        table = RP.pack_row_params(B, cfg_scale=cfg_scale, temperature=temperature, top_p=top_p, top_k=top_k, eos_mul=eos_mul,
                                   do_sample=do_sample, seed=seed, min_tokens=min_tokens, max_tokens=max_tokens)
        if table is not None:
            r0 = table[0]
            cfg_scale, temperature, top_p, eos_mul = float(r0["cfg_scale"]), float(r0["temperature"]), float(r0["top_p"]), float(r0["eos_mul"])
            top_k, do_sample, min_tokens, seed = int(r0["top_k"]), int(r0["do_sample"]), int(r0["min_tokens"]), int(r0["seed"])
            max_tokens = int(table["max_tokens"].max())
        if max_tokens + 2 > self.Tmax or self.T_prompt + max_tokens + 1 > self.Lmax:
            raise L.UmoeError("engine buffers too small for max_tokens")
        tok = torch.full((B, self.Tmax, Cc), -1, dtype=torch.int32, device=self.dev)
        tok[:, : prefill_tokens.shape[1]] = prefill_tokens.to(self.dev, torch.int32)
        step0 = min(prefill_steps) - 1
        st = torch.zeros(4 * B + 8, dtype=torch.int32)
        st[B:2 * B] = -1
        st[2 * B:3 * B] = -1
        st[3 * B:4 * B] = torch.tensor(prefill_steps, dtype=torch.int32)
        st[4 * B + 0], st[4 * B + 1], st[4 * B + 4] = step0, max_tokens, step0
# ... 289 lines not shown
```

Baseline: 2699 audio-tokens/s.

## Add lossless 12-bit packed bf16 expert weight format for flat MoE decode

Adds a WP12 packing for expert gate/up and down weights. Each bf16 keeps its low byte plus a 4-bit code of sign and exponent offset within a per-block 8-exponent window, and up to 32 out-of-window values per block are stored as exception records that are patched in on-device. The flat MoE kernel decodes these 12-bit fragments into bf16 MFMA operands with byte permutes, which cuts the HBM weight traffic in the memory-bound decode MoE by about a quarter. In exchange it adds ALU and readlane work for the decode and exception patching, and layers whose blocks exceed the exception cap fall back to the bf16 path. It is enabled by default for bf16 single-GPU engines with 16 rows or fewer.

```diff
diff --git a/include/umoe.h b/include/umoe.h
--- a/include/umoe.h
+++ b/include/umoe.h
@@ -472,6 +472,8 @@
 int umoe_engine_set_layer_fp8(umoe_engine* e, int layer, const uint8_t* const* gu8, const int8_t* const* gu_e, const uint8_t* const* dn8,
                               const int8_t* const* dn_e);
 int umoe_engine_set_fp8_wide(umoe_engine* e, int on);
+int umoe_engine_set_layer_w12(umoe_engine* e, int layer, const uint8_t* const* gu12, const uint32_t* const* gu_m, const uint8_t* const* dn12,
+                              const uint32_t* const* dn_m);
 int umoe_fp8_convert_probe(const uint8_t* q, const int8_t* e, int N, int K, uint16_t* out, umoe_stream_t stream);
 int umoe_engine_set_globals(umoe_engine* e, const uint16_t* final_norm, const uint16_t* codec_emb,
                             const uint16_t* codec_head_w, const uint16_t* cos_tab, const uint16_t* sin_tab, int max_pos,
diff --git a/unimoe_audio_amd/_lib.py b/unimoe_audio_amd/_lib.py
--- a/unimoe_audio_amd/_lib.py
+++ b/unimoe_audio_amd/_lib.py
@@ -150,6 +150,7 @@
     "umoe_dac_conv1d_win", "umoe_dac_conv_transpose1d_win", "umoe_rvq_from_delayed", "umoe_delay_step_rows",
     "umoe_delay_step_clock", "umoe_engine_reserve", "umoe_engine_admit", "umoe_engine_admit_external", "umoe_gemm_wide", "umoe_pack_rows",
     "umoe_gemm_wide_fp8", "umoe_engine_set_fp8_wide", "umoe_tiled_gemm_wp8",
+    "umoe_engine_set_layer_w12",
 ]
 
 EP_PEER, EP_LOOPBACK, EP_RCCL = 0, 1, 2
@@ -276,6 +277,9 @@
         if not hasattr(L, "umoe_tiled_gemm_wp8"):
             raise UmoeError(f"{_SO} predates this package (no umoe_tiled_gemm_wp8): rebuild it (`make -C unimoe_audio_amd/csrc`)")
         L.umoe_tiled_gemm_wp8.argtypes = [C.POINTER(TGemmArgs), C.POINTER(vp), C.POINTER(vp), vp]
+        if not hasattr(L, "umoe_engine_set_layer_w12"):
+            raise UmoeError(f"{_SO} predates this package (no umoe_engine_set_layer_w12): rebuild it (`make -C unimoe_audio_amd/csrc`)")
+        L.umoe_engine_set_layer_w12.argtypes = [vp, i32, C.POINTER(vp), C.POINTER(vp), C.POINTER(vp), C.POINTER(vp)]
         L.umoe_rvq_from_codes.argtypes = [vp, vp, vp, vp, i32, i32, i32, i32, i32, vp, vp]
         L.umoe_rvq_nearest.argtypes = [vp, vp, vp, vp, vp, vp, i32, i32, i32, i32, i32, vp, vp, vp]
         L.umoe_codec_ce_fwd.argtypes = [vp, vp, i32, i32, i32, vp, vp, vp, vp, vp, vp]
diff --git a/unimoe_audio_amd/csrc/umoe_common.h b/unimoe_audio_amd/csrc/umoe_common.h
--- a/unimoe_audio_amd/csrc/umoe_common.h
+++ b/unimoe_audio_amd/csrc/umoe_common.h
@@ -207,6 +207,8 @@
 int umoe_moe_flat_fp8(const umoe_gemm_args* gu, const umoe_gemm_args* dn, const int8_t* const* e_gu, const int8_t* const* e_dn, uint32_t* flags,
                       int flag_words, int n_wg, hipStream_t s);
 bool umoe_moe_flat_fp8_feasible(int n_wg, int S, int D, int I_dyn, int I_sh, int n_real, int n_fix);
+int umoe_moe_flat_w12(const umoe_gemm_args* gu, const umoe_gemm_args* dn, const uint32_t* const* m_gu, const uint32_t* const* m_dn, uint32_t* flags,
+                      int flag_words, int n_wg, hipStream_t s);
 
 struct umoe_rider2;
 int umoe_gemm_riders(const umoe_gemm_args* a, int kind, const umoe_rider2* r2, const umoe_rider_pub* pub, hipStream_t s);
diff --git a/unimoe_audio_amd/csrc/umoe_engine.hip b/unimoe_audio_amd/csrc/umoe_engine.hip
--- a/unimoe_audio_amd/csrc/umoe_engine.hip
+++ b/unimoe_audio_amd/csrc/umoe_engine.hip
@@ -20,6 +20,9 @@
     std::vector<const uint16_t*> f8_gu, f8_dn;
     std::vector<const int8_t*> f8e_gu, f8e_dn;
     bool has_f8 = false;
+    std::vector<const uint16_t*> w12_gu, w12_dn;
+    std::vector<const uint32_t*> w12m_gu, w12m_dn;
+    bool has_w12 = false;
 };
 
 struct Carver {
@@ -82,6 +85,7 @@
     int expert_launch = 0;
     bool fp8 = false;
     int prefill_fp8 = 0;
+    int expert_w12 = 0;
     int expert_fp8 = 0;
     bool fp8_wide = false;
     int n_cu = 0;
@@ -423,6 +427,26 @@
     return 0;
 }
 
+extern "C" int umoe_engine_set_layer_w12(umoe_engine* e, int layer, const uint8_t* const* gu12, const uint32_t* const* gu_m, const uint8_t* const* dn12,
+                                         const uint32_t* const* dn_m) {
+    UMOE_REQUIRE(e && gu12 && gu_m && dn12 && dn_m && layer >= 0 && layer < e->c.layers, "umoe_engine_set_layer_w12: bad argument (layer %d)", layer);
+    UMOE_REQUIRE(e->c.ep_size == 1, "umoe_engine_set_layer_w12: WP12 expert weights run on the flat expert launch only, not expert parallel (ep_size %d)",
+                 e->c.ep_size);
+    LayerDev& L = e->layers[layer];
+    UMOE_REQUIRE(L.set && L.exp_bf16 && !L.has_f8, "umoe_engine_set_layer_w12: umoe_engine_set_layer(%d) with the WP16 packs first (and no fp8 weights)", layer);
+    const int G = e->c.n_real + e->c.n_fix;
+    for (int i = 0; i < G; ++i)
+        UMOE_REQUIRE(gu12[i] && gu_m[i] && dn12[i] && dn_m[i], "umoe_engine_set_layer_w12: layer %d group %d: null pointer", layer, i);
+    L.w12_gu.assign(G, nullptr); L.w12_dn.assign(G, nullptr);
+    for (int i = 0; i < G; ++i) {
+        L.w12_gu[i] = reinterpret_cast<const uint16_t*>(gu12[i]);
+        L.w12_dn[i] = reinterpret_cast<const uint16_t*>(dn12[i]);
+    }
+    L.w12m_gu.assign(gu_m, gu_m + G); L.w12m_dn.assign(dn_m, dn_m + G);
+    L.has_w12 = true;
+    return 0;
+}
+
 extern "C" int umoe_engine_set_fp8_wide(umoe_engine* e, int on) {
     UMOE_REQUIRE(e, "umoe_engine_set_fp8_wide: null engine");
     e->fp8_wide = on != 0;
@@ -765,6 +789,10 @@
     MOE_WIDE,
 };
 
+static bool flat_w12_on() {
+    const char* v = getenv("UMOE_FLAT_W12");
+    return !v || atoi(v) != 0;
+}
 static bool flat_moe_on() {
     const char* v = getenv("UMOE_FLAT_MOE");
     return !v || atoi(v) != 0;
@@ -1021,6 +1049,7 @@
     dn.max_k = Imax;
     dn.a = e->hbuf; dn.lda = Imax; dn.out = e->ybuf; dn.ldo = D; dn.n_valid = D;
     dn.prologue = UMOE_PRO_PLAIN; dn.epilogue = UMOE_EPI_BF16; dn.nt = dense ? 6 : 0;
+    e->expert_w12 = 0;
     switch (form) {
         case MOE_TILED:
             if ((rc = umoe_router_dispatch_fwd(&ra, e->counts, e->offsets, e->slot_token, e->slot_of, s))) return rc;
@@ -1039,6 +1068,7 @@
             gu.rider_pub = &rpub;
             gu.groups_host = e->h_gu_pub.data() + (size_t)l * G;
             const int n_wg = flat_wgs(e);
+            bool w12 = false;
             if (e->fp8) {
                 UMOE_REQUIRE(L.has_f8 && G <= UMOE_MAXE, "umoe_engine: fp8 expert weights: layer %d has none (umoe_engine_set_layer_fp8)", l);
                 umoe_group_t g8u[UMOE_MAXE], g8d[UMOE_MAXE];
@@ -1053,12 +1083,28 @@
                 gu8.groups_host = g8u; dn8.groups_host = g8d;
                 rc = umoe_moe_flat_fp8(&gu8, &dn8, e8u, e8d, e->ep_words + 64, 512 - 64, n_wg, s);
             } else {
-                rc = umoe_moe_flat(&gu, &dn, e->ep_words + 64, 512 - 64, n_wg, s);
+                rc = 1;
+                if (L.has_w12 && G <= UMOE_MAXE && flat_w12_on()) {
+                    umoe_group_t g12u[UMOE_MAXE], g12d[UMOE_MAXE];
+                    const uint32_t* m12u[UMOE_MAXE];
+                    const uint32_t* m12d[UMOE_MAXE];
+                    for (int i = 0; i < G; ++i) {
+                        const int x = i < c.n_fix ? c.n_real + i : i - c.n_fix;
+                        g12u[i] = gu.groups_host[i]; g12u[i].w = L.w12_gu[x]; m12u[i] = L.w12m_gu[x];
+                        g12d[i] = dn.groups_host[i]; g12d[i].w = L.w12_dn[i]; m12d[i] = L.w12m_dn[i];
+                    }
+                    umoe_gemm_args gu12 = gu, dn12 = dn;
+                    gu12.groups_host = g12u; dn12.groups_host = g12d;
+                    rc = umoe_moe_flat_w12(&gu12, &dn12, m12u, m12d, e->ep_words + 64, 512 - 64, n_wg, s);
+                    w12 = rc == 0;
+                }
+                if (rc == 1) rc = umoe_moe_flat(&gu, &dn, e->ep_words + 64, 512 - 64, n_wg, s);
             }
             UMOE_REQUIRE(rc != 1, "umoe_engine: the %sflat expert launch has no schedule for this shape on %d workgroups (layer %d)", e->fp8 ? "fp8 " : "", n_wg, l);
             if (rc) return rc;
             e->expert_launch = 2;
             e->expert_fp8 = e->fp8 ? 1 : 0;
+            e->expert_w12 = w12 ? 1 : 0;
             PROF(K_GATEUP);
             break;
         }
@@ -1534,6 +1580,7 @@
     if (!strcmp(key, "expert_launch")) return e->expert_launch;
     if (!strcmp(key, "row_tiles")) return e->expert_launch == 4 ? e->row_tiles : 1;
     if (!strcmp(key, "expert_fp8")) return e->expert_fp8;
+    if (!strcmp(key, "expert_w12")) return e->expert_w12;
     if (!strcmp(key, "prefill_fp8")) return e->prefill_fp8;
     if (!strcmp(key, "expert_bf16_resident")) return fp8_only(e) ? 0 : 1;
     if (!strcmp(key, "n_cu")) return e->n_cu;
diff --git a/unimoe_audio_amd/csrc/umoe_flat_dev.h b/unimoe_audio_amd/csrc/umoe_flat_dev.h
--- a/unimoe_audio_amd/csrc/umoe_flat_dev.h
+++ b/unimoe_audio_amd/csrc/umoe_flat_dev.h
@@ -81,20 +81,51 @@
     return bf16x8_t{a[0], a[1], b[0], b[1], c[0], c[1], d[0], d[1]};
 }
 
+#define FLAT_W12_META 40
+struct flat_w12 {
+    const uint32_t* m_gu[FLAT_MAXG];
+    const uint32_t* m_dn[FLAT_MAXG];
+};
+__device__ __forceinline__ flat_u32x4 flat_w12_frag(uint32_t l0, uint32_t l1, uint32_t c, uint32_t wb4) {
+    const uint32_t hl = (((c & 0x07070707u) + wb4) | ((c & 0x08080808u) << 4));
+    const uint32_t hh = ((((c >> 4) & 0x07070707u) + wb4) | (c & 0x80808080u));
+    return flat_u32x4{__builtin_amdgcn_perm(hl, l0, 0x05010400u), __builtin_amdgcn_perm(hh, l0, 0x05030402u),
+                      __builtin_amdgcn_perm(hl, l1, 0x07010600u), __builtin_amdgcn_perm(hh, l1, 0x07030602u)};
+}
+__device__ __forceinline__ uint32_t flat_w12_cursor(uint32_t m, int i0, int lane) {
+    const uint32_t cur = (uint32_t)__builtin_popcountll(__ballot((int)(m >> 25) < i0 && lane <= 32));
+    return cur << 8 | (uint32_t)__builtin_amdgcn_readlane(m, cur) >> 25;
+}
+__device__ __forceinline__ uint32_t flat_w12_base4(uint32_t m) { return ((uint32_t)__builtin_amdgcn_readlane(m, FLAT_W12_META - 1) & 0xffu) * 0x01010101u; }
+__device__ __forceinline__ void flat_w12_patch(flat_u32x4& op, uint32_t m, uint32_t& st, uint32_t ii, int lane) {
+    uint32_t cur = st >> 8, nx;
+    do {
+        const uint32_t en = (uint32_t)__builtin_amdgcn_readlane(m, cur);
+        const uint32_t sh = ((en >> 16) & 1u) * 16u, d = (en >> 17) & 3u;
+        const bool mine = (uint32_t)lane == ((en >> 19) & 63u);
+#pragma unroll
+        for (int q = 0; q < 4; ++q) op[q] = (mine && d == (uint32_t)q) ? ((op[q] & ~(0xffffu << sh)) | ((en & 0xffffu) << sh)) : op[q];
+        ++cur;
+        nx = (uint32_t)__builtin_amdgcn_readlane(m, cur) >> 25;
+    } while (nx == ii);
+    st = cur << 8 | nx;
+}
+
 __device__ __forceinline__ uint32_t flat_epoch(const umoe_rider_pub& pub) {
     asm volatile("" ::: "memory");
     return __builtin_nontemporal_load(pub.step) * (uint32_t)pub.layers + (uint32_t)pub.layer + 1u;
 }
 
-template <int NP, bool PUBLISH = true, bool F8 = false>
+template <int NP, bool PUBLISH = true, bool F8 = false, bool W12 = false>
 __device__ __forceinline__ void flat_gateup(const flat_args& A, const umoe_rider_pub& pub, const int fp0, const unsigned b, char* smem, flat_stamps& st,
-                                            const int tid_in, const flat_f8* F = nullptr) {
+                                            const int tid_in, const flat_f8* F = nullptr, const flat_w12* Wm = nullptr) {
+    static_assert(!(F8 && W12), "one weight format");
     constexpr int NT = 2 * NP, WV = 8, KB = 64;
     const int tid = tid_in, lane = tid & 63;
     const int wave = __builtin_amdgcn_readfirstlane(tid >> 6);
     constexpr int QS = (KB * 16 + 255) & ~255, RS = QS * 4;
     const int i0 = __builtin_amdgcn_readfirstlane((KB * wave) / WV), i1 = __builtin_amdgcn_readfirstlane((KB * (wave + 1)) / WV);
-    constexpr int CS = F8 ? 2 : 1;
+    constexpr int CS = (F8 || W12) ? 2 : 1;
     const int c0 = i0 / CS, c1 = i1 / CS;
     int g0 = 0;
 #pragma unroll
@@ -106,13 +137,21 @@
     const flat_u32x4* wp[NT];
     [[maybe_unused]] const int8_t* ep[F8 ? NT : 1];
     [[maybe_unused]] int ev[F8 ? NT : 1];
+    [[maybe_unused]] const flat_u32x2* cp[W12 ? NT : 1];
+    [[maybe_unused]] const uint32_t* mp[W12 ? NT : 1];
 #pragma unroll
     for (int t = 0; t < NT; ++t) {
         acc[t] = f32x4_t{0.f, 0.f, 0.f, 0.f};
         const int pp = fp0 + (t >> 1);
         const bool second = pp >= cut;
         const int lp = pp - (second ? cut : p0);
-        if constexpr (F8) {
+        if constexpr (W12) {
+            const int blk = 2 * lp + (t & 1);
+            const char* base = reinterpret_cast<const char*>(second ? wg1 : wg0) + (size_t)blk * (KB * 768);
+            wp[t] = reinterpret_cast<const flat_u32x4*>(base) + lane;
+            cp[t] = reinterpret_cast<const flat_u32x2*>(base + KB * 512) + lane;
+            mp[t] = (second ? Wm->m_gu[g0 + 1 < FLAT_MAXG ? g0 + 1 : g0] : Wm->m_gu[g0]) + blk * FLAT_W12_META + min(lane, FLAT_W12_META - 1);
+        } else if constexpr (F8) {
             const int blk = 2 * lp + (t & 1);
             wp[t] = reinterpret_cast<const flat_u32x4*>(second ? wg1 : wg0) + ((size_t)blk * (KB / 2)) * 64 + lane;
             ep[t] = (second ? F->e_gu[g0 + 1 < FLAT_MAXG ? g0 + 1 : g0] : F->e_gu[g0]) + blk * 16 + (lane & 15);
@@ -124,6 +163,14 @@
         if constexpr (F8) {
 #pragma unroll
             for (int t = 0; t < NT; ++t) ev[t] = *ep[t];
+        }
+    };
+    [[maybe_unused]] flat_u32x2 wc[W12 ? NT : 1];
+    [[maybe_unused]] uint32_t mt[W12 ? NT : 1];
+    auto w12_load_tile = [&](flat_u32x4 (&dst)[NT], int t, int ic) {
+        if constexpr (W12) {
+            dst[t] = __builtin_nontemporal_load(wp[t] + (size_t)ic * 64);
+            wc[t] = __builtin_nontemporal_load(cp[t] + (size_t)ic * 64);
         }
     };
     flat_u32x4 w0[NT], w1[NT];
@@ -182,8 +229,15 @@
         for (int n = 0; n < 8; ++n) buf[n] = ld16(src + ((n >> 1) * KB + sub + TPR * (n & 1)) * 8);
         const uint4 nw1 = ld16(A.norm_w + (tid & (4 * KB - 1)) * 8);
         __builtin_amdgcn_sched_barrier(0);
-        load_chunk(w0, c0);
-        load_scales();
+        if constexpr (W12) {
+#pragma unroll
+            for (int t = 0; t < NT; ++t) mt[t] = *mp[t];
+#pragma unroll
+            for (int t = 0; t < NT; ++t) w12_load_tile(w0, t, c0);
+        } else {
+            load_chunk(w0, c0);
+            load_scales();
+        }
         __builtin_amdgcn_sched_barrier(0);
         FSTAMP(1);
         norm_stage(buf, nw1);
@@ -211,11 +265,37 @@
             }
         }
     };
-    for (int i = c0; i < c1; i += 2) {
-        if (i + 1 < c1) load_chunk(w1, i + 1);
-        compute_chunk(w0, i);
-        if (i + 2 < c1) load_chunk(w0, i + 2);
-        if (i + 1 < c1) compute_chunk(w1, i + 1);
+    if constexpr (W12) {
+        uint32_t xs[NT], wb4[NT];
+#pragma unroll
+        for (int t = 0; t < NT; ++t) {
+            xs[t] = flat_w12_cursor(mt[t], i0, lane);
+            wb4[t] = flat_w12_base4(mt[t]);
+        }
+        auto w12_chunk = [&](int ic, auto refill) {
+            const uint4 bv0 = *reinterpret_cast<const uint4*>(bbase + flat_lds_chunk_off(QS, h, 2 * ic, mm));
+            const uint4 bv1 = *reinterpret_cast<const uint4*>(bbase + flat_lds_chunk_off(QS, h, 2 * ic + 1, mm));
+            const bf16x8_t bf0 = __builtin_bit_cast(bf16x8_t, bv0), bf1 = __builtin_bit_cast(bf16x8_t, bv1);
+#pragma unroll
+            for (int t = 0; t < NT; ++t) {
+                flat_u32x4 o0 = flat_w12_frag(w0[t][0], w0[t][1], wc[t][0], wb4[t]);
+                if ((xs[t] & 0xffu) == (uint32_t)(2 * ic)) flat_w12_patch(o0, mt[t], xs[t], (uint32_t)(2 * ic), lane);
+                flat_u32x4 o1 = flat_w12_frag(w0[t][2], w0[t][3], wc[t][1], wb4[t]);
+                if ((xs[t] & 0xffu) == (uint32_t)(2 * ic + 1)) flat_w12_patch(o1, mt[t], xs[t], (uint32_t)(2 * ic + 1), lane);
+                if constexpr (decltype(refill)::value) w12_load_tile(w0, t, ic + 1);
+                acc[t] = __builtin_amdgcn_mfma_f32_16x16x32_bf16(__builtin_bit_cast(bf16x8_t, o0), bf0, acc[t], 0, 0, 0);
+                acc[t] = __builtin_amdgcn_mfma_f32_16x16x32_bf16(__builtin_bit_cast(bf16x8_t, o1), bf1, acc[t], 0, 0, 0);
+            }
+        };
+        for (int ic = c0; ic < c1 - 1; ++ic) w12_chunk(ic, std::true_type{});
+        w12_chunk(c1 - 1, std::false_type{});
+    } else {
+        for (int i = c0; i < c1; i += 2) {
+            if (i + 1 < c1) load_chunk(w1, i + 1);
+            compute_chunk(w0, i);
+            if (i + 2 < c1) load_chunk(w0, i + 2);
+            if (i + 1 < c1) compute_chunk(w1, i + 1);
+        }
     }
     FSTAMP(4);
     __syncthreads();
@@ -260,9 +340,10 @@
     FSTAMP(6);
 }
 
-template <int ND, int U, bool F8 = false>
+template <int ND, int U, bool F8 = false, bool W12 = false>
 __device__ __forceinline__ void flat_down(const flat_args& A, const umoe_rider_pub& pub, const int grp, const int nb0, char* smem, flat_stamps& st,
-                                          const int sb, const int tid_in, const flat_f8* F = nullptr) {
+                                          const int sb, const int tid_in, const flat_f8* F = nullptr, const flat_w12* Wm = nullptr) {
+    static_assert(!(F8 && W12), "one weight format");
     constexpr int NT = ND, WV = 8;
     const int tid = tid_in, lane = tid & 63;
     const int wave = __builtin_amdgcn_readfirstlane(tid >> 6);
@@ -281,14 +362,22 @@
     i1 = __builtin_amdgcn_readfirstlane(i1);
     f32x4_t acc[NT];
     using FW = std::conditional_t<U == 2, flat_u32x4, flat_u32x2>;
-    constexpr int UL = F8 ? 1 : U;
-    using WT = std::conditional_t<F8, FW, flat_u32x4>;
+    constexpr int UL = (F8 || W12) ? 1 : U;
+    using WT = std::conditional_t<F8 || W12, FW, flat_u32x4>;
+    using CT = std::conditional_t<U == 2, flat_u32x2, uint32_t>;
     const WT* wp[NT];
     [[maybe_unused]] int ev[F8 ? NT : 1];
+    [[maybe_unused]] const CT* cp[W12 ? NT : 1];
+    [[maybe_unused]] uint32_t mt[W12 ? NT : 1];
 #pragma unroll
     for (int t = 0; t < NT; ++t) {
         acc[t] = f32x4_t{0.f, 0.f, 0.f, 0.f};
-        if constexpr (F8) {
+        if constexpr (W12) {
+            const char* base = reinterpret_cast<const char*>(A.w_dn[grp]) + (size_t)(nb0 + t) * ((size_t)KB * 768);
+            wp[t] = reinterpret_cast<const WT*>(base) + lane;
+            cp[t] = reinterpret_cast<const CT*>(base + (size_t)KB * 512) + lane;
+            mt[t] = Wm->m_dn[grp][(nb0 + t) * FLAT_W12_META + min(lane, FLAT_W12_META - 1)];
+        } else if constexpr (F8) {
             const int KB2 = (KB + 1) >> 1;
             wp[t] = reinterpret_cast<const WT*>(reinterpret_cast<const flat_u32x4*>(A.w_dn[grp]) + ((size_t)(nb0 + t) * KB2) * 64 + lane);
         } else {
@@ -296,8 +385,17 @@
         }
     }
     WT w0[NT][UL], w1[NT][UL];
+    [[maybe_unused]] CT c0[W12 ? NT : 1], c1[W12 ? NT : 1];
     auto load_chunk = [&](WT (&dst)[NT][UL], int ibase) {
-        if constexpr (F8) {
+        if constexpr (W12) {
+            const int ii = min(ibase, i1 - U) / U;
+            CT(&cd)[W12 ? NT : 1] = (&dst == &w0) ? c0 : c1;
+#pragma unroll
+            for (int t = 0; t < NT; ++t) {
+                dst[t][0] = __builtin_nontemporal_load(wp[t] + (size_t)ii * 64);
+                cd[t] = __builtin_nontemporal_load(cp[t] + (size_t)ii * 64);
+            }
+        } else if constexpr (F8) {
             const int ii = min(ibase, i1 - U);
 #pragma unroll
             for (int t = 0; t < NT; ++t)
@@ -352,6 +450,14 @@
     FSTAMP(sb + 1);
     const int h = lane >> 4, mm = lane & 15;
     const char* bbase = smem + mm * RS;
+    [[maybe_unused]] uint32_t xs[W12 ? NT : 1], wb4[W12 ? NT : 1];
+    if constexpr (W12) {
+#pragma unroll
+        for (int t = 0; t < NT; ++t) {
+            xs[t] = flat_w12_cursor(mt[t], i0, lane);
+            wb4[t] = flat_w12_base4(mt[t]);
+        }
+    }
     auto compute_chunk = [&](const WT (&src)[NT][UL], int ibase) {
 #pragma unroll
         for (int u = 0; u < U; ++u) {
@@ -361,7 +467,14 @@
                 const bf16x8_t bfrag = __builtin_bit_cast(bf16x8_t, bv);
 #pragma unroll
                 for (int t = 0; t < NT; ++t) {
-                    if constexpr (F8)
+                    if constexpr (W12) {
+                        const CT(&cs)[NT] = (&src == &w0) ? c0 : c1;
+                        uint32_t cw;
+                        if constexpr (U == 2) cw = cs[t][u]; else cw = cs[t];
+                        flat_u32x4 o = flat_w12_frag(src[t][0][2 * u], src[t][0][2 * u + 1], cw, wb4[t]);
+                        if ((xs[t] & 0xffu) == (uint32_t)ii) flat_w12_patch(o, mt[t], xs[t], (uint32_t)ii, lane);
+                        acc[t] = __builtin_amdgcn_mfma_f32_16x16x32_bf16(__builtin_bit_cast(bf16x8_t, o), bfrag, acc[t], 0, 0, 0);
+                    } else if constexpr (F8)
                         acc[t] = __builtin_amdgcn_mfma_f32_16x16x32_bf16(flat_f8_frag(src[t][0][2 * u], src[t][0][2 * u + 1], flat_f8_scale(ev[t])), bfrag, acc[t], 0, 0, 0);
                     else
                         acc[t] = __builtin_amdgcn_mfma_f32_16x16x32_bf16(__builtin_bit_cast(bf16x8_t, src[t][u]), bfrag, acc[t], 0, 0, 0);
diff --git a/unimoe_audio_amd/csrc/umoe_moe_flat.hip b/unimoe_audio_amd/csrc/umoe_moe_flat.hip
--- a/unimoe_audio_amd/csrc/umoe_moe_flat.hip
+++ b/unimoe_audio_amd/csrc/umoe_moe_flat.hip
@@ -11,8 +11,9 @@
 
 #define FLAT_RIDER_LDS 512
 
-template <bool F8>
-__device__ __forceinline__ void moe_flat_body(const flat_args& A, const umoe_router_args& ra, const umoe_rider_pub& pub, const int lds_gemm, const flat_f8* F) {
+template <bool F8, bool W12 = false>
+__device__ __forceinline__ void moe_flat_body(const flat_args& A, const umoe_router_args& ra, const umoe_rider_pub& pub, const int lds_gemm, const flat_f8* F,
+                                              const flat_w12* Wm = nullptr) {
     extern __shared__ __attribute__((aligned(16))) char smem[];
     const unsigned b = blockIdx.x;
     const unsigned eg = A.gu[b], ed = A.dn[b];
@@ -40,10 +41,10 @@
     }
     const int fp0 = (int)(eg & 2047u), np = (int)((eg >> 11) & 7u);
     switch (np) {
-        case 4: flat_gateup<4, true, F8>(A, pub, fp0, b, smem, st, (int)threadIdx.x, F); break;
-        case 5: flat_gateup<5, true, F8>(A, pub, fp0, b, smem, st, (int)threadIdx.x, F); break;
-        case 6: flat_gateup<6, true, F8>(A, pub, fp0, b, smem, st, (int)threadIdx.x, F); break;
-        case 7: flat_gateup<7, true, F8>(A, pub, fp0, b, smem, st, (int)threadIdx.x, F); break;
+        case 4: flat_gateup<4, true, F8, W12>(A, pub, fp0, b, smem, st, (int)threadIdx.x, F, Wm); break;
+        case 5: flat_gateup<5, true, F8, W12>(A, pub, fp0, b, smem, st, (int)threadIdx.x, F, Wm); break;
+        case 6: flat_gateup<6, true, F8, W12>(A, pub, fp0, b, smem, st, (int)threadIdx.x, F, Wm); break;
+        case 7: flat_gateup<7, true, F8, W12>(A, pub, fp0, b, smem, st, (int)threadIdx.x, F, Wm); break;
         default: break;
     }
     for (int sl = 0; sl < FLAT_SLICES; ++sl) {
@@ -53,25 +54,25 @@
         __syncthreads();
         if (A.dn_kb[grp] & 1) {
             switch (nd) {
-                case 1: flat_down<1, 1, F8>(A, pub, grp, nb0, smem, st, 7 + 4 * sl, (int)threadIdx.x, F); break;
-                case 2: flat_down<2, 1, F8>(A, pub, grp, nb0, smem, st, 7 + 4 * sl, (int)threadIdx.x, F); break;
-                case 3: flat_down<3, 1, F8>(A, pub, grp, nb0, smem, st, 7 + 4 * sl, (int)threadIdx.x, F); break;
-                case 4: flat_down<4, 1, F8>(A, pub, grp, nb0, smem, st, 7 + 4 * sl, (int)threadIdx.x, F); break;
-                case 5: flat_down<5, 1, F8>(A, pub, grp, nb0, smem, st, 7 + 4 * sl, (int)threadIdx.x, F); break;
-                case 6: flat_down<6, 1, F8>(A, pub, grp, nb0, smem, st, 7 + 4 * sl, (int)threadIdx.x, F); break;
-                case 7: flat_down<7, 1, F8>(A, pub, grp, nb0, smem, st, 7 + 4 * sl, (int)threadIdx.x, F); break;
-                case 8: flat_down<8, 1, F8>(A, pub, grp, nb0, smem, st, 7 + 4 * sl, (int)threadIdx.x, F); break;
-                case 9: flat_down<9, 1, F8>(A, pub, grp, nb0, smem, st, 7 + 4 * sl, (int)threadIdx.x, F); break;
-                default: flat_down<10, 1, F8>(A, pub, grp, nb0, smem, st, 7 + 4 * sl, (int)threadIdx.x, F); break;
+                case 1: flat_down<1, 1, F8, W12>(A, pub, grp, nb0, smem, st, 7 + 4 * sl, (int)threadIdx.x, F, Wm); break;
+                case 2: flat_down<2, 1, F8, W12>(A, pub, grp, nb0, smem, st, 7 + 4 * sl, (int)threadIdx.x, F, Wm); break;
+                case 3: flat_down<3, 1, F8, W12>(A, pub, grp, nb0, smem, st, 7 + 4 * sl, (int)threadIdx.x, F, Wm); break;
+                case 4: flat_down<4, 1, F8, W12>(A, pub, grp, nb0, smem, st, 7 + 4 * sl, (int)threadIdx.x, F, Wm); break;
+                case 5: flat_down<5, 1, F8, W12>(A, pub, grp, nb0, smem, st, 7 + 4 * sl, (int)threadIdx.x, F, Wm); break;
+                case 6: flat_down<6, 1, F8, W12>(A, pub, grp, nb0, smem, st, 7 + 4 * sl, (int)threadIdx.x, F, Wm); break;
+                case 7: flat_down<7, 1, F8, W12>(A, pub, grp, nb0, smem, st, 7 + 4 * sl, (int)threadIdx.x, F, Wm); break;
+                case 8: flat_down<8, 1, F8, W12>(A, pub, grp, nb0, smem, st, 7 + 4 * sl, (int)threadIdx.x, F, Wm); break;
+                case 9: flat_down<9, 1, F8, W12>(A, pub, grp, nb0, smem, st, 7 + 4 * sl, (int)threadIdx.x, F, Wm); break;
+                default: flat_down<10, 1, F8, W12>(A, pub, grp, nb0, smem, st, 7 + 4 * sl, (int)threadIdx.x, F, Wm); break;
             }
         } else {
             switch (nd) {
-                case 1: flat_down<1, 2, F8>(A, pub, grp, nb0, smem, st, 7 + 4 * sl, (int)threadIdx.x, F); break;
-                case 2: flat_down<2, 2, F8>(A, pub, grp, nb0, smem, st, 7 + 4 * sl, (int)threadIdx.x, F); break;
-                case 3: flat_down<3, 2, F8>(A, pub, grp, nb0, smem, st, 7 + 4 * sl, (int)threadIdx.x, F); break;
-                case 4: flat_down<4, 2, F8>(A, pub, grp, nb0, smem, st, 7 + 4 * sl, (int)threadIdx.x, F); break;
-                case 5: flat_down<5, 2, F8>(A, pub, grp, nb0, smem, st, 7 + 4 * sl, (int)threadIdx.x, F); break;
-                default: flat_down<6, 2, F8>(A, pub, grp, nb0, smem, st, 7 + 4 * sl, (int)threadIdx.x, F); break;
+                case 1: flat_down<1, 2, F8, W12>(A, pub, grp, nb0, smem, st, 7 + 4 * sl, (int)threadIdx.x, F, Wm); break;
+                case 2: flat_down<2, 2, F8, W12>(A, pub, grp, nb0, smem, st, 7 + 4 * sl, (int)threadIdx.x, F, Wm); break;
+                case 3: flat_down<3, 2, F8, W12>(A, pub, grp, nb0, smem, st, 7 + 4 * sl, (int)threadIdx.x, F, Wm); break;
+                case 4: flat_down<4, 2, F8, W12>(A, pub, grp, nb0, smem, st, 7 + 4 * sl, (int)threadIdx.x, F, Wm); break;
+                case 5: flat_down<5, 2, F8, W12>(A, pub, grp, nb0, smem, st, 7 + 4 * sl, (int)threadIdx.x, F, Wm); break;
+                default: flat_down<6, 2, F8, W12>(A, pub, grp, nb0, smem, st, 7 + 4 * sl, (int)threadIdx.x, F, Wm); break;
             }
         }
     }
@@ -91,6 +92,11 @@
 __global__ __launch_bounds__(512, 1) void moe_flat_fp8_kernel(const flat_args A, const umoe_router_args ra, const umoe_rider_pub pub, const int lds_gemm,
                                                               const flat_f8 F) {
     moe_flat_body<true>(A, ra, pub, lds_gemm, &F);
+}
+
+__global__ __launch_bounds__(512, 1) void moe_flat_w12_kernel(const flat_args A, const umoe_router_args ra, const umoe_rider_pub pub, const int lds_gemm,
+                                                              const flat_w12 W) {
+    moe_flat_body<false, true>(A, ra, pub, lds_gemm, nullptr, &W);
 }
 
 struct FlatPlan {
@@ -107,6 +113,7 @@
     int rider_less, heavy_at;
     double rider, stage, flagc, pair_scale;
     int fp8;
+    double wcost() const { return fp8 == 1 ? 0.5 : fp8 == 2 ? 0.75 : 1.0; }
     bool operator==(const FlatShape& o) const { return memcmp(this, &o, sizeof(*this)) == 0; }
 };
 
@@ -117,7 +124,7 @@
     for (int j = 0; j < n; ++j) { fre[j] = avail[j]; o.n[j] = 0; }
     for (int q = 0; q < sh.G; ++q) {
         const int i = ex[q];
-        const double se = seam[sh.dn_src[i]], cb = sh.fp8 ? 0.5 * sh.dn_kb[i] : (double)sh.dn_kb[i];
+        const double se = seam[sh.dn_src[i]], cb = sh.wcost() * sh.dn_kb[i];
         const int ndmax = (sh.dn_kb[i] & 1) ? FLAT_ND_MAX1 : FLAT_ND_MAX2;
         int left = sh.dn_nb[i], next = 0;
         while (left > 0) {
@@ -149,10 +156,10 @@
     for (int i = 0; i < G; ++i) { pair0[i] = P; P += sh.pairs[i]; }
     pair0[G] = P;
     if (P >= 2048) return;
-    const double cp = sh.fp8 ? (double)sh.kb_gu : 2.0 * sh.kb_gu;
+    const double cp = sh.wcost() * 2.0 * sh.kb_gu;
     double total = P * cp + S * sh.rider + n * sh.stage;
     int kb_big = 0;
-    for (int i = 0; i < G; ++i) { total += (sh.fp8 ? 0.5 : 1.0) * sh.dn_nb[i] * sh.dn_kb[i]; kb_big = std::max(kb_big, sh.dn_kb[i]); }
+    for (int i = 0; i < G; ++i) { total += sh.wcost() * sh.dn_nb[i] * sh.dn_kb[i]; kb_big = std::max(kb_big, sh.dn_kb[i]); }
     FlatPlan best;
     double best_T = 1e30;
     std::vector<int> np(n), fp0(n);
@@ -260,7 +267,7 @@
 }
 
 static int moe_flat_launch(const umoe_gemm_args* gu, const umoe_gemm_args* dn, uint32_t* flags, int flag_words, int n_wg, hipStream_t s,
-                           const flat_f8* f8) {
+                           const flat_f8* f8, const flat_w12* w12 = nullptr) {
     UMOE_REQUIRE(gu && dn && flags, "umoe_moe_flat: null argument");
     const int G = gu->num_groups;
     if (!(gu->fused_router && gu->rider_pub && gu->groups_host && dn->groups_host && G == dn->num_groups && G <= FLAT_MAXG && gu->prologue == UMOE_PRO_PLAIN &&
@@ -292,10 +299,11 @@
         sh.dn_src[i] = j;
     }
     flat_knobs(sh);
-    sh.fp8 = f8 ? 1 : 0;
-    static FlatShape cached_shapes[2];
-    static FlatPlan cached_plans[2];
-    static bool haves[2] = {false, false};
+    sh.fp8 = f8 ? 1 : w12 ? 2 : 0;
+    if (w12 && (sh.kb_gu & 1)) return 1;
+    static FlatShape cached_shapes[3];
+    static FlatPlan cached_plans[3];
+    static bool haves[3] = {false, false, false};
     FlatShape& cached_shape = cached_shapes[sh.fp8];
     FlatPlan& cached_plan = cached_plans[sh.fp8];
     bool& have = haves[sh.fp8];
@@ -338,8 +346,9 @@
     lds = std::max(lds, (size_t)8 * 2 * FLAT_NP_MAX * 1024);
     lds = std::max(lds, (size_t)8 * FLAT_ND_MAX1 * 1024);
     if (lds + FLAT_RIDER_LDS > 160 * 1024) return 1;
-    static size_t configured[2] = {0, 0};
-    const void* kfn = f8 ? reinterpret_cast<const void*>(&moe_flat_fp8_kernel) : reinterpret_cast<const void*>(&moe_flat_kernel);
+    static size_t configured[3] = {0, 0, 0};
+    const void* kfn = f8 ? reinterpret_cast<const void*>(&moe_flat_fp8_kernel)
+                         : w12 ? reinterpret_cast<const void*>(&moe_flat_w12_kernel) : reinterpret_cast<const void*>(&moe_flat_kernel);
     if (lds + FLAT_RIDER_LDS > configured[sh.fp8]) {
         UMOE_HIP(hipFuncSetAttribute(kfn, hipFuncAttributeMaxDynamicSharedMemorySize, (int)(lds + FLAT_RIDER_LDS)));
         configured[sh.fp8] = lds + FLAT_RIDER_LDS;
@@ -347,6 +356,7 @@
     umoe_router_args rr = *r;
     rr.h_out = nullptr;
     if (f8) moe_flat_fp8_kernel<<<dim3((unsigned)n_wg), 512, lds + FLAT_RIDER_LDS, s>>>(A, rr, pub, (int)lds, *f8);
+    else if (w12) moe_flat_w12_kernel<<<dim3((unsigned)n_wg), 512, lds + FLAT_RIDER_LDS, s>>>(A, rr, pub, (int)lds, *w12);
     else moe_flat_kernel<<<dim3((unsigned)n_wg), 512, lds + FLAT_RIDER_LDS, s>>>(A, rr, pub, (int)lds);
     UMOE_LAUNCH_CHECK();
     return 0;
@@ -366,6 +376,19 @@
         F.e_gu[i] = e_gu[i]; F.e_dn[i] = e_dn[i];
     }
     return moe_flat_launch(gu, dn, flags, flag_words, n_wg, s, &F);
+}
+
+int umoe_moe_flat_w12(const umoe_gemm_args* gu, const umoe_gemm_args* dn, const uint32_t* const* m_gu, const uint32_t* const* m_dn, uint32_t* flags,
+                      int flag_words, int n_wg, hipStream_t s) {
+    UMOE_REQUIRE(m_gu && m_dn && gu && dn && gu->num_groups <= FLAT_MAXG, "umoe_moe_flat_w12: bad argument");
+    flat_w12 W;
+    memset(&W, 0, sizeof(W));
+    for (int i = 0; i < gu->num_groups; ++i) {
+        UMOE_REQUIRE(m_gu[i] && m_dn[i], "umoe_moe_flat_w12: group %d has no block records", i);
+        UMOE_REQUIRE(dn->groups_host && dn->groups_host[i].k / 32 < 127, "umoe_moe_flat_w12: group %d: K too large for the exception records", i);
+        W.m_gu[i] = m_gu[i]; W.m_dn[i] = m_dn[i];
+    }
+    return moe_flat_launch(gu, dn, flags, flag_words, n_wg, s, nullptr, &W);
 }
 
 bool umoe_moe_flat_feasible(int n_wg, int S, int D, int I_dyn, int I_sh, int n_real, int n_fix) {
@@ -411,6 +434,10 @@
     return flat_plan_probe(n_wg, S, D, I_dyn, I_sh, n_real, n_fix, out, out_len, 0);
 }
 
+extern "C" int umoe_moe_flat_plan_w12_probe(int n_wg, int S, int D, int I_dyn, int I_sh, int n_real, int n_fix, double* out, int out_len) {
+    return flat_plan_probe(n_wg, S, D, I_dyn, I_sh, n_real, n_fix, out, out_len, 2);
+}
+
 extern "C" int umoe_moe_flat_plan_fp8_probe(int n_wg, int S, int D, int I_dyn, int I_sh, int n_real, int n_fix, double* out, int out_len) {
     return flat_plan_probe(n_wg, S, D, I_dyn, I_sh, n_real, n_fix, out, out_len, 1);
 }
diff --git a/unimoe_audio_amd/model.py b/unimoe_audio_amd/model.py
--- a/unimoe_audio_amd/model.py
+++ b/unimoe_audio_amd/model.py
@@ -1,6 +1,7 @@
 from __future__ import annotations
 
 import ctypes as C
+import os
 from dataclasses import dataclass
 from typing import Dict, List, NamedTuple, Optional, Tuple
 
@@ -8,7 +9,7 @@
 import torch.nn as nn
 
 from . import _lib as L
-from . import ops, quant
+from . import ops, quant, w12
 from . import row_params as RP
 from .codec_utils import DecoderOutput
 from .config import UniMoEAudioConfig
@@ -325,6 +326,20 @@
     def _pack_key(self):
         return tuple((p.data_ptr(), p._version) for n, p in self.named_parameters() if not n.startswith("visual."))
 
+    def packed_w12(self) -> list:
+        key = self._pack_key()
+        if getattr(self, "_pk12", None) is not None and self._pk12_key == key:
+            return self._pk12
+        D = self.config.hidden_size
+        out = []
+        for lp in self.packed()["layers"]:
+            pk = lp["moe"]
+            gu = [w12.pack(t.view(torch.int16), D // 32) for t in pk["exp_gu"] + pk["sh_gu"]]
+            dn = [w12.pack(t.view(torch.int16), t.numel() // (D // 16 * 512)) for t in pk["exp_dn"] + pk["sh_dn"]]
+            out.append(None if any(x is None for x in gu + dn) else dict(gu=gu, dn=dn))
+        self._pk12, self._pk12_key = out, key
+        return out
+
     def engine(self, batch: int, max_prompt: int, max_tokens: int, attn_splits: int = 8, ep=None,
                expert_weights: Optional[str] = None) -> "DecodeEngine":
         need_L = max_prompt + max_tokens + 8
@@ -481,6 +496,7 @@
         self.ep = ep
         self.ep_rank, self.ep_size = (0, 1) if ep is None else (ep.rank, ep.size)
         self.pack_key = model._pack_key()
+        self.w12 = fmt == "bf16" and self.ep_size == 1 and self.rows <= 16 and os.environ.get("UMOE_FLAT_W12", "1") != "0"
         h = C.c_void_p()
         L.check(L.lib().umoe_engine_create(C.byref(c), C.byref(h)), "umoe_engine_create")
         self.h = h
@@ -546,6 +562,8 @@
             L.check(lib.umoe_engine_set_layer(self.h, li, C.byref(w)), "umoe_engine_set_layer")
             if self.expert_weights in ("fp8", "fp8-only"):
                 self._set_layer_fp8(li, ex, sh)
+            elif self.w12:
+                self._set_layer_w12(li)
         emb, head = mpk["emb"], mpk["head"]
         max_pos = self.Lmax + 4104 if max_pos_override is None else int(max_pos_override)
         self.max_pos = max_pos
@@ -555,6 +573,15 @@
         L.check(lib.umoe_engine_set_globals(self.h, m.language_model.norm.weight.data_ptr(), emb.data_ptr(), head.data_ptr(),
                                             cos.data_ptr(), sin.data_ptr(), max_pos, delay), "umoe_engine_set_globals")
         torch.cuda.synchronize()
+
+    def _set_layer_w12(self, li):
+        pk = self.model.packed_w12()[li]
+        if pk is None:
+            return
+        self._k(pk)
+        arr = lambda ts: (C.c_void_p * len(ts))(*[t.data_ptr() for t in ts])
+        L.check(L.lib().umoe_engine_set_layer_w12(self.h, li, arr([d for d, _ in pk["gu"]]), arr([m for _, m in pk["gu"]]),
+                                                  arr([d for d, _ in pk["dn"]]), arr([m for _, m in pk["dn"]])), "umoe_engine_set_layer_w12")
 
     def _set_layer_fp8(self, li, ex, sh):
         gu8, gue, dn8, dne = [], [], [], []
diff --git a/unimoe_audio_amd/w12.py b/unimoe_audio_amd/w12.py
--- /dev/null
+++ b/unimoe_audio_amd/w12.py
@@ -0,0 +1,90 @@
+from typing import Optional, Tuple
+
+import torch
+
+CAP = 32
+META = 40
+SENTINEL = 0xFFFFFFFF
+
+
+def wp16_from_rows(W: torch.Tensor) -> torch.Tensor:
+    N, K = W.shape
+    assert N % 16 == 0 and K % 32 == 0, (N, K)
+    v = W.contiguous().view(torch.int16).view(N // 16, 16, 4, K // 32, 8)
+    return v.permute(0, 3, 2, 1, 4).contiguous().view(-1)
+
+
+def rows_from_wp16(p: torch.Tensor, N: int, K: int) -> torch.Tensor:
+    v = p.view(N // 16, K // 32, 4, 16, 8).permute(0, 3, 2, 1, 4).contiguous()
+    return v.view(N, K).view(torch.bfloat16)
+
+
+def wp16_gate_up(Wg: torch.Tensor, Wu: torch.Tensor) -> torch.Tensor:
+    I, K = Wg.shape
+    both = torch.stack([Wg.view(I // 16, 16, K), Wu.view(I // 16, 16, K)], 1).reshape(2 * I, K)
+    return wp16_from_rows(both)
+
+
+def steps_per_chunk(KB: int) -> int:
+    return 2 if KB % 2 == 0 else 1
+
+
+def block_bytes(KB: int) -> int:
+    return KB * 768
+
+
+def pack(wp16: torch.Tensor, KB: int, cap: int = CAP) -> Optional[Tuple[torch.Tensor, torch.Tensor]]:
+    assert cap <= CAP and wp16.dtype == torch.int16 and wp16.numel() % (KB * 512) == 0 and 0 < KB < 127
+    NB = wp16.numel() // (KB * 512)
+    CS = steps_per_chunk(KB)
+    v = wp16.view(NB, KB, 64, 8).to(torch.int32) & 0xFFFF
+    lo, hb = v & 0xFF, v >> 8
+    e7, sg = hb & 0x7F, hb >> 7
+    hist = torch.zeros(NB, 129, dtype=torch.int64, device=v.device)
+    hist[:, 1:].scatter_add_(1, e7.view(NB, -1).to(torch.int64), torch.ones(1, dtype=torch.int64, device=v.device).expand(NB, KB * 512))
+    cum = hist.cumsum(1)
+    wb = (cum[:, 8:] - cum[:, :-8]).argmax(1).to(torch.int32)
+    off = e7 - wb.view(NB, 1, 1, 1)
+    inwin = (off >= 0) & (off < 8)
+    code = torch.where(inwin, (sg << 3) | off, torch.zeros_like(off))
+    exc = (~inwin).nonzero()
+    meta = torch.full((NB, META), -1, dtype=torch.int64, device=v.device)
+    if exc.shape[0]:
+        cnt = torch.bincount(exc[:, 0], minlength=NB)
+        if int(cnt.max()) > cap:
+            return None
+        first = cnt.cumsum(0) - cnt
+        rank = torch.arange(exc.shape[0], device=v.device) - first[exc[:, 0]]
+        val = v[exc[:, 0], exc[:, 1], exc[:, 2], exc[:, 3]].to(torch.int64)
+        meta[exc[:, 0], rank] = (exc[:, 1] << 25) | (exc[:, 2] << 19) | (exc[:, 3] << 16) | val
+    meta[:, META - 1] = wb.to(torch.int64)
+    meta = torch.where(meta >= 2 ** 31, meta - 2 ** 32, meta).to(torch.int32)
+    cb = torch.stack([code[..., 0] | (code[..., 2] << 4), code[..., 1] | (code[..., 3] << 4),
+                      code[..., 4] | (code[..., 6] << 4), code[..., 5] | (code[..., 7] << 4)], -1)
+    lows = lo.view(NB, KB // CS, CS, 64, 8).permute(0, 1, 3, 2, 4).reshape(NB, KB * 512)
+    codes = cb.view(NB, KB // CS, CS, 64, 4).permute(0, 1, 3, 2, 4).reshape(NB, KB * 256)
+    data = torch.cat([lows, codes], 1).to(torch.uint8).contiguous().view(-1)
+    return data, meta.contiguous().view(-1)
+
+
+def unpack(data: torch.Tensor, meta: torch.Tensor, KB: int) -> torch.Tensor:
+    NB = meta.numel() // META
+    CS = steps_per_chunk(KB)
+    d = data.view(NB, KB * 768).to(torch.int32)
+    lo = d[:, : KB * 512].view(NB, KB // CS, 64, CS, 8).permute(0, 1, 3, 2, 4).reshape(NB, KB, 64, 8)
+    cb = d[:, KB * 512:].view(NB, KB // CS, 64, CS, 4).permute(0, 1, 3, 2, 4).reshape(NB, KB, 64, 4)
+    l4, h4 = cb & 0xF, cb >> 4
+    code = torch.stack([l4[..., 0], l4[..., 1], h4[..., 0], h4[..., 1], l4[..., 2], l4[..., 3], h4[..., 2], h4[..., 3]], -1)
+    m = meta.view(NB, META).to(torch.int64) & 0xFFFFFFFF
+    wb = m[:, META - 1].to(torch.int32).view(NB, 1, 1, 1)
+    v = (((code & 8) << 4) | ((code & 7) + wb)) << 8 | lo
+    ent = m[:, : CAP + 1]
+    nb, r = (ent != SENTINEL).nonzero(as_tuple=True)
+    en = ent[nb, r]
+    v[nb, (en >> 25) & 0x7F, (en >> 19) & 63, (en >> 16) & 7] = (en & 0xFFFF).to(torch.int32)
+    return torch.where(v >= 0x8000, v - 0x10000, v).to(torch.int16).view(-1)
+
+
+def exceptions_per_block(meta: torch.Tensor) -> torch.Tensor:
+    m = meta.view(-1, META).to(torch.int64) & 0xFFFFFFFF
+    return (m[:, : CAP + 1] != SENTINEL).sum(1)
```

New measurement: 3022 audio-tokens/s (median of 6 runs). +12.0%, better.
